# ansonb/FeTA_TMLR

Hardware: AMD Instinct MI355X
Metric: graphs/sec fwd+bwd, ZINC batch (N<=37,d=64,K=16) (higher is better)
Workload: dtype f32; 1 GPU; ZINC-shaped synthetic padded-graph batch, ChebConvDynamic block (attention + coefficient generator + spectral filter), fwd+bwd; graphs_per_gpu=128, global_batch=128, n_pad=37, d_model=64, heads=4, filter_order=4, k_eig=16, filter_mode=spectral, layers=3, norm=batch(per-rank stats), hip_graph=True, backward=single, two_phase=False, graph_collectives=False, ranks=1, parallelism=dp1

## Files before the change

### feta_tmlr_amd/_abi.py

```python
import ctypes as C
import os

import torch

_F = C.c_void_p
_I = C.c_void_p
_S = C.c_void_p

SIGNATURES = {
    'feta_version': ([], C.c_int),
    'feta_last_error': ([], C.c_char_p),
    'feta_attn_fwd': ([_F, _F, _F, C.c_int64, C.c_int64, _F, _I, _F, C.c_int64, C.c_int64,
                       _F, _F, C.c_float, C.c_int, C.c_int, C.c_int, C.c_int, _S], C.c_int),
    'feta_attn_bwd': ([_F, _F, _F, C.c_int64, C.c_int64, _F, _I, _F, _F, _F, C.c_int64, C.c_int64,
                       _F, _F, _F, _F, _F, C.c_float, C.c_int, C.c_int, C.c_int, C.c_int, _S],
                      C.c_int),
    'feta_coeff_fwd': ([_F, _I, _F, _F, _F, _F, C.c_int, C.c_int, C.c_int, C.c_int, _S], C.c_int),
    'feta_coeff_bwd_groups': ([C.c_int, C.c_int], C.c_int),
    'feta_coeff_bwd': ([_F, _I, _F, _F, _F, _F, _F, _F, _F, C.c_int, C.c_int, C.c_int, C.c_int, C.c_int, _S],
                       C.c_int),
    'feta_colsum': ([_F, _F, C.c_int, C.c_int, _S], C.c_int),
    'feta_cheb_filter_fwd': ([_F, C.c_int64, C.c_int64, _F, _F, _F, _I, _F, C.c_int64, C.c_int64,
                              C.c_int, C.c_int, C.c_int, C.c_int, C.c_int, C.c_int, _S], C.c_int),
    'feta_cheb_filter_bwd': ([_F, C.c_int64, C.c_int64, _F, _F, _I, _F, C.c_int64, C.c_int64,
                              _F, _F, _F, C.c_int, C.c_int, C.c_int, C.c_int, C.c_int, C.c_int, _S],
                             C.c_int),
    'feta_spec_filter_fwd': ([_F, C.c_int64, C.c_int64, _F, _F, _F, _F, _I, _F, C.c_int64, C.c_int64,
                              C.c_int, C.c_int, C.c_int, C.c_int, C.c_int, C.c_int, C.c_int, _S],
                             C.c_int),
    'feta_spec_filter_bwd': ([_F, C.c_int64, C.c_int64, _F, _F, _F, _I, _F, C.c_int64, C.c_int64,
                              _F, _F, _F, C.c_int, C.c_int, C.c_int, C.c_int, C.c_int, C.c_int,
                              C.c_int, _S], C.c_int),
    'feta_rowlin_blocks': ([C.c_int], C.c_int),
    'feta_rowlin_chunks': ([C.c_int], C.c_int),
    'feta_rowlin_fwd': ([_F, _F, _F, _F, _F, _F, _F, C.c_int, C.c_int, C.c_int, C.c_int, _S], C.c_int),
    'feta_rowlin_bwd': ([_F, _F, _F, _F, _F, _F, _F, _F, C.c_int, C.c_int, C.c_int, _S], C.c_int),
    'feta_bn_stats': ([_F, _F, C.c_int, C.c_int, _S], C.c_int),
    'feta_bn_stats_shift': ([_F, _F, _F, C.c_int, C.c_int, _S], C.c_int),
    'feta_bn_apply_fwd': ([_F, _F, _F, _F, _F, _F, _F, _F, _I, C.c_float, C.c_float, C.c_int, C.c_int, _S],
                          C.c_int),
    'feta_bn_bwd': ([_F, _F, _F, _F, _F, _F, _F, _F, C.c_int, C.c_int, _S], C.c_int),
    'feta_lhat_from_edges': ([_I, C.c_int64, _I, _I, _F, _F, C.c_int, C.c_int, C.c_int64, _S],
                             C.c_int),
    'feta_layernorm_blocks': ([C.c_int], C.c_int),
    'feta_layernorm_fwd': ([_F, _F, _F, C.c_float, _F, _F, C.c_int, C.c_int, _S], C.c_int),
    'feta_layernorm_bwd': ([_F, _F, _F, _F, _F, _F, C.c_int, _F, C.c_int, C.c_int, _S], C.c_int),
    'feta_layernorm_fwd_ex': ([_F, _F, _F, C.c_float, _F, _F, C.c_int, C.c_int, C.c_int, C.c_int, _S], C.c_int),
    'feta_layernorm_bwd_eps': ([_F, _F, _F, C.c_float, _F, _F, _F, C.c_int, _F, C.c_int, C.c_int, C.c_int, C.c_int, C.c_int, _S],
                               C.c_int),
    'feta_layernorm_bwd_ex': ([_F, _F, _F, _F, _F, _F, C.c_int, _F, C.c_int, C.c_int, C.c_int, C.c_int, C.c_int, _S],
                              C.c_int),
    'feta_eigh_sym_supported': ([C.c_int], C.c_int),
    'feta_eigh_sym_workspace_bytes': ([C.c_int, C.c_int], C.c_int64),
    'feta_eigh_sym': ([_F, _I, C.c_float, _F, _F, _I, _F, C.c_int, C.c_int, C.c_int, C.c_int, C.c_float, _S],
                      C.c_int),
    'feta_spectral_kernel': ([_F, _F, _I, C.c_int, C.c_float, C.c_int, C.c_float, C.c_int, _F,
                              C.c_int, C.c_int, C.c_int, _S], C.c_int),
}

SIGNATURES.update({
    'feta_attn_fwd_bf16': SIGNATURES['feta_attn_fwd'],
    'feta_attn_bwd_bf16': ([_F, _F, _F, C.c_int64, C.c_int64, _F, _I, _F, _F, C.c_int64, C.c_int64,
                            _F, _F, _F, _F, _F, C.c_float, C.c_int, C.c_int, C.c_int, C.c_int, _S], C.c_int),
    'feta_attn_fwd_drop': ([_F, _F, _F, C.c_int64, C.c_int64, _F, _I, _F, C.c_int64, C.c_int64, _F, _F, C.c_float,
                            C.c_float, C.c_uint64, C.c_uint64, C.c_int, C.c_int, C.c_int, C.c_int, C.c_int, _S], C.c_int),
    'feta_attn_bwd_drop': ([_F, _F, _F, C.c_int64, C.c_int64, _F, _I, _F, _F, C.c_int64, C.c_int64, _F, _F, _F, _F, _F,
                            C.c_float, C.c_float, C.c_uint64, C.c_uint64, C.c_int, C.c_int, C.c_int, C.c_int, C.c_int,
                            _S], C.c_int),
    'feta_attn_fwd_drop_dev': ([_F, _F, _F, C.c_int64, C.c_int64, _F, _I, _F, C.c_int64, C.c_int64, _F, _F, C.c_float,
                                C.c_float, _I, C.c_uint64, C.c_int, C.c_int, C.c_int, C.c_int, C.c_int, _S], C.c_int),
    'feta_attn_bwd_drop_dev': ([_F, _F, _F, C.c_int64, C.c_int64, _F, _I, _F, _F, C.c_int64, C.c_int64, _F, _F, _F, _F, _F,
                                C.c_float, C.c_float, _I, C.c_uint64, C.c_int, C.c_int, C.c_int, C.c_int, C.c_int,
                                _S], C.c_int),
    'feta_attn_fwd_stab': ([_F, _F, _F, C.c_int64, C.c_int64, _F, _I, _F, C.c_int64, C.c_int64, _F, _F, C.c_float,
                            C.c_int, C.c_int, C.c_int, C.c_int, C.c_int, C.c_int, _S], C.c_int),
    'feta_attn_bwd_stab': ([_F, _F, _F, C.c_int64, C.c_int64, _F, _I, _F, _F, C.c_int64, C.c_int64, _F, _F, _F, _F, _F,
                            C.c_float, C.c_int, C.c_int, C.c_int, C.c_int, C.c_int, C.c_int, _S], C.c_int),
    'feta_spec_filter_fwd_bf16': SIGNATURES['feta_spec_filter_fwd'],
    'feta_spec_filter_bwd_bf16': SIGNATURES['feta_spec_filter_bwd'],
})


class ColsumSeg(C.Structure):
    _fields_ = [('in_', _F), ('out', _F), ('R', C.c_int), ('C', C.c_int), ('ld', C.c_int),
                ('bcast_out', _F), ('bcast_rows', C.c_int)]


SIGNATURES['feta_colsum_multi'] = ([C.POINTER(ColsumSeg), C.c_int, _S], C.c_int)
SIGNATURES['feta_lin_supported'] = ([C.c_int, C.c_int, C.c_int], C.c_int)
SIGNATURES['feta_lin_fwd'] = ([_F, _F, _F, _F, C.c_int, C.c_int, C.c_int, _S], C.c_int)
SIGNATURES['feta_lin_bwd'] = ([_F, _F, _F, _F, _F, _F, C.c_int, C.c_int, C.c_int, C.POINTER(ColsumSeg), C.c_int, _S],
                              C.c_int)
SIGNATURES['feta_lin_fwd_ex'] = ([_F, _F, _F, _F, C.c_int, C.c_int, C.c_int, C.c_int, _S], C.c_int)
SIGNATURES['feta_lin_bwd_ex'] = ([_F, _F, _F, _F, _F, _F, C.c_int, C.c_int, C.c_int, C.POINTER(ColsumSeg), C.c_int, C.c_int,
                                  _S], C.c_int)


class RowLinEx(C.Structure):
    _fields_ = [
        ('x', _F), ('w', _F), ('bias', _F), ('rowscale', _F),
        ('M', C.c_int), ('KI', C.c_int), ('NO', C.c_int), ('relu', C.c_int),
        ('residual', _F), ('res_bn', _F), ('y', _F), ('stats', _F),
        ('x_bn', _F), ('x_stats', _F), ('Gx', C.c_int),
        ('x_gamma', _F), ('x_beta', _F), ('x_bn_out', _F), ('x_rmean', _F), ('x_rvar', _F), ('x_nbt', _I),
        ('momentum', C.c_float), ('eps', C.c_float),
        ('dy', _F), ('relu_y', _F), ('dx', _F), ('partial', _F), ('partial_ld', C.c_int),
        ('g_y', _F), ('g_bn', _F), ('g_sum', _F), ('Gs', C.c_int),
        ('g_fin', _F), ('g_fin_out', _F), ('dgamma', _F), ('dbeta', _F),
        ('add_plain', _F), ('add_dout', _F), ('add_y', _F), ('add_bn', _F), ('add_fin', _F),
        ('x2', _F), ('x_split', C.c_int), ('dx2', _F),
        ('sum_y', _F), ('sum_bn', _F), ('sum_out', _F), ('stats_shift', _F),
    ]


SIGNATURES.update({
    'feta_rowlin_fwd_ex': ([C.POINTER(RowLinEx), _S], C.c_int),
    'feta_rowlin_bwd_ex': ([C.POINTER(RowLinEx), _F, _S], C.c_int),
    'feta_bn_apply_fwd_prm': ([_F, _F, _F, _F, _F, _F, _F, _F, _I, C.c_float, C.c_float, C.c_int, C.c_int,
                               C.c_int, _S], C.c_int),
    'feta_bn_bwd_reduce': ([_F, _F, _F, _F, C.c_int, C.c_int, _S], C.c_int),
})



class SpecCat(C.Structure):
    _fields_ = [
        ('y2', _F), ('y2_sb', C.c_int64), ('y2_sn', C.c_int64), ('y2_bn', _F), ('y2_stats', _F), ('Gx', C.c_int),
        ('gamma', _F), ('beta', _F), ('bn_out', _F), ('rmean', _F), ('rvar', _F), ('nbt', _I),
        ('momentum', C.c_float), ('eps', C.c_float), ('M', C.c_int), ('w_cat', _F), ('b_cat', _F), ('out', _F),
    ]


class SpecCatGrad(C.Structure):
    _fields_ = [
        ('dout', _F), ('y2', _F), ('y2_sb', C.c_int64), ('y2_sn', C.c_int64), ('y2_bn', _F), ('filt', _F), ('w_cat', _F),
        ('dxn', _F), ('gs', _F), ('partial', _F), ('partial_ld', C.c_int64),
    ]


SIGNATURES.update({
    'feta_spec_cat_bwd_supported': ([C.c_int] * 6, C.c_int),
    'feta_spec_cat_bwd_rows': ([C.c_int], C.c_int),
    'feta_spec_filter_cat_bwd': ([_F, C.c_int64, C.c_int64, _F, _F, _F, _I, C.c_int64, C.c_int64, _F, _F, _F,
                                  C.c_int, C.c_int, C.c_int, C.c_int, C.c_int, C.c_int, C.c_int, C.POINTER(SpecCatGrad), _S],
                                 C.c_int),
    'feta_spec_cat_supported': ([C.c_int] * 6, C.c_int),
    'feta_spec_filter_cat_fwd': ([_F, C.c_int64, C.c_int64, _F, _F, _F, _F, _I, _F, C.c_int64, C.c_int64,
                                  C.c_int, C.c_int, C.c_int, C.c_int, C.c_int, C.c_int, C.c_int, C.POINTER(SpecCat), _S], C.c_int),
})


class AttnBlock(C.Structure):
    _fields_ = [
        ('x', _F), ('x_bn', _F), ('x_stats', _F), ('Gx', C.c_int),
        ('x_gamma', _F), ('x_beta', _F), ('x_bn_out', _F), ('x_rmean', _F), ('x_rvar', _F), ('x_nbt', _I),
        ('momentum', C.c_float), ('eps', C.c_float),
        ('w_in', _F), ('b_in', _F), ('w_out', _F), ('b_out', _F), ('pe', _F), ('n_real', _I),
        ('rowscale', _F), ('qkv', _F), ('out', _F), ('attn_stats', _F), ('attn', _F), ('y', _F),
        ('y_stats', _F), ('scale', C.c_float), ('B', C.c_int), ('N', C.c_int), ('M', C.c_int),
        ('row_sb', C.c_int64), ('row_sn', C.c_int64), ('tie_qk', C.c_int), ('dtype', C.c_int), ('y_shift', _F),
        ('out_f32', _F), ('x_ln_gamma', _F), ('x_ln_beta', _F), ('H', C.c_int),
    ]


SIGNATURES.update({
    'feta_attn_block_supported': ([C.c_int, C.c_int, C.c_int], C.c_int),
    'feta_attn_block_stat_rows': ([C.c_int, C.c_int], C.c_int),
    'feta_attn_out_supported': ([C.c_int, C.c_int, C.c_int], C.c_int),
    'feta_attn_out_stat_rows': ([C.c_int, C.c_int], C.c_int),
    'feta_attn_out_fwd': ([C.POINTER(AttnBlock), _S], C.c_int),
    'feta_attn_out_fwd_sums': ([C.POINTER(AttnBlock), C.POINTER(ColsumSeg), C.c_int, _S], C.c_int),
    'feta_attn_block_fwd': ([C.POINTER(AttnBlock), _S], C.c_int),
    'feta_attn_block_fwd_sums': ([C.POINTER(AttnBlock), C.POINTER(ColsumSeg), C.c_int, _S], C.c_int),
})



class CoeffFwdRole(C.Structure):
    _fields_ = [('attn', _F), ('n_real', _I), ('s', _F), ('gcn_bias', _F), ('cj', _F), ('pooled', _F),
                ('B', C.c_int), ('N', C.c_int), ('H', C.c_int), ('C', C.c_int)]


class CoeffBwdRole(C.Structure):
    _fields_ = [('cj', _F), ('n_real', _I), ('s', _F), ('gcn_bias', _F), ('dpooled', _F), ('partial', _F),
                ('B', C.c_int), ('N', C.c_int), ('H', C.c_int), ('C', C.c_int)]


class Ffn(C.Structure):
    _fields_ = [
        ('x', _F), ('x_bn', _F), ('x_stats', _F), ('Gx', C.c_int),
        ('x_gamma', _F), ('x_beta', _F), ('x_bn_out', _F), ('x_rmean', _F), ('x_rvar', _F), ('x_nbt', _I),
        ('momentum', C.c_float), ('eps', C.c_float),
        ('w1', _F), ('b1', _F), ('w2', _F), ('b2', _F), ('h', _F), ('y', _F), ('y_stats', _F),
        ('M', C.c_int), ('FF', C.c_int), ('dtype', C.c_int), ('y_shift', _F), ('y_f32', C.c_int),
        ('x_ln_gamma', _F), ('x_ln_beta', _F),
        ('y_ln_out', _F), ('y_ln_gamma', _F), ('y_ln_beta', _F), ('y_ln_eps', C.c_float), ('y_ln_f32', C.c_int),
    ]


SIGNATURES.update({
    'feta_ffn_supported': ([C.c_int, C.c_int], C.c_int),
    'feta_ffn_blocks': ([C.c_int], C.c_int),
    'feta_ffn_fwd': ([C.POINTER(Ffn), _S], C.c_int),
    'feta_ffn_fwd_coeff': ([C.POINTER(Ffn), C.POINTER(CoeffFwdRole), _S], C.c_int),
})

class AttnBlockGrad(C.Structure):
    _fields_ = [
        ('dy', _F), ('y1', _F), ('bn1', _F), ('g_sum', _F), ('Gs', C.c_int), ('fin_out', _F), ('dgamma', _F),
        ('dbeta', _F), ('rowscale', _F), ('w_out', _F), ('w_in', _F), ('qkv', _F), ('out', _F), ('dout2', _F),
        ('pe', _F), ('n_real', _I), ('attn_stats', _F), ('x0', _F), ('bn0', _F), ('dx', _F), ('dx_b', _F), ('sum_out', _F),
        ('partial', _F), ('partial_ld', C.c_int), ('scale', C.c_float), ('B', C.c_int), ('N', C.c_int), ('M', C.c_int),
        ('row_sb', C.c_int64), ('row_sn', C.c_int64), ('dtype', C.c_int), ('dout2_f32', C.c_int),
        ('ln1_gamma', _F), ('x0_ln_gamma', _F), ('x0_ln_beta', _F), ('ln_eps', C.c_float), ('H', C.c_int),
    ]


SIGNATURES.update({
    'feta_attn_block_bwd_supported': ([C.c_int, C.c_int, C.c_int], C.c_int),
    'feta_attn_block_bwd_blocks': ([C.c_int], C.c_int),
    'feta_attn_block_bwd': ([C.POINTER(AttnBlockGrad), _S], C.c_int),
    'feta_attn_block_bwd_sums': ([C.POINTER(AttnBlockGrad), C.POINTER(ColsumSeg), C.c_int, _S], C.c_int),
})


class FfnGrad(C.Structure):
    _fields_ = [
        ('dy', _F), ('dy_b', _F), ('g_y', _F), ('g_bn', _F), ('g_sum', _F), ('Gs', C.c_int), ('g_fin', _F), ('g_fin_out', _F),
        ('dgamma', _F), ('dbeta', _F), ('h', _F), ('w2', _F), ('w1', _F), ('x', _F), ('x_bn', _F), ('dx', _F),
        ('sum_out', _F), ('partial', _F), ('partial_ld', C.c_int), ('M', C.c_int), ('FF', C.c_int), ('dtype', C.c_int), ('g_f32', C.c_int),
        ('g_ln_gamma', _F), ('x_ln_gamma', _F), ('x_ln_beta', _F), ('ln_eps', C.c_float),
    ]


SIGNATURES.update({
    'feta_ffn_bwd_supported': ([C.c_int, C.c_int], C.c_int),
    'feta_ffn_bwd_blocks': ([C.c_int], C.c_int),
    'feta_ffn_bwd_chunks': ([C.c_int, C.c_int], C.c_int),
    'feta_ffn_bwd': ([C.POINTER(FfnGrad), _S], C.c_int),
    'feta_ffn_bwd_coeff': ([C.POINTER(FfnGrad), C.POINTER(CoeffBwdRole), _S], C.c_int),
})

class EncoderLayer(C.Structure):
    _fields_ = [
        ('w_in', _F), ('b_in', _F), ('w_out', _F), ('b_out', _F),
        ('n1_gamma', _F), ('n1_beta', _F), ('n1_mean', _F), ('n1_var', _F),
        ('w1', _F), ('b1', _F), ('w2', _F), ('b2', _F),
        ('n2_gamma', _F), ('n2_beta', _F), ('n2_mean', _F), ('n2_var', _F),
        ('n1_eps', C.c_float), ('n2_eps', C.c_float), ('tie_qk', C.c_int),
    ]


class EncoderInfer(C.Structure):
    _fields_ = [
        ('x', _F), ('row_sb', C.c_int64), ('row_sn', C.c_int64), ('pe', _F), ('n_real', _I), ('rowscale', _F),
        ('y', _F), ('out', _F), ('attn', _F), ('B', C.c_int), ('N', C.c_int), ('H', C.c_int), ('FF', C.c_int),
        ('L', C.c_int), ('norm', C.c_int), ('layers', C.c_void_p),
    ]


class EncoderInferEx(C.Structure):
    _fields_ = EncoderInfer._fields_ + [('dtype', C.c_int), ('in_dtype', C.c_int)]


class EncoderFwdSave(C.Structure):
    _fields_ = EncoderInferEx._fields_ + [
        ('qkv', _F), ('out_save', _F), ('attn_stats', _F), ('y1', _F), ('h', _F), ('y2', _F), ('y2_last_f32', _F),
        ('qkv_stride', C.c_int64), ('out_stride', C.c_int64), ('attn_stats_stride', C.c_int64), ('y1_stride', C.c_int64),
        ('h_stride', C.c_int64), ('y2_stride', C.c_int64),
    ]


SIGNATURES.update({
    'feta_encoder_fwd_save_supported': ([C.c_int, C.c_int, C.c_int, C.c_int, C.c_int, C.c_int, C.c_int], C.c_int),
    'feta_encoder_fwd_save': ([C.POINTER(EncoderFwdSave), _S], C.c_int),
    'feta_encoder_fwd_save_sums': ([C.POINTER(EncoderFwdSave), C.POINTER(ColsumSeg), C.c_int, _S], C.c_int),
    'feta_encoder_infer_supported': ([C.c_int, C.c_int, C.c_int, C.c_int, C.c_int], C.c_int),
    'feta_encoder_infer': ([C.POINTER(EncoderInfer), _S], C.c_int),
    'feta_encoder_infer_ex_supported': ([C.c_int, C.c_int, C.c_int, C.c_int, C.c_int, C.c_int], C.c_int),
    'feta_encoder_infer_ex': ([C.POINTER(EncoderInferEx), _S], C.c_int),
})

ABI_VERSION = 13


class FetaError(RuntimeError):
    pass


def _p(t):
    return None if t is None else C.c_void_p(t.data_ptr())


def _same_dtype(dtype, *tensors):
    for t in tensors:
        if t is not None and t.dtype != dtype:
            raise TypeError('expected %s operands, got %s' % (dtype, t.dtype))


def _stack_dtype(ptrs, names, f32_ok=()):
    dt = None
    for k in names:
        t = ptrs.get(k)
        if t is None or k in f32_ok and t.dtype == torch.float32:
            continue
        if dt is None:
            dt = t.dtype
        elif t.dtype != dt:
            raise TypeError('%s is %s, the other token tensors are %s' % (k, t.dtype, dt))
    if dt is None:
        dt = torch.float32
    if dt not in (torch.float32, torch.bfloat16):
        raise TypeError('token tensors must be float32 or bfloat16, got %s' % dt)
    for k, t in ptrs.items():
        if t is not None and k not in names and t.dtype == torch.bfloat16:
            raise TypeError('%s must not be bfloat16' % k)
    return 1 if dt == torch.bfloat16 else 0


def tok_strides(t):
    assert t.dim() == 4 and t.stride(3) == 1 and t.stride(2) == t.shape[3], \
        'token tensor must be a [B,N,H,dh] view with dense (H,dh)'
    return (t.stride(0) if t.shape[0] > 1 else 0), (t.stride(1) if t.shape[1] > 1 else 0)
# ... 44 lines not shown
                                                    1 if q.dtype == torch.bfloat16 else 0, b, n, h, dh, stream),
                        'feta_attn_fwd_drop')
            return
        if q.dtype == torch.bfloat16:
            _same_dtype(torch.bfloat16, k, v, pe, out, attn)
            self._check(self.lib.feta_attn_fwd_bf16(_p(q), _p(k), _p(v), sb, sn, _p(pe), _p(n_real),
                                                    _p(out), osb, osn, _p(attn), _p(stats), scale,
                                                    b, n, h, dh, stream), 'feta_attn_fwd_bf16')
            return
        self._check(self.lib.feta_attn_fwd(_p(q), _p(k), _p(v), sb, sn, _p(pe), _p(n_real),
                                           _p(out), osb, osn, _p(attn), _p(stats), scale,
                                           b, n, h, dh, stream), 'feta_attn_fwd')

    @staticmethod
    def attn_bwd_takes_dout2(n, dh, dtype=torch.float32, heads=None):
        if dtype != torch.float32:
            return False
        head_kernel = os.environ.get('FETA_ATTN_BWD_HEAD', '1') != '0'
        return (n <= 64 and dh <= 16) or (head_kernel and n <= 256 and dh == 16 and heads == 4)

    def attn_bwd(self, q, k, v, pe, n_real, out, dout, stats, delta, dq, dk, dv, scale, stream, dout2=None,
                 drop=None, clamp5=False):
        b, n, h, dh = q.shape
        sb, sn = tok_strides(q)
        for t in (k, v, dq, dk, dv):
            assert tok_strides(t) == (sb, sn)
        osb, osn = tok_strides(out)
        assert tok_strides(dout) == (osb, osn)
        if clamp5:
            assert dout2 is None and (drop is None or drop[0] == 0.0)
            _same_dtype(q.dtype, k, v, pe, out, dout, dq, dk, dv)
            self._check(self.lib.feta_attn_bwd_stab(_p(q), _p(k), _p(v), sb, sn, _p(pe), _p(n_real), _p(out), _p(dout),
                                                    osb, osn, _p(stats), _p(delta), _p(dq), _p(dk), _p(dv), scale, 1,
                                                    1 if q.dtype == torch.bfloat16 else 0, b, n, h, dh, stream),
                        'feta_attn_bwd_stab')
            return
        if drop is not None and drop[0] > 0.0 and torch.is_tensor(drop[1]):
            _same_dtype(q.dtype, k, v, pe, out, dout, dq, dk, dv)
            assert dout2 is None
            self._check(self.lib.feta_attn_bwd_drop_dev(_p(q), _p(k), _p(v), sb, sn, _p(pe), _p(n_real), _p(out), _p(dout),
                                                        osb, osn, _p(stats), _p(delta), _p(dq), _p(dk), _p(dv), scale,
                                                        float(drop[0]), _p(drop[1]), int(drop[2]),
                                                        1 if q.dtype == torch.bfloat16 else 0, b, n, h, dh, stream),
                        'feta_attn_bwd_drop_dev')
            return
        if drop is not None and drop[0] > 0.0:
            _same_dtype(q.dtype, k, v, pe, out, dout, dq, dk, dv)
            assert dout2 is None
            self._check(self.lib.feta_attn_bwd_drop(_p(q), _p(k), _p(v), sb, sn, _p(pe), _p(n_real), _p(out), _p(dout),
                                                    osb, osn, _p(stats), _p(delta), _p(dq), _p(dk), _p(dv), scale,
                                                    float(drop[0]), int(drop[1]), int(drop[2]),
                                                    1 if q.dtype == torch.bfloat16 else 0, b, n, h, dh, stream),
                        'feta_attn_bwd_drop')
            return
        if q.dtype == torch.bfloat16:
            _same_dtype(torch.bfloat16, k, v, pe, out, dout, dq, dk, dv)
            assert dout2 is None
            self._check(self.lib.feta_attn_bwd_bf16(_p(q), _p(k), _p(v), sb, sn, _p(pe), _p(n_real),
                                                    _p(out), _p(dout), osb, osn, _p(stats), _p(delta),
                                                    _p(dq), _p(dk), _p(dv), scale, b, n, h, dh, stream),
                        'feta_attn_bwd_bf16')
            return
        self._check(self.lib.feta_attn_bwd(_p(q), _p(k), _p(v), sb, sn, _p(pe), _p(n_real),
                                           _p(out), _p(dout), _p(dout2), osb, osn, _p(stats), _p(delta),
                                           _p(dq), _p(dk), _p(dv), scale, b, n, h, dh, stream),
                    'feta_attn_bwd')

    def coeff_fwd(self, attn, n_real, s, gcn_bias, cj, pooled, stream):
        b, h, n, _ = attn.shape
        c = s.shape[0]
        self._check(self.lib.feta_coeff_fwd(_p(attn), _p(n_real), _p(s), _p(gcn_bias), _p(cj),
                                            _p(pooled), b, n, h, c, stream), 'feta_coeff_fwd')

    def coeff_bwd_groups(self, b, h):
        return self.lib.feta_coeff_bwd_groups(b, h)

    def coeff_bwd(self, cj, n_real, s, gcn_bias, dpooled, partial, ds, dbias, b, n, h, stream, dw_dense=None):
        c = s.shape[0]
        self._check(self.lib.feta_coeff_bwd(_p(cj), _p(n_real), _p(s), _p(gcn_bias), _p(dpooled),
                                            _p(partial), _p(ds), _p(dbias), _p(dw_dense),
                                            0 if dw_dense is None else dw_dense.shape[0], b, n, h, c, stream),
                    'feta_coeff_bwd')

    @staticmethod
    def _colsum_segs(pairs):
        segs = (ColsumSeg * max(len(pairs), 1))()
        for sg, pr in zip(segs, pairs):
            x, out = pr[0], pr[1]
            assert x.stride(1) == 1
            sg.in_, sg.out, sg.R, sg.C, sg.ld = x.data_ptr(), out.data_ptr(), x.shape[0], x.shape[1], x.stride(0)
            if len(pr) > 2 and pr[2] is not None:
                sg.bcast_out, sg.bcast_rows = pr[2].data_ptr(), pr[2].shape[0]
        return segs

    def colsum_multi(self, pairs, stream):
        self._check(self.lib.feta_colsum_multi(self._colsum_segs(pairs), len(pairs), stream), 'feta_colsum_multi')

    def lin_supported(self, r, k, n):
        return bool(self.lib.feta_lin_supported(r, k, n))

    def lin_fwd(self, x, w, bias, y, stream, bf16=False):
        r, k = x.shape
        self._check(self.lib.feta_lin_fwd_ex(_p(x), _p(w), _p(bias), _p(y), r, k, w.shape[0], int(bool(bf16)), stream),
                    'feta_lin_fwd')

    def lin_bwd(self, x, w, dy, dx, dw, db, stream, pairs=(), bf16=False):
        r, k = x.shape
        self._check(self.lib.feta_lin_bwd_ex(_p(x), _p(w), _p(dy), _p(dx), _p(dw), _p(db), r, k, w.shape[0],
                                             self._colsum_segs(pairs), len(pairs), int(bool(bf16)), stream),
                    'feta_lin_bwd')

    def colsum(self, x, out, stream):
        r, c = x.shape
        self._check(self.lib.feta_colsum(_p(x), _p(out), r, c, stream), 'feta_colsum')

    def cheb_filter_fwd(self, x, lhat, coeff, bias, n_real, y, order, share, stream):
        b, n, h, dh = x.shape
        xsb, xsn = tok_strides(x)
        ysb, ysn = tok_strides(y)
        self._check(self.lib.feta_cheb_filter_fwd(_p(x), xsb, xsn, _p(lhat), _p(coeff), _p(bias),
                                                  _p(n_real), _p(y), ysb, ysn, b, n, h, dh, order,
                                                  int(share), stream), 'feta_cheb_filter_fwd')

    def cheb_filter_bwd(self, x, lhat, coeff, n_real, dy, dx, dcoeff, dbias_part, order, share,
                        stream):
        b, n, h, dh = x.shape
        xsb, xsn = tok_strides(x)
        assert tok_strides(dx) == (xsb, xsn)
        ysb, ysn = tok_strides(dy)
        self._check(self.lib.feta_cheb_filter_bwd(_p(x), xsb, xsn, _p(lhat), _p(coeff), _p(n_real),
                                                  _p(dy), ysb, ysn, _p(dx), _p(dcoeff),
                                                  _p(dbias_part), b, n, h, dh, order, int(share),
                                                  stream), 'feta_cheb_filter_bwd')

    def spec_filter_fwd(self, x, u, lam, coeff, bias, n_real, y, order, share, stream):
        b, n, h, dh = x.shape
        k = u.shape[2]
        xsb, xsn = tok_strides(x)
        ysb, ysn = tok_strides(y)
        fn, nm = self.lib.feta_spec_filter_fwd, 'feta_spec_filter_fwd'
        if x.dtype == torch.bfloat16:
            _same_dtype(torch.bfloat16, u, coeff, y)
            fn, nm = self.lib.feta_spec_filter_fwd_bf16, 'feta_spec_filter_fwd_bf16'
        self._check(fn(_p(x), xsb, xsn, _p(u), _p(lam), _p(coeff), _p(bias), _p(n_real), _p(y), ysb, ysn,
                       b, n, h, dh, order, k, int(share), stream), nm)

    def spec_cat_supported(self, n, h, dh, order, k, share):
        return bool(self.lib.feta_spec_cat_supported(n, h, dh, order, k, int(share)))

    def spec_filter_cat_fwd(self, x, u, lam, coeff, bias, n_real, y, order, share, stream, y2, w_cat, b_cat, out,
                            y2_bn=None, y2_stats=None, Gx=0, gamma=None, beta=None, bn_out=None, rmean=None, rvar=None,
                            nbt=None, momentum=0.1, eps=1e-5):
        b, n, h, dh = x.shape
        k = u.shape[2]
        xsb, xsn = tok_strides(x)
        ysb, ysn = tok_strides(y)
        assert tok_strides(out) == (ysb, ysn)
        c = SpecCat()
        c.y2_sb, c.y2_sn = tok_strides(y2)
        c.Gx, c.momentum, c.eps, c.M = Gx, momentum, eps, b * n
        for name, t in (('y2', y2), ('y2_bn', y2_bn), ('y2_stats', y2_stats), ('gamma', gamma), ('beta', beta),
                        ('bn_out', bn_out), ('rmean', rmean), ('rvar', rvar), ('nbt', nbt), ('w_cat', w_cat),
                        ('b_cat', b_cat), ('out', out)):
            if t is not None:
                setattr(c, name, t.data_ptr())
        self._check(self.lib.feta_spec_filter_cat_fwd(_p(x), xsb, xsn, _p(u), _p(lam), _p(coeff), _p(bias), _p(n_real), _p(y),
                                                      ysb, ysn, b, n, h, dh, order, k, int(share), C.byref(c), stream),
                    'feta_spec_filter_cat_fwd')

    def spec_cat_bwd_supported(self, n, h, dh, order, k, share):
        return bool(self.lib.feta_spec_cat_bwd_supported(n, h, dh, order, k, int(share)))

    def spec_cat_bwd_rows(self, b):
        return int(self.lib.feta_spec_cat_bwd_rows(b))

    def spec_filter_cat_bwd(self, x, u, lam, coeff, n_real, filt, dx, dcoeff, dbias_part, order, share, stream, dout, y2,
                            w_cat, dxn, partial, y2_bn=None, gs=None):
        b, n, h, dh = x.shape
        k = u.shape[2]
        xsb, xsn = tok_strides(x)
        assert tok_strides(dx) == (xsb, xsn)
        ysb, ysn = tok_strides(filt)
        c = SpecCatGrad()
        c.y2_sb, c.y2_sn = tok_strides(y2)
        assert tok_strides(dout) == (c.y2_sb, c.y2_sn) and tok_strides(dxn) == (c.y2_sb, c.y2_sn)
        assert partial.shape[0] == self.spec_cat_bwd_rows(b) and partial.stride(1) == 1
        assert gs is None or gs.shape[0] == partial.shape[0]
        c.partial_ld = partial.stride(0)
        for name, t in (('dout', dout), ('y2', y2), ('y2_bn', y2_bn), ('filt', filt), ('w_cat', w_cat), ('dxn', dxn),
                        ('gs', gs), ('partial', partial)):
            if t is not None:
                setattr(c, name, t.data_ptr())
        self._check(self.lib.feta_spec_filter_cat_bwd(_p(x), xsb, xsn, _p(u), _p(lam), _p(coeff), _p(n_real), ysb, ysn,
                                                      _p(dx), _p(dcoeff), _p(dbias_part), b, n, h, dh, order, k, int(share),
                                                      C.byref(c), stream), 'feta_spec_filter_cat_bwd')

    def spec_filter_bwd(self, x, u, lam, coeff, n_real, dy, dx, dcoeff, dbias_part, order, share,
                        stream):
        b, n, h, dh = x.shape
        k = u.shape[2]
        xsb, xsn = tok_strides(x)
        assert tok_strides(dx) == (xsb, xsn)
        ysb, ysn = tok_strides(dy)
        fn, nm = self.lib.feta_spec_filter_bwd, 'feta_spec_filter_bwd'
        if x.dtype == torch.bfloat16:
            _same_dtype(torch.bfloat16, u, coeff, dy, dx, dcoeff)
            fn, nm = self.lib.feta_spec_filter_bwd_bf16, 'feta_spec_filter_bwd_bf16'
        self._check(fn(_p(x), xsb, xsn, _p(u), _p(lam), _p(coeff), _p(n_real), _p(dy), ysb, ysn, _p(dx),
                       _p(dcoeff), _p(dbias_part), b, n, h, dh, order, k, int(share), stream), nm)

    ROWLIN_DIMS = (16, 32, 64, 128, 192, 256)

    def rowlin_blocks(self, m):
        return self.lib.feta_rowlin_blocks(m)

    def rowlin_chunks(self, m):
        return self.lib.feta_rowlin_chunks(m)

    def rowlin_fwd(self, x, w, bias, rowscale, residual, y, stats, relu, stream):
        m, ki = x.shape
        no = w.shape[0]
        self._check(self.lib.feta_rowlin_fwd(_p(x), _p(w), _p(bias), _p(rowscale), _p(residual), _p(y),
                                             _p(stats), int(relu), m, ki, no, stream), 'feta_rowlin_fwd')

    def rowlin_bwd(self, x, w, dy, rowscale, ysaved, dx, partial, dwdb, stream):
        m, ki = x.shape
        no = w.shape[0]
        self._check(self.lib.feta_rowlin_bwd(_p(x), _p(w), _p(dy), _p(rowscale), _p(ysaved), _p(dx),
                                             _p(partial), _p(dwdb), m, ki, no, stream), 'feta_rowlin_bwd')

    def bn_stats(self, y, stats, stream, shift=None):
        m, d = y.shape
        assert stats.shape[0] == self.rowlin_blocks(m) + 1, 'stats needs rowlin_blocks(M) + 1 rows (shift row)'
        self._check(self.lib.feta_bn_stats_shift(_p(y), _p(shift), _p(stats), m, d, stream), 'feta_bn_stats')

    def bn_apply_fwd(self, y, stats, gamma, beta, out, mean_rstd, running_mean, running_var, momentum,
                     eps, stream, nbt=None):
        m, d = y.shape
        self._check(self.lib.feta_bn_apply_fwd(_p(y), _p(stats), _p(gamma), _p(beta), _p(out),
                                               _p(mean_rstd), _p(running_mean), _p(running_var), _p(nbt),
                                               momentum, eps, m, d, stream), 'feta_bn_apply_fwd')

    def bn_bwd(self, y, dout, mean_rstd, gamma, partial, dy, dgamma, dbeta, stream):
        m, d = y.shape
        self._check(self.lib.feta_bn_bwd(_p(y), _p(dout), _p(mean_rstd), _p(gamma), _p(partial), _p(dy),
                                         _p(dgamma), _p(dbeta), m, d, stream), 'feta_bn_bwd')

    def rowlin_ex(self, m, ki, no, relu=False, momentum=0.1, eps=1e-5, Gx=0, Gs=0, partial_ld=0,
# ... 60 lines not shown

    def attn_block_bwd_supported(self, n, d_model, heads):
        return bool(self.lib.feta_attn_block_bwd_supported(n, d_model, heads))

    def attn_block_bwd_blocks(self, b):
        return int(self.lib.feta_attn_block_bwd_blocks(b))

    def attn_block_bwd(self, b, n, scale, stream, seq_first=True, Gs=0, partial_ld=0, partial_ptr=None, sums=(), ln_eps=1e-5,
                       heads=4, **ptrs):
        d = AttnBlockGrad()
        d.B, d.N, d.M, d.scale, d.Gs, d.partial_ld, d.ln_eps, d.H = b, n, b * n, scale, Gs, partial_ld, ln_eps, heads
        d.row_sb, d.row_sn = (1, b) if seq_first else (n, 1)
        if partial_ptr is not None:
            d.partial = partial_ptr
        d.dtype = _stack_dtype(ptrs, ('dy', 'y1', 'qkv', 'out', 'dout2', 'pe', 'x0', 'dx', 'dx_b'), f32_ok=('dout2',))
        d.dout2_f32 = int(ptrs.get('dout2') is not None and ptrs['dout2'].dtype == torch.float32)
        for k, t in ptrs.items():
            if t is not None:
                setattr(d, k, t.data_ptr())
        if sums:
            self._check(self.lib.feta_attn_block_bwd_sums(C.byref(d), self._colsum_segs(sums), len(sums), stream),
                        'feta_attn_block_bwd_sums')
        else:
            self._check(self.lib.feta_attn_block_bwd(C.byref(d), stream), 'feta_attn_block_bwd')

    def ffn_supported(self, d_model, ff):
        return bool(self.lib.feta_ffn_supported(d_model, ff))

    def ffn_blocks(self, m):
        return int(self.lib.feta_ffn_blocks(m))

    def ffn_fwd(self, m, ff, stream, momentum=0.1, eps=1e-5, Gx=0, coeff=None, y_ln_eps=1e-5, **ptrs):
        self.ffn_launch(self.ffn_desc(m, ff, momentum, eps, Gx, y_ln_eps=y_ln_eps, **ptrs), stream, coeff)

    def ffn_desc(self, m, ff, momentum=0.1, eps=1e-5, Gx=0, y_ln_eps=1e-5, **ptrs):
        d = Ffn()
        d.M, d.FF, d.momentum, d.eps, d.Gx, d.y_ln_eps = m, ff, momentum, eps, Gx, y_ln_eps
        d.dtype = _stack_dtype(ptrs, ('x', 'h', 'y', 'y_ln_out'), f32_ok=('y', 'y_ln_out'))
        d.y_f32 = int(ptrs['y'].dtype == torch.float32)
        if ptrs.get('y_ln_out') is not None:
            d.y_ln_f32 = int(ptrs['y_ln_out'].dtype == torch.float32)
        for k, t in ptrs.items():
            if t is not None:
                setattr(d, k, t.data_ptr())
        return d

    def ffn_launch(self, desc, stream, coeff=None):
        if coeff is None:
            self._check(self.lib.feta_ffn_fwd(C.byref(desc), stream), 'feta_ffn_fwd')
            return
        attn, n_real, s, gcn_bias, cj, pooled = coeff
        b, h, n, _ = attn.shape
        r = CoeffFwdRole()
        r.attn, r.n_real, r.s, r.gcn_bias, r.cj, r.pooled = (t.data_ptr() for t in (attn, n_real, s, gcn_bias, cj, pooled))
        r.B, r.N, r.H, r.C = b, n, h, s.shape[0]
        self._check(self.lib.feta_ffn_fwd_coeff(C.byref(desc), C.byref(r), stream), 'feta_ffn_fwd_coeff')

    def ffn_bwd_supported(self, d_model, ff):
        return bool(self.lib.feta_ffn_bwd_supported(d_model, ff))

    def ffn_bwd_blocks(self, m):
        return int(self.lib.feta_ffn_bwd_blocks(m))

    def ffn_bwd_chunks(self, m, ff):
        return int(self.lib.feta_ffn_bwd_chunks(m, ff))

    def ffn_bwd_desc(self, m, ff, Gs=0, partial_ld=0, partial_ptr=None, ln_eps=1e-5, **ptrs):
        d = FfnGrad()
        d.M, d.FF, d.Gs, d.partial_ld, d.ln_eps = m, ff, Gs, partial_ld, ln_eps
        if partial_ptr is not None:
            d.partial = partial_ptr
        d.dtype = _stack_dtype(ptrs, ('dy', 'dy_b', 'g_y', 'h', 'x', 'dx'), f32_ok=('dy', 'g_y'))
        d.g_f32 = int(ptrs['dy'].dtype == torch.float32)
        if ptrs.get('g_y') is not None and ptrs['g_y'].dtype != ptrs['dy'].dtype:
            raise TypeError('dy and g_y must share a dtype')
        for k, t in ptrs.items():
            if t is not None:
                setattr(d, k, t.data_ptr())
        return d

    def ffn_bwd_launch(self, desc, stream, coeff=None):
        if coeff is None:
            self._check(self.lib.feta_ffn_bwd(C.byref(desc), stream), 'feta_ffn_bwd')
            return
        cj, n_real, s, gcn_bias, dpooled, partial, b, n, h = coeff
        r = CoeffBwdRole()
        r.cj, r.n_real, r.s, r.gcn_bias, r.dpooled, r.partial = (t.data_ptr() for t in
                                                                (cj, n_real, s, gcn_bias, dpooled, partial))
        r.B, r.N, r.H, r.C = b, n, h, s.shape[0]
        self._check(self.lib.feta_ffn_bwd_coeff(C.byref(desc), C.byref(r), stream), 'feta_ffn_bwd_coeff')

    def ffn_bwd(self, m, ff, stream, coeff=None, **kw):
        self.ffn_bwd_launch(self.ffn_bwd_desc(m, ff, **kw), stream, coeff)

    def bn_apply_fwd_prm(self, y, stats, gamma, beta, out, bn_prm, running_mean, running_var, momentum,
                         eps, stream, nbt=None):
        m, d = y.shape
        self._check(self.lib.feta_bn_apply_fwd_prm(_p(y), _p(stats), _p(gamma), _p(beta), _p(out),
                                                   _p(bn_prm), _p(running_mean), _p(running_var), _p(nbt),
                                                   momentum, eps, m, d, stats.shape[0] - 1, stream),
                    'feta_bn_apply_fwd_prm')

    def bn_bwd_reduce(self, y, dout, bn_prm, partial, stream):
        m, d = y.shape
        self._check(self.lib.feta_bn_bwd_reduce(_p(y), _p(dout), _p(bn_prm), _p(partial), m, d, stream),
                    'feta_bn_bwd_reduce')

    def lhat_from_edges(self, edge_index, node_graph, node_off, deg, lhat, stream):
        b, n, _ = lhat.shape
        self._check(self.lib.feta_lhat_from_edges(_p(edge_index), edge_index.shape[1],
                                                  _p(node_graph), _p(node_off), _p(deg), _p(lhat),
                                                  b, n, node_graph.shape[0], stream),
                    'feta_lhat_from_edges')

    def layernorm_blocks(self, m):
        return self.lib.feta_layernorm_blocks(m)

    @staticmethod
    def _dt(t):
        if t.dtype == torch.float32:
            return 0
        if t.dtype == torch.bfloat16:
            return 1
        raise TypeError('float32 or bfloat16 rows, got %s' % t.dtype)

    def layernorm_fwd(self, y, gamma, beta, eps, out, stats, stream):
        m, d = y.shape
        self._check(self.lib.feta_layernorm_fwd_ex(_p(y), _p(gamma), _p(beta), eps, _p(out), _p(stats), m, d,
                                                   self._dt(y), self._dt(out), stream), 'feta_layernorm_fwd')

    def layernorm_bwd(self, dout, y, stats, gamma, dy, partial, dgdb, stream, partial_ld=0, partial_ptr=None, eps=1e-5):
        m, d = y.shape
        pp = _p(partial) if partial_ptr is None else C.c_void_p(partial_ptr)
        self._check(self.lib.feta_layernorm_bwd_eps(_p(dout), _p(y), _p(stats), eps, _p(gamma), _p(dy), pp, partial_ld,
                                                    _p(dgdb), m, d, self._dt(dout), self._dt(y), self._dt(dy), stream),
                    'feta_layernorm_bwd')

    def eigh_sym_supported(self, n):
        return bool(self.lib.feta_eigh_sym_supported(n))

    def eigh_sym_workspace_bytes(self, b, n):
        return int(self.lib.feta_eigh_sym_workspace_bytes(b, n))

    def eigh_sym(self, a, n_real, shift, u, lam, sweeps, max_sweeps, tol, stream, workspace=None):
        b, n, k = u.shape
        if workspace is None and self.eigh_sym_workspace_bytes(b, n) > 0:
            workspace = torch.empty(self.eigh_sym_workspace_bytes(b, n) // 4, dtype=torch.float32, device=a.device)
        self._check(self.lib.feta_eigh_sym(_p(a), _p(n_real), shift, _p(u), _p(lam), _p(sweeps), _p(workspace),
                                           b, n, k, max_sweeps, tol, stream), 'feta_eigh_sym')

    def spectral_kernel(self, u, lam, n_real, mode, beta, p, lam_offset, zero_diag, out, stream):
        b, n, k = u.shape
        self._check(self.lib.feta_spectral_kernel(_p(u), _p(lam), _p(n_real), mode, beta, p, lam_offset,
                                                  int(zero_diag), _p(out), b, n, k, stream),
                    'feta_spectral_kernel')

    def encoder_infer_supported(self, n, d_model, heads, ff, nl):
        return bool(self.lib.feta_encoder_infer_supported(n, d_model, heads, ff, nl))

    @staticmethod
    def _encoder_table(layers):
        table = (EncoderLayer * len(layers))()
        for e, lp in zip(table, layers):
            for k, v in lp.items():
                if torch.is_tensor(v):
                    _same_dtype(torch.float32, v)
# ... 85 lines not shown
```

### feta_tmlr_amd/csrc/coeff.hip

```cpp
#include <cmath>

#include "feta_abi_common.h"
#include <feta_device.h>
#include <cstdlib>

#include "feta_coeff.h"
#include "feta_colsum.h"

namespace feta {

__global__ __launch_bounds__(kCoeffThreads) void coeff_fwd_kernel(
    const float* __restrict__ attn, const int32_t* __restrict__ n_real, const float* __restrict__ s,
    const float* __restrict__ gbias, float* __restrict__ cj_out, float* __restrict__ pooled, int B,
    int N, int H, int C, int stage) {
  coeff_fwd_body(attn, n_real, s, gbias, cj_out, pooled, B, N, H, C, stage, (int)blockIdx.x, (int)blockIdx.y,
                 (int)gridDim.y);
}

__global__ __launch_bounds__(kCoeffWideThreads) void coeff_fwd_wide_kernel(
    const float* __restrict__ attn, const int32_t* __restrict__ n_real, const float* __restrict__ s,
    const float* __restrict__ gbias, float* __restrict__ cj_out, float* __restrict__ pooled, int B,
    int N, int H, int C) {
  coeff_fwd_body<kCoeffWideThreads>(attn, n_real, s, gbias, cj_out, pooled, B, N, H, C, 2, (int)blockIdx.x);
}

__global__ __launch_bounds__(kCoeffThreads) void coeff_bwd_kernel(
    const float* __restrict__ cj, const int32_t* __restrict__ n_real, const float* __restrict__ s,
    const float* __restrict__ gbias, const float* __restrict__ dpooled, float* __restrict__ partial,
    int B, int N, int H, int C, int G) {
  coeff_bwd_body(cj, n_real, s, gbias, dpooled, partial, B, N, H, C, G, (int)blockIdx.x, (int)blockIdx.y);
}

constexpr int kCsCols = 16, kCsSlices = 64;
__global__ __launch_bounds__(kCsCols * kCsSlices) void colsum_kernel(const float* __restrict__ in,
                                                                      float* __restrict__ out, int R,
                                                                      int C, int ld) {
  float* red = feta_lds;
  const int lc = threadIdx.x & (kCsCols - 1);
  const int slice = threadIdx.x / kCsCols;
  const int col = blockIdx.x * kCsCols + lc;
  float acc = 0.0f;
  if (col < C)
    for (int r = slice; r < R; r += kCsSlices) acc += in[(int64_t)r * ld + col];
  red[threadIdx.x] = acc;
  __syncthreads();
  for (int half = kCsSlices / 2; half >= 1; half >>= 1) {
    if (slice < half) red[threadIdx.x] += red[threadIdx.x + half * kCsCols];
    __syncthreads();
  }
  if (slice == 0 && col < C) out[col] = red[lc];
}

__global__ __launch_bounds__(64) void colsum_wide_kernel(const float* __restrict__ in, float* __restrict__ out,
                                                         int R, int C4, int ld) {
  const int c4 = blockIdx.x * 64 + threadIdx.x;
  if (c4 >= C4) return;
  const float* p = in + 4 * (int64_t)c4;
  float4 acc = make_float4(0.0f, 0.0f, 0.0f, 0.0f);
  int r = 0;
  for (; r + 8 <= R; r += 8) {
    float4 v[8];
#pragma unroll
    for (int i = 0; i < 8; ++i) v[i] = *reinterpret_cast<const float4*>(p + (int64_t)(r + i) * ld);
#pragma unroll
    for (int i = 0; i < 8; ++i) {
      acc.x += v[i].x; acc.y += v[i].y; acc.z += v[i].z; acc.w += v[i].w;
    }
  }
  for (; r < R; ++r) {
    const float4 v = *reinterpret_cast<const float4*>(p + (int64_t)r * ld);
    acc.x += v.x; acc.y += v.y; acc.z += v.z; acc.w += v.w;
  }
  *reinterpret_cast<float4*>(out + 4 * (int64_t)c4) = acc;
}

int launch_colsum_strided(const float* in, float* out, int R, int C, int ld, hipStream_t stream) {
  if (R <= 256 && C >= 4096 && (C & 3) == 0 && (ld & 3) == 0 && aligned16(in) && aligned16(out)) {
    const int c4 = C / 4;
    auto kern = colsum_wide_kernel;
    hipLaunchKernelGGL(kern, dim3((c4 + 63) / 64), dim3(64), 0, stream, in, out, R, c4, ld);
    return check_launch("feta_colsum");
  }
  const dim3 grid((C + kCsCols - 1) / kCsCols), block(kCsCols * kCsSlices);
  auto kern = colsum_kernel;
  hipLaunchKernelGGL(kern, grid, block, kCsCols * kCsSlices * sizeof(float), stream, in, out, R, C, ld);
  return check_launch("feta_colsum");
}
int launch_colsum(const float* in, float* out, int R, int C, hipStream_t stream) {
  return launch_colsum_strided(in, out, R, C, C, stream);
}

struct ColsumSegs {
  feta_colsum_seg seg[FETA_COLSUM_MAX_SEGS];
  int tile_end[FETA_COLSUM_MAX_SEGS];
  int nseg;
};

__global__ __launch_bounds__(kCsCols * kCsSlices) void colsum_multi_kernel(ColsumSegs a) {
  float* red = feta_lds;
  int si = 0;
  while (si + 1 < a.nseg && (int)blockIdx.x >= a.tile_end[si]) ++si;
  const feta_colsum_seg sg = a.seg[si];
  const int tile = (int)blockIdx.x - (si > 0 ? a.tile_end[si - 1] : 0);
  const int lc = threadIdx.x & (kCsCols - 1);
  const int slice = threadIdx.x / kCsCols;
  const int col = tile * kCsCols + lc;
  const int ld = sg.ld > 0 ? sg.ld : sg.C;
  float acc = 0.0f;
  if (col < sg.C)
    for (int r = slice; r < sg.R; r += kCsSlices) acc += sg.in[(int64_t)r * ld + col];
  red[threadIdx.x] = acc;
  __syncthreads();
  for (int half = kCsSlices / 2; half >= 1; half >>= 1) {
// ... 73 lines not shown
    a.tile_end[i] = tiles;
  }
  auto kern = colsum_multi_kernel;
  hipLaunchKernelGGL(kern, dim3(tiles), dim3(kCsCols * kCsSlices), kCsCols * kCsSlices * sizeof(float), stream, a);
  return check_launch("feta_colsum_multi");
}

}

using namespace feta;

extern "C" int feta_coeff_fwd(const float* attn, const int32_t* n_real, const float* s,
                              const float* gcn_bias, float* cj, float* pooled, int B, int N, int H,
                              int C, feta_stream_t stream) {
  FETA_REQUIRE(attn && n_real && s && gcn_bias && cj && pooled, "coeff_fwd: null pointer");
  FETA_REQUIRE(B > 0 && H > 0 && C > 0 && N > 0 && N <= kCoeffThreads,
               "coeff_fwd: need 0 < N <= %d (got %d)", kCoeffThreads, N);
  const int want = N > 64 ? 2 : 1;
  const int stage = sizeof(float) * (size_t)coeff_fwd_lds_floats_mode(N, want) <= 150 * 1024 ? want : 0;
  const size_t lds = sizeof(float) * (size_t)coeff_fwd_lds_floats_mode(N, stage);
  if (N > 64) {
    const size_t wide = sizeof(float) * (size_t)coeff_fwd_lds_floats_mode(N, 2, kCoeffWideThreads);
    const char* e = getenv("FETA_COEFF_WIDE");
    if (wide <= 160 * 1024 && !(e != nullptr && e[0] == '0')) {
      auto kern = coeff_fwd_wide_kernel;
      static LdsSeen wide_seen;
      allow_dynamic_lds(kern, wide, wide_seen);
      hipLaunchKernelGGL(kern, dim3(B * H), dim3(kCoeffWideThreads), wide, (hipStream_t)stream, attn, n_real, s, gcn_bias,
                         cj, pooled, B, N, H, C);
      return check_launch("feta_coeff_fwd");
    }
  }
  const int cs = (N > 64 && C >= 4 * kCoeffThreads) ? 4 : 1;
  const dim3 grid(B * H, cs), block(kCoeffThreads);
  auto kern = coeff_fwd_kernel;
  static LdsSeen lds_seen;
  allow_dynamic_lds(kern, lds, lds_seen);
  hipLaunchKernelGGL(kern, grid, block, lds, (hipStream_t)stream, attn, n_real, s, gcn_bias, cj,
                     pooled, B, N, H, C, stage);
  return check_launch("feta_coeff_fwd");
}

extern "C" int feta_coeff_bwd_groups(int B, int H) {
  const int t = B * H;
  if (t >= 2048) return 4 * kCoeffGroupsMax;
  return t < kCoeffGroupsMax ? t : kCoeffGroupsMax;
}

extern "C" int feta_colsum_multi(const feta_colsum_seg* segs, int nseg, feta_stream_t stream) {
  FETA_REQUIRE(segs != nullptr && nseg >= 1 && nseg <= FETA_COLSUM_MAX_SEGS, "colsum_multi: 1..%d segments",
               FETA_COLSUM_MAX_SEGS);
  for (int i = 0; i < nseg; ++i)
    FETA_REQUIRE(segs[i].in && segs[i].out && segs[i].R > 0 && segs[i].C > 0 && (segs[i].ld == 0 || segs[i].ld >= segs[i].C) &&
                 (segs[i].bcast_out == nullptr || segs[i].bcast_rows > 0), "colsum_multi: bad segment %d", i);
  return launch_colsum_multi(segs, nseg, (hipStream_t)stream);
}

extern "C" int feta_coeff_bwd(const float* cj, const int32_t* n_real, const float* s,
                              const float* gcn_bias, const float* dpooled, float* partial, float* ds,
                              float* dbias, float* dw_dense, int dw_rows, int B, int N, int H, int C,
                              feta_stream_t stream) {
  FETA_REQUIRE(cj && n_real && s && gcn_bias && dpooled && partial && (ds == nullptr || dbias != nullptr),
               "coeff_bwd: null pointer");
  FETA_REQUIRE(B > 0 && H > 0 && C > 0 && N > 0, "coeff_bwd: empty shape");
  const int G = feta_coeff_bwd_groups(B, H);
  const dim3 grid((C + kCoeffThreads - 1) / kCoeffThreads, G), block(kCoeffThreads);
  auto kern = coeff_bwd_kernel;
  hipLaunchKernelGGL(kern, grid, block, kCoeffPass * N * sizeof(float), (hipStream_t)stream, cj, n_real, s,
                     gcn_bias, dpooled, partial, B, N, H, C, G);
  int rc = check_launch("feta_coeff_bwd");
  if (rc != FETA_OK || ds == nullptr) return rc;
  if (dw_dense != nullptr) {
    FETA_REQUIRE(dw_rows > 0, "coeff_bwd: dw_dense needs dw_rows");
    feta_colsum_seg segs[2] = {{partial, ds, G, C, 2 * C, dw_dense, dw_rows}, {partial + C, dbias, G, C, 2 * C, nullptr, 0}};
    return launch_colsum_multi(segs, 2, (hipStream_t)stream);
  }
  if (dbias == ds + C)
    return launch_colsum(partial, ds, G, 2 * C, (hipStream_t)stream);
  rc = launch_colsum_strided(partial, ds, G, C, 2 * C, (hipStream_t)stream);
  if (rc != FETA_OK) return rc;
  return launch_colsum_strided(partial + C, dbias, G, C, 2 * C, (hipStream_t)stream);
}

extern "C" int feta_colsum(const float* in, float* out, int R, int C, feta_stream_t stream) {
  FETA_REQUIRE(in && out && R > 0 && C > 0, "colsum: bad arguments");
  return launch_colsum(in, out, R, C, (hipStream_t)stream);
}
```

### feta_tmlr_amd/csrc/feta_coeff.h

```cpp
#pragma once
#include <cmath>

#include "feta_abi_common.h"
#include <feta_device.h>

namespace feta {

constexpr int kCoeffThreads = 256;
constexpr int kCoeffWideThreads = 1024;
constexpr int kCoeffGroupsMax = 128;
constexpr int kCoeffLdsTileMax = 12 * 1024;

template <int TH = 256>
__device__ __forceinline__ void coeff_fwd_body(
    const float* __restrict__ attn, const int32_t* __restrict__ n_real, const float* __restrict__ s,
    const float* __restrict__ gbias, float* __restrict__ cj_out, float* __restrict__ pooled, int B,
    int N, int H, int C, int stage, int blk, int cs = 0, int CS = 1) {
  float* dis = feta_lds;
  float* cjs = feta_lds + N;
  float* ps = feta_lds + 2 * N;
  float* tile = ps + 4 * 64;
  const int h = blk / B, b = blk % B;
  const int n = n_real[b];
  const float* a = attn + ((int64_t)b * H + h) * N * N;
// ... 189 lines not shown
    for (int k = 0; k < 4; ++k) {
      const int c = c0 + k * TH;
      if (c < cend) pooled[(int64_t)blk * C + c] = acc[k] * inv_n;
    }
  }
}

constexpr int kCoeffPass = 4;
__device__ __forceinline__ void coeff_bwd_body(
    const float* __restrict__ cj, const int32_t* __restrict__ n_real, const float* __restrict__ s,
    const float* __restrict__ gbias, const float* __restrict__ dpooled, float* __restrict__ partial,
    int B, int N, int H, int C, int G, int bx, int grp) {
  float* cjs = feta_lds;
  const int c = bx * kCoeffThreads + threadIdx.x;
  const int cc = c < C ? c : C - 1;
  const int total = B * H;
  const float sc = s[cc], bc = gbias[cc];
  float as = 0.0f, ab = 0.0f;
  for (int blk0 = grp; blk0 < total; blk0 += G * kCoeffPass) {
    float dp[kCoeffPass];
    int nn[kCoeffPass];
#pragma unroll
    for (int u = 0; u < kCoeffPass; ++u) {
      const int blk = blk0 + u * G;
      const int bc_ = blk < total ? blk : total - 1;
      nn[u] = blk < total ? n_real[bc_ % B] : 0;
      dp[u] = dpooled[(int64_t)bc_ * C + cc];
    }
    __syncthreads();
    for (int i = threadIdx.x; i < kCoeffPass * N; i += kCoeffThreads) {
      const int u = i / N, k = i - u * N;
      const int blk = blk0 + u * G;
      cjs[i] = blk < total ? cj[(int64_t)blk * N + k] : 0.0f;
    }
    __syncthreads();
    int nmax = 0;
#pragma unroll
    for (int u = 0; u < kCoeffPass; ++u) nmax = max(nmax, nn[u]);
    if (N <= 64 && (int64_t)total * N <= 32768) {
      float dpn[kCoeffPass], as_[kCoeffPass], ab_[kCoeffPass];
#pragma unroll
      for (int u = 0; u < kCoeffPass; ++u) {
        dpn[u] = nn[u] > 0 ? dp[u] / (float)nn[u] : 0.0f;
        as_[u] = ab_[u] = 0.0f;
      }
      for (int i = 0; i < nmax; ++i) {
#pragma unroll
        for (int u = 0; u < kCoeffPass; ++u) {
          const float ci = cjs[u * N + i];
          const float z = fast_tanh(ci * sc + bc);
          const float t = i < nn[u] ? dpn[u] * (1.0f - z * z) : 0.0f;
          as_[u] += t * ci;
          ab_[u] += t;
        }
      }
#pragma unroll
      for (int u = 0; u < kCoeffPass; ++u) {
        as += as_[u];
        ab += ab_[u];
      }
    } else {
#pragma unroll
      for (int u = 0; u < kCoeffPass; ++u) {
        const int n = nn[u];
        if (n == 0) continue;
        const float dpn = dp[u] / (float)n;
        for (int i = 0; i < n; ++i) {
          const float ci = cjs[u * N + i];
          const float z = fast_tanh(ci * sc + bc);
          const float t = dpn * (1.0f - z * z);
          as += t * ci;
          ab += t;
        }
      }
    }
  }
  if (c < C) {
    partial[(int64_t)grp * 2 * C + c] = as;
    partial[(int64_t)grp * 2 * C + C + c] = ab;
  }
}


__host__ __device__ inline int coeff_fwd_stage(int N) {
  if (N <= 64) return 1;
  return N * ((N + 3) & ~3) <= kCoeffLdsTileMax ? 2 : 0;
}
__host__ __device__ inline int coeff_fwd_lds_floats_mode(int N, int stage, int threads = kCoeffThreads) {
  return 2 * N + (stage == 2 ? 4 * threads + N * ((N + 3) & ~3) : 4 * 64 + (stage == 1 ? N * N : 0));
}
__host__ __device__ inline int coeff_fwd_lds_floats(int N) { return coeff_fwd_lds_floats_mode(N, coeff_fwd_stage(N)); }

struct CoeffFwdRole {
  const float* attn; const int32_t* n_real; const float* s; const float* gbias; float* cj; float* pooled;
  int B, N, H, C;
};
struct CoeffBwdRole {
  const float* cj; const int32_t* n_real; const float* s; const float* gbias; const float* dpooled; float* partial;
  int B, N, H, C, G;
};

}
```

### feta_tmlr_amd/csrc/ffn_bwd.hip

```cpp
#include <cstdlib>

#include "feta_abi_common.h"
#include "feta_coeff.h"
#include "feta_ln.h"
#include "feta_lp.h"
#include "feta_rowops.h"

namespace feta {

typedef feta_ffn_grad FfnGradArgs;

constexpr int kFbD = 64;
constexpr int kFbRows = 32;
constexpr int kFbSlice = 32;

struct FfnBwdGeom {
  int XB;
  int RC;
  int per;
  int NS;
  int xcd;
  int wxcd;
  int cxw;
  int main_grid;
  int role, role_lead;
};

inline int ffn_bwd_xblocks(int M) {
  int cap = 512;
  if (const char* e = getenv("FETA_FFN_MAX_GRID")) cap = atoi(e) > 0 ? atoi(e) : cap;
  const int nblk = (M + kFbRows - 1) / kFbRows;
  return nblk < cap ? nblk : cap;
}

template <int NV>
__device__ __forceinline__ void g2_of(float (&v)[NV], const float (&yy)[NV], const float* gv, int o, bool gbn) {
  if (gbn) {
#pragma unroll
    for (int s = 0; s < NV; ++s) {
      const float xh = (yy[s] - gv[kFbD + o + s]) * gv[2 * kFbD + o + s];
      v[s] = gv[o + s] * (v[s] - gv[3 * kFbD + o + s] - xh * gv[4 * kFbD + o + s]);
    }
  }
}

template <class T> struct FbPad { static constexpr int W = 16; };
template <> struct FbPad<bf16_t> { static constexpr int W = 8; };

template <class T>
inline size_t ffn_bwd_lds_bytes(int FF, bool gbn) {
  const size_t x_lds = kFbRows * (kFbD + Lp<T>::PAD) + kFbRows * (FF + Lp<T>::PAD);
  const size_t w_lds = 2 * 64 * (kFbD + FbPad<T>::W) + 2 * 64 * (kFbSlice + FbPad<T>::W);
  return sizeof(T) * (x_lds > w_lds ? x_lds : w_lds) + sizeof(float) * (gbn ? 5 * kFbD + reduce_scratch_floats(kFbD) : 0);
}

template <class T, int FF>
__global__ __launch_bounds__(kRowThreads) void ffn_bwd_kernel(FfnGradArgs a, FfnBwdGeom ge, CoeffBwdRole cb) {
  typedef Lp<T> L;
  typedef typename L::Op Op;
  typedef typename L::Vec Vec;
  constexpr int D = kFbD, NJ2 = FF / 16, VEC = L::VEC, RV = D / VEC;
  int bid = (int)blockIdx.x;
  if (bid < ge.role_lead || bid >= ge.role_lead + ge.main_grid) {
    const int r = bid < ge.role_lead ? bid : bid - ge.main_grid;
    const int nbx = (cb.C + kCoeffThreads - 1) / kCoeffThreads;
    if (r < ge.role)
      coeff_bwd_body(cb.cj, cb.n_real, cb.s, cb.gbias, cb.dpooled, cb.partial, cb.B, cb.N, cb.H, cb.C, cb.G, r % nbx, r / nbx);
    return;
  }
  bid -= ge.role_lead;
  const int tid = threadIdx.x, lane = tid & 63, w = tid >> 6, lq = lane & 15, g = lane >> 4;
  const T* gdy = reinterpret_cast<const T*>(a.dy);
  const T* gdyb = reinterpret_cast<const T*>(a.dy_b);
  const T* ggy = reinterpret_cast<const T*>(a.g_y);
  const T* ghh = reinterpret_cast<const T*>(a.h);
  const T* gxx = reinterpret_cast<const T*>(a.x);
  T* gdx = reinterpret_cast<T*>(a.dx);
  int xblk, wbi;
  if (ge.xcd) {
    const int xcd = bid & 7, v = bid >> 3, items = 2 + ge.NS;
    const int item = v % items, rc = (v / items) * 8 + xcd;
    if (rc >= ge.RC) return;
    xblk = item < 2 ? 2 * rc + item : -1;
    wbi = item < 2 ? -1 : rc * ge.NS + (item - 2);
    if (item < 2 && xblk >= ge.XB) return;
  } else {
    xblk = bid < ge.XB ? bid : -1;
    wbi = bid - ge.XB;
    if (wbi >= 0 && ge.wxcd) {
      const int xcd = wbi & 7, v = wbi >> 3;
      const int si_ = v % ge.NS, rc_ = (v / ge.NS) * 8 + xcd;
      if (rc_ >= ge.RC) return;
      wbi = rc_ * ge.NS + si_;
    }
  }
  int x_lo = xblk, x_hi = (a.M + kFbRows - 1) / kFbRows, x_step = ge.XB;
  if (ge.cxw > 0) {
    const int xcd = bid & 7, v = bid >> 3, items = ge.cxw + ge.NS;
    const int item = v % items, rc = (v / items) * 8 + xcd;
    if (rc >= ge.RC) return;
    if (item < ge.cxw) {
      xblk = rc * ge.cxw + item;
      wbi = -1;
      x_lo = rc * (ge.per / 2) + item;
      x_hi = min((rc + 1) * (ge.per / 2), x_hi);
      x_step = ge.cxw;
    } else {
      xblk = -1;
      wbi = rc * ge.NS + (item - ge.cxw);
    }
  }
  float* gv = feta_lds;
  float* after = gv;
  const bool gbn = a.g_bn != nullptr;
  const bool gln = a.g_ln_gamma != nullptr, xln = a.x_ln_gamma != nullptr;
  const float ln_eps = a.ln_eps;
  float gl2[L::VEC], gl1[L::VEC], bl1[L::VEC];
  {
    const int c0v = L::VEC * (tid % (kFbD / L::VEC));
#pragma unroll
    for (int e = 0; e < L::VEC; ++e) {
      gl2[e] = gln ? a.g_ln_gamma[c0v + e] : 1.0f;
      gl1[e] = xln ? a.x_ln_gamma[c0v + e] : 1.0f;
      bl1[e] = xln ? a.x_ln_beta[c0v + e] : 0.0f;
    }
  }
  if (gbn) {
    float* scr = gv + 5 * D;
    after = scr;
    const int cpre = min(tid, D - 1);
    const float bn_scale = a.g_bn[cpre], bn_mean = a.g_bn[2 * D + cpre], bn_rstd = a.g_bn[3 * D + cpre];
    if (a.g_sum != nullptr) {
      reduce_partials_t<kRowThreads, 32>(a.g_sum, a.Gs, D, scr + 2 * D, scr);
      for (int c = tid; c < D; c += kRowThreads) {
        gv[3 * D + c] = scr[c] / (float)a.M;
        gv[4 * D + c] = scr[D + c] / (float)a.M;
        if (bid == 0) {
          if (a.dbeta != nullptr) a.dbeta[c] = scr[c];
          if (a.dgamma != nullptr) a.dgamma[c] = scr[D + c];
          if (a.g_fin_out != nullptr) {
            a.g_fin_out[c] = gv[3 * D + c];
            a.g_fin_out[D + c] = gv[4 * D + c];
          }
        }
      }
    } else {
      for (int c = tid; c < 2 * D; c += kRowThreads) gv[3 * D + c] = a.g_fin[c];
    }
    if (tid < D) {
      gv[tid] = bn_scale;
// ... 271 lines not shown
  float* p = a.partial + (int64_t)rc * (a.partial_ld > 0 ? (int64_t)a.partial_ld
                                                         : (int64_t)(2 * D * FF + D + FF + (gln ? 2 * D : 0)));
  float* pW2 = p;
  float* pb2 = p + D * FF;
  float* pW1 = pb2 + D;
  float* pb1 = pW1 + FF * D;
#pragma unroll
  for (int ct = 0; ct < 2; ++ct)
#pragma unroll
    for (int r = 0; r < 4; ++r) {
      pW2[(int64_t)(16 * w + 4 * g + r) * FF + c0 + 16 * ct + lq] = aW2[ct][r];
      pW1[(int64_t)(c0 + 16 * ct + 4 * g + r) * D + 16 * w + lq] = aW1[ct][r];
    }
  __syncthreads();
  float* red2 = after;
  float* red1 = after + kRowThreads * VEC;
  float* red3 = red1 + 4 * 2 * 16;
  float* red4 = red3 + kRowThreads * VEC;
  if (gln && si == 0) {
#pragma unroll
    for (int e = 0; e < VEC; ++e) {
      red3[tid * VEC + e] = dgam[e];
      red4[tid * VEC + e] = dbet[e];
    }
  }
#pragma unroll
  for (int e = 0; e < VEC; ++e) red2[tid * VEC + e] = cs2[e];
#pragma unroll
  for (int t = 0; t < 2; ++t)
#pragma unroll
    for (int r = 0; r < 4; ++r) {
      const float sv = row16_sum(cs1[t][r]);
      if (lq == 0) red1[(w * 2 + t) * 16 + 4 * g + r] = sv;
    }
  __syncthreads();
  if (si == 0 && tid < D) {
    const int c4 = tid / VEC, e = tid % VEC;
    float sv = 0.0f;
    for (int k = 0; k < kRowThreads / RV; ++k) sv += red2[(c4 + RV * k) * VEC + e];
    pb2[tid] = sv;
    if (gln) {
      float sg = 0.0f, sb = 0.0f;
      for (int k = 0; k < kRowThreads / RV; ++k) {
        sg += red3[(c4 + RV * k) * VEC + e];
        sb += red4[(c4 + RV * k) * VEC + e];
      }
      pb1[FF + tid] = sg;
      pb1[FF + D + tid] = sb;
    }
  }
  if (tid < kFbSlice) {
    const int t = tid >> 4, cc = tid & 15;
    pb1[c0 + tid] = (red1[(0 * 2 + t) * 16 + cc] + red1[(1 * 2 + t) * 16 + cc]) +
                    (red1[(2 * 2 + t) * 16 + cc] + red1[(3 * 2 + t) * 16 + cc]);
  }
}

extern int row_chunks(int M);

static int ffn_bwd_main_grid(int M, int RC, int NS) {
  const int XB = ffn_bwd_xblocks(M), nblk = (M + kFbRows - 1) / kFbRows, nrb16 = (M + 15) / 16;
  const int per = (nrb16 + RC - 1) / RC;
  const bool xcd = XB == nblk && per == 4;
  return xcd ? 8 * ((RC + 7) / 8) * (2 + NS) : XB + 8 * ((RC + 7) / 8) * NS;
}
static int ffn_bwd_chunks_for(int M, int ff) {
  const int rc = row_chunks(M), ns = ff / kFbSlice;
  if (const char* e = getenv("FETA_FFN_BWD_RC_HALF"))
    if (atoi(e) == 0) return rc;
  const int half = (rc + 1) / 2;
  if (rc >= 2 && ffn_bwd_main_grid(M, rc, ns) > 512 && ffn_bwd_main_grid(M, half, ns) <= 512) return half;
  return rc;
}

template <class T, int FF>
int launch_ffn_bwd(const FfnGradArgs& a, const CoeffBwdRole& cb, hipStream_t stream) {
  FfnBwdGeom ge{};
  ge.XB = ffn_bwd_xblocks(a.M);
  ge.RC = ffn_bwd_chunks_for(a.M, FF);
  const int nrb16 = (a.M + 15) / 16;
  ge.per = (nrb16 + ge.RC - 1) / ge.RC;
  ge.NS = FF / kFbSlice;
  size_t lds = ffn_bwd_lds_bytes<T>(FF, a.g_bn != nullptr);
  const int role = cb.cj != nullptr ? ((cb.C + kCoeffThreads - 1) / kCoeffThreads) * cb.G : 0;
  if (role > 0 && sizeof(float) * (size_t)(kCoeffPass * cb.N) > lds) lds = sizeof(float) * (size_t)(kCoeffPass * cb.N);
  auto kern = ffn_bwd_kernel<T, FF>;
  static LdsSeen seen;
  allow_dynamic_lds(kern, lds, seen);
  const int nblk = (a.M + kFbRows - 1) / kFbRows;
  ge.xcd = (ge.XB == nblk && ge.per == 4) ? 1 : 0;
  if (const char* e = getenv("FETA_FFN_BWD_XCD")) ge.xcd = ge.xcd && atoi(e) != 0;
  ge.wxcd = ge.xcd ? 0 : 1;
  if (const char* e = getenv("FETA_FFN_BWD_WXCD")) ge.wxcd = ge.wxcd && atoi(e) != 0;
  ge.cxw = 0;
  if (const char* e = getenv("FETA_FFN_BWD_CXW")) {
    if (atoi(e) != 0 && !ge.xcd && ge.wxcd && ge.per % 2 == 0 && ge.XB >= ge.RC && ge.XB % ge.RC == 0) ge.cxw = ge.XB / ge.RC;
  }
  if (ge.cxw > 0) ge.wxcd = 0;
  const int grid = ge.xcd ? 8 * ((ge.RC + 7) / 8) * (2 + ge.NS)
                 : ge.cxw > 0 ? 8 * ((ge.RC + 7) / 8) * (ge.cxw + ge.NS)
                              : ge.XB + (ge.wxcd ? 8 * ((ge.RC + 7) / 8) * ge.NS : ge.RC * ge.NS);
  ge.main_grid = grid;
  ge.role = role;
  ge.role_lead = 8 * ((role + 7) / 8);
  if (const char* e = getenv("FETA_COEFF_ROLE_FIRST")) if (atoi(e) == 0) ge.role_lead = 0;
  hipLaunchKernelGGL(kern, dim3(grid + (ge.role_lead > 0 ? ge.role_lead : role)), dim3(kRowThreads), lds, stream, a, ge, cb);
  return check_launch("feta_ffn_bwd");
}

}

using namespace feta;

extern "C" int feta_ffn_bwd_supported(int d_model, int ff) { return (d_model == kFbD && (ff == 64 || ff == 128)) ? 1 : 0; }

extern "C" int feta_ffn_bwd_blocks(int M) { return ffn_bwd_xblocks(M); }
extern "C" int feta_ffn_bwd_chunks(int M, int ff) { return (M < 1 || !feta_ffn_bwd_supported(kFbD, ff)) ? 0 : ffn_bwd_chunks_for(M, ff); }

extern "C" int feta_ffn_bwd(const feta_ffn_grad* d, feta_stream_t stream) { return feta_ffn_bwd_coeff(d, nullptr, stream); }

extern "C" int feta_ffn_bwd_coeff(const feta_ffn_grad* d, const feta_coeff_bwd_role* c, feta_stream_t stream) {
  FETA_REQUIRE(d != nullptr, "ffn_bwd: null descriptor");
  CoeffBwdRole cb{};
  if (c != nullptr) {
    FETA_REQUIRE(c->cj && c->n_real && c->s && c->gcn_bias && c->dpooled && c->partial, "ffn_bwd_coeff: null pointer");
    FETA_REQUIRE(c->B > 0 && c->H > 0 && c->C > 0 && c->N > 0, "ffn_bwd_coeff: empty shape");
    cb = CoeffBwdRole{c->cj, c->n_real, c->s, c->gcn_bias, c->dpooled, c->partial, c->B, c->N, c->H, c->C,
                      feta_coeff_bwd_groups(c->B, c->H)};
  }
  const FfnGradArgs& a = *d;
  FETA_REQUIRE(a.dy && a.h && a.w2 && a.w1 && a.x && a.dx && a.partial && a.M > 0, "ffn_bwd: null pointer / empty");
  FETA_REQUIRE(feta_ffn_bwd_supported(kFbD, a.FF), "ffn_bwd: dim_feedforward %d not in {64,128}", a.FF);
  FETA_REQUIRE(!a.g_y || a.g_ln_gamma || (a.g_bn && (a.g_sum || a.g_fin)), "ffn_bwd: g_y needs g_bn and g_sum | g_fin, or g_ln_gamma");
  FETA_REQUIRE(!a.g_ln_gamma || (a.g_y && !a.g_bn && !a.g_sum && !a.g_fin), "ffn_bwd: g_ln_gamma needs g_y and excludes g_bn / g_sum / g_fin");
  FETA_REQUIRE(!a.x_ln_gamma || (a.x_ln_beta && !a.x_bn), "ffn_bwd: x_ln_gamma needs x_ln_beta and excludes x_bn");
  FETA_REQUIRE(!a.g_bn || a.g_y, "ffn_bwd: g_bn needs g_y");
  FETA_REQUIRE(!a.g_sum || a.Gs > 0, "ffn_bwd: g_sum needs Gs");
  FETA_REQUIRE(!a.sum_out || a.x_bn, "ffn_bwd: sum_out needs x_bn (the BatchNorm that produced x)");
  FETA_REQUIRE(aligned16(a.dy_b) && aligned16(a.dy) && aligned16(a.h) && aligned16(a.x) && aligned16(a.dx) && aligned16(a.g_y) &&
               aligned16(a.x_bn) && aligned16(a.g_sum), "ffn_bwd: pointers must be 16-byte aligned");
  FETA_REQUIRE(a.dtype == FETA_F32 || a.dtype == FETA_BF16, "ffn_bwd: dtype %d", a.dtype);
  if (a.dtype == FETA_BF16) {
    if (a.FF == 64) return launch_ffn_bwd<bf16_t, 64>(a, cb, (hipStream_t)stream);
    return launch_ffn_bwd<bf16_t, 128>(a, cb, (hipStream_t)stream);
  }
  if (a.FF == 64) return launch_ffn_bwd<float, 64>(a, cb, (hipStream_t)stream);
  return launch_ffn_bwd<float, 128>(a, cb, (hipStream_t)stream);
}
```

### feta_tmlr_amd/csrc/filter.hip

```cpp
#include "feta_abi_common.h"
#include "feta_rowops.h"
#include "feta_tiles.h"

namespace feta {

struct FilterArgs {
  const float* x;
  const float* lhat;
  const float* u;
  const float* lam;
  const float* coeff;
  const float* bias;
  const int32_t* n_real;
  const float* dy;
  float* y;
  float* dx;
  float* dcoeff;
  float* dbias_part;
  int64_t xsb, xsn, ysb, ysn;
  int B, N, H, P, K;
  int share;
  int total;
};

constexpr int kFWaves = 4;


template <int DH>
__device__ __forceinline__ f32x4 load_acc(const float* p, int64_t sb, int64_t sn, int b, int h,
                                          int row0, int nvalid, int ct, int lq, int g) {
  f32x4 v;
  const int c = 16 * ct + lq;
#pragma unroll
  for (int r = 0; r < 4; ++r) {
    const int node = row0 + 4 * g + r;
    v[r] = (node < nvalid && c < DH) ? tok_row(p, sb, sn, b, node, h, DH)[c] : 0.0f;
  }
  return v;
}

template <int DH>
__device__ __forceinline__ float w_b(const float* w, int k, int j, int s, int ct, int lq, int g) {
  const int c = 16 * j + 4 * g + s, cp = 16 * ct + lq;
  return (c < DH && cp < DH) ? w[(k * DH + c) * DH + cp] : 0.0f;
}

template <int DH>
__device__ __forceinline__ float4 w_row4(const float* w, int k, int ct, int j, int lq, int g) {
  const int c = 16 * ct + lq, cp = 16 * j + 4 * g;
  if (c < DH && cp < DH) return *reinterpret_cast<const float4*>(w + (k * DH + c) * DH + cp);
  return make_float4(0.0f, 0.0f, 0.0f, 0.0f);
}

__device__ __forceinline__ float4 keep4(bool c, const float4& v) {
  return make_float4(c ? v.x : 0.0f, c ? v.y : 0.0f, c ? v.z : 0.0f, c ? v.w : 0.0f);
}

__device__ __forceinline__ float f4(const float4& v, int s) {
  return s == 0 ? v.x : (s == 1 ? v.y : (s == 2 ? v.z : v.w));
}

template <int DH>
__device__ __forceinline__ void xw_tile(const Feat<DH>& xf, const float* w, int k, int lq, int g,
                                        f32x4 (&z)[Feat<DH>::CT]) {
  constexpr int CT = Feat<DH>::CT, NJ = Feat<DH>::NJ;
#pragma unroll
  for (int ct = 0; ct < CT; ++ct) {
    z[ct] = zero4();
#pragma unroll
    for (int j = 0; j < NJ; ++j)
#pragma unroll
      for (int s = 0; s < 4; ++s) z[ct] = mfma16(xf.f[j][s], w_b<DH>(w, k, j, s, ct, lq, g), z[ct]);
  }
}

template <int DH>
__device__ __forceinline__ void dyw_tile(const Feat<DH>& dyf, const float* w, int k, int lq, int g,
                                         f32x4 (&gk)[Feat<DH>::CT]) {
  constexpr int CT = Feat<DH>::CT, NJ = Feat<DH>::NJ;
#pragma unroll
  for (int ct = 0; ct < CT; ++ct) {
    gk[ct] = zero4();
#pragma unroll
// ... 1133 lines not shown
    const float4 l4 = *reinterpret_cast<const float4*>(lams + 16 * et + 4 * g);
#pragma unroll
    for (int r = 0; r < 4; ++r) {
      float tk[kMaxOrder];
      cheb_poly(f4(l4, r), PP, tk);
#pragma unroll
      for (int k = 0; k < PP; ++k) dwa[k] = mfma16(xt[et][r] * tk[k], dyt[et][r], dwa[k]);
    }
  }
#pragma unroll
  for (int k = 0; k < PP; ++k)
#pragma unroll
    for (int r = 0; r < 4; ++r) dw[(k * DH + 4 * g + r) * DH + lq] = dwa[k][r];

  f32x4 dxt[ET_MAX];
#pragma unroll
  for (int et = 0; et < ET_MAX; ++et) {
    float tk[kMaxOrder];
    cheb_poly(lams[16 * et + lq], PP, tk);
    dxt[et] = zero4();
#pragma unroll
    for (int k = 0; k < PP; ++k) {
      dxt[et] = mfma16(dytT[et][0] * tk[k], wr[k].x, dxt[et]);
      dxt[et] = mfma16(dytT[et][1] * tk[k], wr[k].y, dxt[et]);
      dxt[et] = mfma16(dytT[et][2] * tk[k], wr[k].z, dxt[et]);
      dxt[et] = mfma16(dytT[et][3] * tk[k], wr[k].w, dxt[et]);
    }
  }

  f32x4 dx[NT_MAX];
#pragma unroll
  for (int nt = 0; nt < NT_MAX; ++nt) {
    dx[nt] = zero4();
    if (16 * nt < n) {
#pragma unroll
      for (int et = 0; et < ET_MAX; ++et) {
        const float4 ub = *reinterpret_cast<const float4*>(Us + (16 * nt + lq) * UP + 16 * et + 4 * g);
        dx[nt] = mfma16(ub.x, dxt[et][0], dx[nt]);
        dx[nt] = mfma16(ub.y, dxt[et][1], dx[nt]);
        dx[nt] = mfma16(ub.z, dxt[et][2], dx[nt]);
        dx[nt] = mfma16(ub.w, dxt[et][3], dx[nt]);
      }
    }
  }
  __syncthreads();
#pragma unroll
  for (int nt = 0; nt < NT_MAX; ++nt)
#pragma unroll
    for (int r = 0; r < 4; ++r) Xs[(16 * nt + 4 * g + r) * XP + DH * h + lq] = dx[nt][r];
  __syncthreads();
#pragma unroll
  for (int i = 0; i < NT_MAX; ++i) {
    const int idx = tid + 256 * i, node = idx >> 4, q = idx & 15;
    if (node < a.N)
      *reinterpret_cast<float4*>(tok_row(a.dx, a.xsb, a.xsn, b, node, 0, DH) + 4 * q) =
          *reinterpret_cast<const float4*>(Xs + node * XP + 4 * q);
  }
}

struct CatArgs {
  const float* y2;
  int64_t y2sb, y2sn;
  const float* y2_bn;
  const float* y2_stats;
  int Gx;
  const float* gamma; const float* beta;
  float* bn_out; float* rmean; float* rvar; int64_t* nbt;
  float momentum, eps;
  int M;
  const float* w_cat;
  const float* b_cat;
  float* out;
};

constexpr int kCatD = 64;

template <int NT_MAX, int ET_MAX>
__host__ __device__ inline int spec_cat_fwd_lds_floats(int pp) {
  constexpr int NR = 16 * NT_MAX, UP = 16 * ET_MAX + 4;
  return 2 * NR * kGraphXP + NR * UP + 16 * ET_MAX + 4 * pp * 16 * kGraphWP + 16 * ET_MAX * (kCatD + 4) + 2 * kCatD +
         reduce_scratch_floats(kCatD, 256);
}

template <int NT_MAX, int ET_MAX, int PP>
__global__ __launch_bounds__(256) void spec_cat_fwd_graph_kernel(FilterArgs a, CatArgs c) {
  constexpr int DH = 16, XP = kGraphXP, UP = 16 * ET_MAX + 4, WP = kGraphWP, NR = 16 * NT_MAX, D = kCatD, YP = D + 4;
  const int tid = threadIdx.x, lane = tid & 63, h = tid >> 6, lq = lane & 15, g = lane >> 4;
  const int b = blockIdx.x;
  const int n = a.n_real[b], nm1 = max(n - 1, 0), Nm1 = a.N - 1;
  float* Xs = feta_lds;
  float* Ys = Xs + NR * XP;
  float* Us = Ys + NR * XP;
  float* lams = Us + NR * UP;
  float* Wsb = lams + 16 * ET_MAX;
  float* Ws = Wsb + h * (PP * DH * WP);
  float* YT = Wsb + 4 * PP * DH * WP;
  float* xss = YT + 16 * ET_MAX * YP;
  float* scr = xss + 2 * D;
  const float* U = a.u + (int64_t)b * a.N * a.K;
  const float* w = a.coeff + ((int64_t)h * a.B + b) * PP * DH * DH;

  PartialBatchT<32> pb;
  partials_request_t<256, 32>(c.y2_stats != nullptr ? c.y2_stats : c.w_cat, c.y2_stats != nullptr ? c.Gx : 0, D, pb);
  float4 xv[NT_MAX], yv[NT_MAX];
#pragma unroll
  for (int i = 0; i < NT_MAX; ++i) {
    const int idx = tid + 256 * i, node = idx >> 4, q = idx & 15;
    const float4 v = *reinterpret_cast<const float4*>(tok_row(a.x, a.xsb, a.xsn, b, min(node, nm1), 0, DH) + 4 * q);
    xv[i] = keep4(node < n, v);
    yv[i] = *reinterpret_cast<const float4*>(c.y2 + (int64_t)b * c.y2sb + (int64_t)min(node, Nm1) * c.y2sn + 4 * q);
  }
  constexpr int UQ = 4 * ET_MAX, UI = (NR * UQ + 255) / 256;
  float4 uv[UI];
#pragma unroll
  for (int i = 0; i < UI; ++i) {
    const int idx = tid + 256 * i, node = idx / UQ, e = 4 * (idx % UQ);
    const float4 v = *reinterpret_cast<const float4*>(U + (int64_t)min(node, nm1) * a.K + min(e, a.K - 4));
    uv[i] = keep4(node < n && e < a.K, v);
  }
  {
    float4 wv[PP];
#pragma unroll
    for (int i = 0; i < PP; ++i) wv[i] = reinterpret_cast<const float4*>(w)[lane + 64 * i];
#pragma unroll
    for (int i = 0; i < PP; ++i) {
      const int idx = lane + 64 * i;
      *reinterpret_cast<float4*>(Ws + (idx >> 2) * WP + 4 * (idx & 3)) = wv[i];
    }
  }
  Feat<D> waf, wbf;
  load_row<D>(waf, c.w_cat + (int64_t)(DH * h + lq) * 2 * D, g);
  load_row<D>(wbf, c.w_cat + (int64_t)(DH * h + lq) * 2 * D + D, g);
  const float bcat = c.b_cat != nullptr ? c.b_cat[DH * h + lq] : 0.0f;
  const float lv = a.lam[(int64_t)b * a.K + min(tid, a.K - 1)];
  const float bv = (a.bias != nullptr) ? a.bias[lq] : 0.0f;
  float4 bs4 = make_float4(0.0f, 0.0f, 0.0f, 0.0f);
  if (a.bias != nullptr) bs4 = *reinterpret_cast<const float4*>(a.bias + 4 * g);
  float xg = 1.0f, xb = 0.0f, xk = 0.0f;
  if (c.y2_stats != nullptr && tid < D) {
    xg = c.gamma[tid];
    xb = c.beta[tid];
    xk = partials_shift(c.y2_stats, c.Gx, D, tid);
  }
  if (c.y2_stats != nullptr) {
    reduce_partials_finish_t<256, 32>(c.y2_stats, c.Gx, D, pb, scr + 2 * D, scr);
    if (tid < D) {
      float mean, var;
      bn_moments_k(xk, D, c.M, scr, tid, mean, var);
      const float rstd = rsqrtf(var + c.eps);
      const float scale = xg * rstd, shift = xb - mean * scale;
      xss[tid] = scale;
      xss[D + tid] = shift;
      if (blockIdx.x == 0) {
        c.bn_out[tid] = scale;
        c.bn_out[D + tid] = shift;
        c.bn_out[2 * D + tid] = mean;
        c.bn_out[3 * D + tid] = rstd;
        if (c.rmean != nullptr) {
          const float unbiased = c.M > 1 ? var * (float)c.M / (float)(c.M - 1) : var;
          c.rmean[tid] = (1.0f - c.momentum) * c.rmean[tid] + c.momentum * mean;
          c.rvar[tid] = (1.0f - c.momentum) * c.rvar[tid] + c.momentum * unbiased;
        }
        if (tid == 0 && c.nbt != nullptr) *c.nbt += 1;
      }
    }
  } else if (tid < 2 * D) {
    xss[tid] = c.y2_bn != nullptr ? c.y2_bn[tid] : (tid < D ? 1.0f : 0.0f);
  }
// ... 24 lines not shown
      for (int r = 0; r < 4; ++r) {
        const int nd = 16 * nt + 4 * g + r;
        const float xa = Xs[nd * XP + DH * h + lq];
#pragma unroll
        for (int et = 0; et < ET_MAX; ++et) xtT[et] = mfma16(xa, Us[nd * UP + 16 * et + lq], xtT[et]);
      }
    }
  }
  f32x4 yt[ET_MAX];
#pragma unroll
  for (int et = 0; et < ET_MAX; ++et) {
    float tk[kMaxOrder];
    cheb_poly(lams[16 * et + lq], PP, tk);
    yt[et] = zero4();
#pragma unroll
    for (int k = 0; k < PP; ++k)
#pragma unroll
      for (int r = 0; r < 4; ++r)
        yt[et] = mfma16(xtT[et][r] * tk[k], Ws[(k * DH + 4 * g + r) * WP + lq], yt[et]);
#pragma unroll
    for (int r = 0; r < 4; ++r) YT[(16 * et + 4 * g + r) * YP + DH * h + lq] = yt[et][r];
  }
  __syncthreads();
  f32x4 ytp[ET_MAX];
#pragma unroll
  for (int et = 0; et < ET_MAX; ++et) {
    Feat<D> yf;
    load_row<D>(yf, YT + (16 * et + lq) * YP, g);
    ytp[et] = dot_rows<D>(yf, wbf, zero4());
  }
  float cbo = 0.0f;
#pragma unroll
  for (int j = 0; j < 4; ++j)
    cbo += (wbf.f[j][0] * bs4.x + wbf.f[j][1] * bs4.y) + (wbf.f[j][2] * bs4.z + wbf.f[j][3] * bs4.w);
  cbo += shfl_xor(cbo, 16);
  cbo += shfl_xor(cbo, 32);
  f32x4 y[NT_MAX], o[NT_MAX];
#pragma unroll
  for (int nt = 0; nt < NT_MAX; ++nt) {
    y[nt] = zero4();
    o[nt] = zero4();
    if (16 * nt < a.N) {
      Feat<D> xf;
      load_row<D>(xf, Ys + (16 * nt + lq) * XP, g);
      o[nt] = dot_rows<D>(xf, waf, zero4());
    }
    if (16 * nt < n) {
#pragma unroll
      for (int et = 0; et < ET_MAX; ++et) {
        const float4 ub = *reinterpret_cast<const float4*>(Us + (16 * nt + lq) * UP + 16 * et + 4 * g);
        y[nt] = mfma16(ub.x, yt[et][0], y[nt]);
        y[nt] = mfma16(ub.y, yt[et][1], y[nt]);
        y[nt] = mfma16(ub.z, yt[et][2], y[nt]);
        y[nt] = mfma16(ub.w, yt[et][3], y[nt]);
        o[nt] = mfma16(ub.x, ytp[et][0], o[nt]);
        o[nt] = mfma16(ub.y, ytp[et][1], o[nt]);
        o[nt] = mfma16(ub.z, ytp[et][2], o[nt]);
        o[nt] = mfma16(ub.w, ytp[et][3], o[nt]);
      }
    }
  }
  __syncthreads();
#pragma unroll
  for (int nt = 0; nt < NT_MAX; ++nt)
#pragma unroll
    for (int r = 0; r < 4; ++r) {
      const int nd = 16 * nt + 4 * g + r;
      Xs[nd * XP + DH * h + lq] = nd < n ? y[nt][r] + bv : 0.0f;
      Ys[nd * XP + DH * h + lq] = o[nt][r] + bcat + (nd < n ? cbo : 0.0f);
    }
  __syncthreads();
#pragma unroll
  for (int i = 0; i < NT_MAX; ++i) {
    const int idx = tid + 256 * i, node = idx >> 4, q = idx & 15;
    if (node < a.N) {
      *reinterpret_cast<float4*>(tok_row(a.y, a.ysb, a.ysn, b, node, 0, DH) + 4 * q) =
          *reinterpret_cast<const float4*>(Xs + node * XP + 4 * q);
      *reinterpret_cast<float4*>(tok_row(c.out, a.ysb, a.ysn, b, node, 0, DH) + 4 * q) =
          *reinterpret_cast<const float4*>(Ys + node * XP + 4 * q);
    }
  }
}

template <int NT_MAX, int ET_MAX>
int launch_spec_cat_fwd(const FilterArgs& a, const CatArgs& c, hipStream_t stream) {
  const size_t lds = sizeof(float) * spec_cat_fwd_lds_floats<NT_MAX, ET_MAX>(4);
  auto kern = spec_cat_fwd_graph_kernel<NT_MAX, ET_MAX, 4>;
  static LdsSeen lds_seen;
  allow_dynamic_lds(kern, lds, lds_seen);
  hipLaunchKernelGGL(kern, dim3(a.B), dim3(256), lds, stream, a, c);
  return check_launch("feta_spec_filter_cat_fwd");
}

constexpr int kCatBwdMaxGrid = 512;
inline int spec_cat_bwd_rows(int B) { return B < kCatBwdMaxGrid ? B : kCatBwdMaxGrid; }

struct CatGradArgs {
  const float* dout;
  const float* y2;
  int64_t y2sb, y2sn;
  const float* y2_bn;
  const float* filt;
  const float* w_cat;
  float* dxn;
  float* gs;
  float* partial;
  int64_t partial_ld;
};

template <int NT_MAX, int ET_MAX>
__host__ __device__ inline int spec_cat_bwd_lds_floats() {
  constexpr int NR = 16 * NT_MAX, UP = 16 * ET_MAX + 4;
  return 2 * NR * kGraphXP + NR * UP + 16 * ET_MAX + 16 * ET_MAX * (kCatD + 4) + 2 * kCatD;
}

template <int NT_MAX, int ET_MAX, int PP>
__global__ __launch_bounds__(256) void spec_cat_bwd_graph_kernel(FilterArgs a, CatGradArgs c) {
  constexpr int DH = 16, XP = kGraphXP, UP = 16 * ET_MAX + 4, NR = 16 * NT_MAX, D = kCatD, DP = D + 4;
  const int h = threadIdx.x >> 6, lane0 = threadIdx.x & 63;
  const int Nm1 = a.N - 1;
  const int col = DH * h + (lane0 & 15);
  float* Xs = feta_lds;
  float* Ds = Xs + NR * XP;
  float* Us = Ds + NR * XP;
  float* lams = Us + NR * UP;
  float* DT = lams + 16 * ET_MAX;
  float* SR = DT + 16 * ET_MAX * DP;
  float wa[16], wb[16];
#pragma unroll
  for (int j = 0; j < 4; ++j)
#pragma unroll
    for (int s_ = 0; s_ < 4; ++s_) {
      const float* row = c.w_cat + (int64_t)(16 * j + 4 * (lane0 >> 4) + s_) * 2 * D;
      wa[4 * j + s_] = row[col];
      wb[4 * j + s_] = row[D + col];
    }
  float bsc = 1.0f, bsh = 0.0f, bmean = 0.0f, brstd = 0.0f;
  if (c.y2_bn != nullptr) {
    bsc = c.y2_bn[col];
    bsh = c.y2_bn[D + col];
    bmean = c.y2_bn[2 * D + col];
    brstd = c.y2_bn[3 * D + col];
  }
  f32x4 gaw[4], gbw[4];
#pragma unroll
  for (int t = 0; t < 4; ++t) {
    gaw[t] = zero4();
    gbw[t] = zero4();
  }
  float sall_w = 0.0f, g1 = 0.0f, g2 = 0.0f;
  for (int b = blockIdx.x; b < a.B; b += gridDim.x) {
  if (b != (int)blockIdx.x) __syncthreads();
  int lane_l = lane0;
  FETA_OPAQUE_LANE(lane_l);
  const int lane = lane_l, tid = (h << 6) | lane, lq = lane & 15, g = lane >> 4;
  const int item = b * a.H + h;
  const int n = a.n_real[b], nm1 = max(n - 1, 0);
  const float* U = a.u + (int64_t)b * a.N * a.K;
  const int64_t blk = (int64_t)h * a.B + b;
  const float* w = a.coeff + blk * PP * DH * DH;
  float* dw = a.dcoeff + blk * PP * DH * DH;
  const int64_t rb = (int64_t)b * c.y2sb;

  float4 xv[NT_MAX], dv[NT_MAX];
#pragma unroll
  for (int i = 0; i < NT_MAX; ++i) {
    const int idx = tid + 256 * i, node = idx >> 4, q = idx & 15;
    const float4 v1 = *reinterpret_cast<const float4*>(tok_row(a.x, a.xsb, a.xsn, b, min(node, nm1), 0, DH) + 4 * q);
    const float4 v2 = *reinterpret_cast<const float4*>(c.dout + rb + (int64_t)min(node, Nm1) * c.y2sn + 4 * q);
    xv[i] = keep4(node < n, v1);
    dv[i] = keep4(node < a.N, v2);
  }
  constexpr int UQ = 4 * ET_MAX, UI = (NR * UQ + 255) / 256;
// ... 396 lines not shown
                                    const float* lam, const float* coeff, const float* bias,
                                    const int32_t* n_real, float* y, int64_t y_sb, int64_t y_sn,
                                    int B, int N, int H, int dh, int P, int K,
                                    int heads_share_graph, feta_stream_t stream) {
  FilterArgs a{};
  a.x = x; a.u = u; a.lam = lam; a.coeff = coeff; a.bias = bias; a.n_real = n_real; a.y = y;
  a.xsb = x_sb; a.xsn = x_sn; a.ysb = y_sb; a.ysn = y_sn;
  a.B = B; a.N = N; a.H = H; a.P = P; a.K = K; a.share = heads_share_graph; a.total = B * H;
  FETA_REQUIRE(x && u && lam && coeff && n_real && y, "spec_filter_fwd: null pointer");
  FETA_REQUIRE(K >= 1 && K <= FETA_MAX_NODES, "spec_filter_fwd: K=%d out of range", K);
  int rc = check_filter(a, dh, x, y);
  if (rc != FETA_OK) return rc;
  int rcd = FETA_OK;
  if (try_spec_dense(a, dh, false, (hipStream_t)stream, &rcd)) return rcd;
  return dispatch<SpecFwd>(a, dh, (K + 15) / 16, (hipStream_t)stream);
}

extern "C" int feta_spec_filter_bwd(const float* x, int64_t x_sb, int64_t x_sn, const float* u,
                                    const float* lam, const float* coeff, const int32_t* n_real,
                                    const float* dy, int64_t y_sb, int64_t y_sn, float* dx,
                                    float* dcoeff, float* dbias_part, int B, int N, int H, int dh,
                                    int P, int K, int heads_share_graph, feta_stream_t stream) {
  FilterArgs a{};
  a.x = x; a.u = u; a.lam = lam; a.coeff = coeff; a.n_real = n_real; a.dy = dy;
  a.dx = dx; a.dcoeff = dcoeff; a.dbias_part = dbias_part;
  a.xsb = x_sb; a.xsn = x_sn; a.ysb = y_sb; a.ysn = y_sn;
  a.B = B; a.N = N; a.H = H; a.P = P; a.K = K; a.share = heads_share_graph; a.total = B * H;
  FETA_REQUIRE(x && u && lam && coeff && n_real && dy && dx && dcoeff && dbias_part,
               "spec_filter_bwd: null pointer");
  FETA_REQUIRE(K >= 1 && K <= FETA_MAX_NODES, "spec_filter_bwd: K=%d out of range", K);
  int rc = check_filter(a, dh, x, dy);
  if (rc != FETA_OK) return rc;
  FETA_REQUIRE(aligned16(dx) && aligned16(dcoeff), "spec_filter_bwd: outputs must be 16-byte aligned");
  int rcd = FETA_OK;
  if (try_spec_dense(a, dh, true, (hipStream_t)stream, &rcd)) return rcd;
  return dispatch<SpecBwd>(a, dh, (K + 15) / 16, (hipStream_t)stream);
}

extern "C" int feta_spec_cat_supported(int N, int H, int dh, int P, int K, int heads_share_graph) {
  const int nt = (N + 15) / 16, et = (K + 15) / 16;
  return (heads_share_graph && H == 4 && dh == 16 && P == 4 && nt >= 1 && nt <= 8 && et <= 2 && (K & 3) == 0 && K >= 4) ? 1 : 0;
}

extern "C" int feta_spec_cat_bwd_supported(int N, int H, int dh, int P, int K, int heads_share_graph) {
  const int nt = (N + 15) / 16, et = (K + 15) / 16;
  return (heads_share_graph && H == 4 && dh == 16 && P == 4 && nt >= 1 && nt <= 4 && et <= 2 && (K & 3) == 0 && K >= 4) ? 1 : 0;
}

extern "C" int feta_spec_cat_bwd_rows(int B) { return B < 1 ? 0 : spec_cat_bwd_rows(B); }

extern "C" int feta_spec_filter_cat_bwd(const float* x, int64_t x_sb, int64_t x_sn, const float* u, const float* lam,
                                        const float* coeff, const int32_t* n_real, int64_t y_sb, int64_t y_sn, float* dx,
                                        float* dcoeff, float* dbias_part, int B, int N, int H, int dh, int P, int K,
                                        int heads_share_graph, const feta_spec_cat_grad* cat, feta_stream_t stream) {
  FilterArgs a{};
  a.x = x; a.u = u; a.lam = lam; a.coeff = coeff; a.n_real = n_real; a.dx = dx; a.dcoeff = dcoeff; a.dbias_part = dbias_part;
  a.xsb = x_sb; a.xsn = x_sn; a.ysb = y_sb; a.ysn = y_sn;
  a.B = B; a.N = N; a.H = H; a.P = P; a.K = K; a.share = heads_share_graph; a.total = B * H;
  FETA_REQUIRE(x && u && lam && coeff && n_real && dx && dcoeff && dbias_part && cat, "spec_filter_cat_bwd: null pointer");
  FETA_REQUIRE(feta_spec_cat_bwd_supported(N, H, dh, P, K, heads_share_graph),
               "spec_filter_cat_bwd: needs 4 heads x 16, order 4, N <= 64, K <= 32 (multiple of 4), every head on the graph");
  int rc = check_filter(a, dh, x, dx);
  if (rc != FETA_OK) return rc;
  FETA_REQUIRE(cat->dout && cat->y2 && cat->filt && cat->w_cat && cat->dxn && cat->partial,
               "spec_filter_cat_bwd: dout, y2, filt, w_cat, dxn, partial");
  FETA_REQUIRE(cat->partial_ld >= 64 * 128 + 64, "spec_filter_cat_bwd: partial_ld %lld < 64 * 128 + 64", (long long)cat->partial_ld);
  FETA_REQUIRE(!cat->gs || cat->y2_bn, "spec_filter_cat_bwd: gs (BatchNorm-backward sums) needs the published block y2_bn");
  FETA_REQUIRE(aligned16(u) && aligned16(cat->dout) && aligned16(cat->dxn) && aligned16(cat->filt) && (cat->y2_sb % 4) == 0 &&
                   (cat->y2_sn % 4) == 0 && (y_sb % 4) == 0 && (y_sn % 4) == 0,
               "spec_filter_cat_bwd: 16-byte aligned tensors, strides multiples of 4 elements");
  CatGradArgs c{};
  c.dout = cat->dout; c.y2 = cat->y2; c.y2sb = cat->y2_sb; c.y2sn = cat->y2_sn; c.y2_bn = cat->y2_bn; c.filt = cat->filt;
  c.w_cat = cat->w_cat; c.dxn = cat->dxn; c.gs = cat->gs; c.partial = cat->partial; c.partial_ld = cat->partial_ld;
  const int nt = (N + 15) / 16, et = (K + 15) / 16;
  hipStream_t st = (hipStream_t)stream;
  if (nt <= 3) return et <= 1 ? launch_spec_cat_bwd<3, 1>(a, c, st) : launch_spec_cat_bwd<3, 2>(a, c, st);
  return et <= 1 ? launch_spec_cat_bwd<4, 1>(a, c, st) : launch_spec_cat_bwd<4, 2>(a, c, st);
}

extern "C" int feta_spec_filter_cat_fwd(const float* x, int64_t x_sb, int64_t x_sn, const float* u, const float* lam,
                                        const float* coeff, const float* bias, const int32_t* n_real, float* y,
                                        int64_t y_sb, int64_t y_sn, int B, int N, int H, int dh, int P, int K,
                                        int heads_share_graph, const feta_spec_cat* cat, feta_stream_t stream) {
  FilterArgs a{};
  a.x = x; a.u = u; a.lam = lam; a.coeff = coeff; a.bias = bias; a.n_real = n_real; a.y = y;
  a.xsb = x_sb; a.xsn = x_sn; a.ysb = y_sb; a.ysn = y_sn;
  a.B = B; a.N = N; a.H = H; a.P = P; a.K = K; a.share = heads_share_graph; a.total = B * H;
  FETA_REQUIRE(x && u && lam && coeff && n_real && y && cat, "spec_filter_cat_fwd: null pointer");
  FETA_REQUIRE(feta_spec_cat_supported(N, H, dh, P, K, heads_share_graph),
               "spec_filter_cat_fwd: needs 4 heads x 16, order 4, N <= 128, K <= 32 (multiple of 4), every head on the graph");
  int rc = check_filter(a, dh, x, y);
  if (rc != FETA_OK) return rc;
  FETA_REQUIRE(cat->y2 && cat->w_cat && cat->out, "spec_filter_cat_fwd: y2, w_cat, out");
  FETA_REQUIRE(!(cat->y2_bn && cat->y2_stats), "spec_filter_cat_fwd: y2_bn and y2_stats exclude each other");
  FETA_REQUIRE(!cat->y2_stats || (cat->gamma && cat->beta && cat->bn_out && cat->Gx > 0 && cat->M > 0),
               "spec_filter_cat_fwd: y2_stats needs gamma, beta, bn_out, Gx, M");
  FETA_REQUIRE(aligned16(u) && aligned16(cat->y2) && aligned16(cat->w_cat) && aligned16(cat->out) && aligned16(cat->y2_stats) &&
                   aligned16(bias) && (cat->y2_sb % 4) == 0 && (cat->y2_sn % 4) == 0,
               "spec_filter_cat_fwd: 16-byte aligned tensors, strides multiples of 4 elements");
  CatArgs c{};
  c.y2 = cat->y2; c.y2sb = cat->y2_sb; c.y2sn = cat->y2_sn; c.y2_bn = cat->y2_bn; c.y2_stats = cat->y2_stats; c.Gx = cat->Gx;
  c.gamma = cat->gamma; c.beta = cat->beta; c.bn_out = cat->bn_out; c.rmean = cat->rmean; c.rvar = cat->rvar;
  c.nbt = cat->nbt; c.momentum = cat->momentum; c.eps = cat->eps; c.M = cat->M;
  c.w_cat = cat->w_cat; c.b_cat = cat->b_cat; c.out = cat->out;
  const int nt = (N + 15) / 16, et = (K + 15) / 16;
  hipStream_t st = (hipStream_t)stream;
  if (nt <= 3) return et <= 1 ? launch_spec_cat_fwd<3, 1>(a, c, st) : launch_spec_cat_fwd<3, 2>(a, c, st);
  if (nt <= 4) return et <= 1 ? launch_spec_cat_fwd<4, 1>(a, c, st) : launch_spec_cat_fwd<4, 2>(a, c, st);
  return et <= 1 ? launch_spec_cat_fwd<8, 1>(a, c, st) : launch_spec_cat_fwd<8, 2>(a, c, st);
}
```

### feta_tmlr_amd/functional.py

```python
import torch

from . import _lib


def _token_view(t, batch_first, heads):
    d = t.shape[-1]
    v = t.view(t.shape[0], t.shape[1], heads, d // heads)
    return v if batch_first else v.permute(1, 0, 2, 3)


def _dense_like(t, batch_first):
    if batch_first:
        return t.contiguous()
    return t.permute(1, 0, 2, 3).contiguous().permute(1, 0, 2, 3)


def _new_token(b, n, h, dh, batch_first, ref):
    if batch_first:
        return torch.empty((b, n, h, dh), dtype=ref.dtype, device=ref.device)
    return torch.empty((n, b, h, dh), dtype=ref.dtype, device=ref.device).permute(1, 0, 2, 3)


class AttentionCoreFn(torch.autograd.Function):

    @staticmethod
    def forward(ctx, qkv, pe, n_real, num_heads, need_attn, tie_qk, batch_first, drop=None, clamp5=False):
        abi, stream = _lib.backend(qkv, pe, n_real)
        ctx.set_materialize_grads(False)
        qkv = qkv.contiguous()
        l0, l1, d3 = qkv.shape
        d = d3 // 3
        dh = d // num_heads
        b, n = (l0, l1) if batch_first else (l1, l0)
        v5 = qkv.view(l0, l1, 3, num_heads, dh)
        sel = (lambda i: v5[:, :, i]) if batch_first else (lambda i: v5[:, :, i].permute(1, 0, 2, 3))
        q, k, v = sel(0), (sel(0) if tie_qk else sel(1)), sel(2)
        out = _new_token(b, n, num_heads, dh, batch_first, qkv)
        attn = torch.empty((b, num_heads, n, n), dtype=qkv.dtype, device=qkv.device) if need_attn else None
        stats = torch.empty((b, num_heads, n, 2), dtype=torch.float32, device=qkv.device)
        pe_c = None if pe is None else pe.to(qkv.dtype).contiguous()
        scale = float(dh) ** -0.5
        abi.attn_fwd(q, k, v, pe_c, n_real, out, attn, stats, scale, stream, drop=drop, clamp5=clamp5)
        ctx.clamp5 = bool(clamp5)
        ctx.save_for_backward(qkv, pe_c, n_real, out, stats)
        ctx.cfg = (num_heads, tie_qk, batch_first, scale)
        ctx.drop = drop
        concat = (out if batch_first else out.permute(1, 0, 2, 3)).reshape(l0, l1, d)
        if attn is not None:
            ctx.mark_non_differentiable(attn)
        return concat, attn

    @staticmethod
    def backward(ctx, dconcat, _dattn):
        qkv, pe_c, n_real, out, stats = ctx.saved_tensors
        if dconcat is None:
            return (None,) * 9
        num_heads, tie_qk, batch_first, scale = ctx.cfg
        abi, stream = _lib.backend(qkv)
        l0, l1, d3 = qkv.shape
        d = d3 // 3
        dh = d // num_heads
        b, n = (l0, l1) if batch_first else (l1, l0)
        v5 = qkv.view(l0, l1, 3, num_heads, dh)
        dqkv = torch.empty_like(qkv)
        g5 = dqkv.view(l0, l1, 3, num_heads, dh)
        if batch_first:
            sel, gsel = (lambda i: v5[:, :, i]), (lambda i: g5[:, :, i])
        else:
            sel = lambda i: v5[:, :, i].permute(1, 0, 2, 3)
            gsel = lambda i: g5[:, :, i].permute(1, 0, 2, 3)
        q, k, v = sel(0), (sel(0) if tie_qk else sel(1)), sel(2)
        dout = _token_view(dconcat.to(qkv.dtype).contiguous(), batch_first, num_heads)
        delta = torch.empty((b, num_heads, n), dtype=torch.float32, device=qkv.device)
        abi.attn_bwd(q, k, v, pe_c, n_real, out, dout, stats, delta, gsel(0), gsel(1), gsel(2),
                     scale, stream, drop=ctx.drop, clamp5=ctx.clamp5)
        if tie_qk:
            dqkv[..., :d] += dqkv[..., d:2 * d]
            dqkv[..., d:2 * d] = 0
        return dqkv, None, None, None, None, None, None, None, None


class FilterCoefficientsFn(torch.autograd.Function):

    @staticmethod
    def forward(ctx, attn, n_real, gcn_weight, gcn_bias, pending=None):
        abi, stream = _lib.backend(attn, gcn_weight)
        ctx.pending = pending
        ctx.params = (gcn_weight, gcn_bias)
        if pending is not None and (ctx.needs_input_grad[2] or ctx.needs_input_grad[3]):
            pending.coeff_armed = True
        attn = attn.contiguous()
        b, h, n, _ = attn.shape
        c = gcn_weight.shape[1]
        dev = attn.device
        if pending is not None and pending.s is not None:
            s = pending.s
            left = pending.take_fwd()
            if left:
                abi.colsum_multi(left, stream)
            pending.s = None
        else:
            s = torch.empty(c, dtype=torch.float32, device=dev)
            abi.colsum(gcn_weight.contiguous(), s, stream)
        gb = gcn_bias.contiguous()
        if pending is not None and pending.coeff_fwd_out is not None:
            cj, pooled = pending.coeff_fwd_out
            pending.coeff_fwd_out = None
        else:
            cj = torch.empty((h * b, n), dtype=torch.float32, device=dev)
            pooled = torch.empty((h * b, c), dtype=torch.float32, device=dev)
            abi.coeff_fwd(attn, n_real, s, gb, cj, pooled, stream)
        if pending is not None:
            pending.coeff_fwd_req = None
        ctx.save_for_backward(cj, n_real, s, gb)
        ctx.dims = (b, n, h, gcn_weight.shape[0])
        return pooled

    @staticmethod
    def backward(ctx, dpooled):
        cj, n_real, s, gb = ctx.saved_tensors
        b, n, h, rows = ctx.dims
        abi, stream = _lib.backend(cj)
        c = s.shape[0]
        groups = abi.coeff_bwd_groups(b, h)
        partial = torch.empty((groups, 2, c), dtype=torch.float32, device=cj.device)
        dsdb = torch.empty((2, c), dtype=torch.float32, device=cj.device)
        ds, db = dsdb[0], dsdb[1]
        dw = torch.empty((rows, c), dtype=torch.float32, device=cj.device)
        pend = ctx.pending
        if (pend is not None and pend.stack_armed and not pend.stack_done and PendingSums.untouched(*ctx.params)):
            pend.coeff_bwd_req = (cj, n_real, s, gb, dpooled.contiguous(), partial, b, n, h)
            p2 = partial.view(groups, 2 * c)
            pend.add(p2[:, :c], ds, dw, owners=[(ctx.params[0], dw)])
            pend.add(p2[:, c:], db, owners=[(ctx.params[1], db)])
            return None, None, dw, db, None
        waiting = pend.take() if pend is not None else []
        if waiting:
            abi.coeff_bwd(cj, n_real, s, gb, dpooled.contiguous(), partial, None, None, b, n, h, stream)
            p2 = partial.view(groups, 2 * c)
            abi.colsum_multi([(p2[:, :c], ds, dw), (p2[:, c:], db)] + waiting, stream)
        else:
            abi.coeff_bwd(cj, n_real, s, gb, dpooled.contiguous(), partial, ds, db, b, n, h, stream, dw_dense=dw)
        return None, None, dw, db, None


class DenseLinearFn(torch.autograd.Function):

    @staticmethod
    def forward(ctx, x, w, bias):
        ctx.save_for_backward(x, w)
        with _lib.tuned_gemm():
            return torch.addmm(bias, x, w.t())

    @staticmethod
    def backward(ctx, dy):
        x, w = ctx.saved_tensors
        abi, stream = _lib.backend(dy)
        dy = dy.contiguous()
        db = torch.empty(dy.shape[1], dtype=dy.dtype, device=dy.device)
        abi.colsum(dy, db, stream)
        with _lib.tuned_gemm():
            return dy.mm(w), dy.t().mm(x), db


def dense_linear(x, w, bias):
    return DenseLinearFn.apply(x, w, bias)


class _FilterFn(torch.autograd.Function):

    @staticmethod
    def forward(ctx, x, coeff, bias, n_real, g0, g1, mode, order, share, batch_first):
        abi, stream = _lib.backend(x, coeff)
        b, n, h, dh = x.shape
        xs = _dense_like(x, batch_first)
        coeff = coeff.contiguous()
        y = _new_token(b, n, h, dh, batch_first, x)
        if mode == 'cheb':
            abi.cheb_filter_fwd(xs, g0, coeff, bias, n_real, y, order, share, stream)
        else:
            abi.spec_filter_fwd(xs, g0, g1, coeff, bias, n_real, y, order, share, stream)
        ctx.save_for_backward(xs, coeff, n_real, g0, g1)
        ctx.cfg = (mode, order, share, batch_first, bias is not None)
        return y

    @staticmethod
    def backward(ctx, dy):
        xs, coeff, n_real, g0, g1 = ctx.saved_tensors
        mode, order, share, batch_first, has_bias = ctx.cfg
        abi, stream = _lib.backend(xs)
        b, n, h, dh = xs.shape
        dys = _dense_like(dy.to(xs.dtype), batch_first)
        dx = _new_token(b, n, h, dh, batch_first, xs)
        dcoeff = torch.empty_like(coeff)
        dbp = torch.empty((b * h, dh), dtype=torch.float32, device=xs.device)
        if mode == 'cheb':
            abi.cheb_filter_bwd(xs, g0, coeff, n_real, dys, dx, dcoeff, dbp, order, share, stream)
        else:
            abi.spec_filter_bwd(xs, g0, g1, coeff, n_real, dys, dx, dcoeff, dbp, order, share, stream)
        dbias = None
        if has_bias:
            dbias = torch.empty(dh, dtype=torch.float32, device=xs.device)
            abi.colsum(dbp, dbias, stream)
        return dx, dcoeff, dbias, None, None, None, None, None, None, None


import os as _os
LIN_OWN_GEMM_MAX_MACS = int(_os.environ.get('FETA_LIN_OWN_MAX_MACS', str(1 << 27)))
LIN_LIB_BF16_MIN_ROWS = int(_os.environ.get('FETA_LIN_LIB_BF16_MIN_ROWS', '2048'))


COEFF_ROLE_MAX_BLOCKS = int(_os.environ.get('FETA_COEFF_ROLE_MAX', 2048))


class PendingSums:

    def __init__(self):
        self.armed = False
        self.coeff_armed = False
        self.stack_armed = False
        self.stack_done = False
        self.items = []
        self.owners = []
        self._callback_queued = False
        self.fwd_sums = []
        self.s = None
        self.coeff_fwd_req = None
        self.coeff_fwd_out = None
        self.coeff_bwd_req = None

    @staticmethod
    def untouched(*params):
        if torch.is_grad_enabled() or torch.is_anomaly_enabled():
            return False
        for p in params:
            if p is None:
                continue
            if p.grad is not None or p._backward_hooks or getattr(p, '_post_accumulate_grad_hooks', None):
                return False
        return True

    def add(self, partial, out, bcast=None, owners=()):
        self.items.append((partial, out.detach(), None if bcast is None else bcast.detach()))
        for p, g in owners:
            if p is not None and g is not None:
                self.owners.append((p, g.detach()))
        if not self._callback_queued:
            torch.autograd.Variable._execution_engine.queue_callback(self._finish_pass)
            self._callback_queued = True

    def take(self):
        items, self.items = self.items, []
        return items

    def take_fwd(self):
        sums, self.fwd_sums = self.fwd_sums, []
        return sums

    def coeff_fwd_role(self, attn, n_real):
        if self.coeff_fwd_req is None or self.s is None or self.fwd_sums or attn is None:
            return None
        if attn.shape[-1] > 64:
            return None
        if attn.shape[0] * attn.shape[1] > COEFF_ROLE_MAX_BLOCKS:
            return None
        gcn_bias, self.coeff_fwd_req = self.coeff_fwd_req, None
        b, h, n, _ = attn.shape
        cj = torch.empty((h * b, n), dtype=torch.float32, device=attn.device)
        pooled = torch.empty((h * b, self.s.shape[0]), dtype=torch.float32, device=attn.device)
        self.coeff_fwd_out = (cj, pooled)
        return (attn, n_real, self.s, gcn_bias.detach().contiguous(), cj, pooled)

    def take_coeff_bwd(self):
        req, self.coeff_bwd_req = self.coeff_bwd_req, None
        return req

    def _finish_pass(self):
        self._callback_queued = False
        req = self.take_coeff_bwd()
        items = self.take()
        if items:
            abi, stream = _lib.backend(items[0][0])
            if req is not None:
                cj, n_real, s, gb, dpooled, partial, b, n, h = req
                abi.coeff_bwd(cj, n_real, s, gb, dpooled, partial, None, None, b, n, h, stream)
            abi.colsum_multi(items, stream)
        owners, self.owners = self.owners, []
        for p, g in owners:
            if p.grad is not None and p.grad.data_ptr() != g.data_ptr():
                with torch.no_grad():
                    p.grad.copy_(g.view_as(p.grad))


USE_CAT_FOLD = _os.environ.get('FETA_CAT_FOLD', '1') != '0'


class CatFold:

    def __init__(self, y2, w, bias, tail=None):
        self.y2, self.w, self.bias, self.tail = y2.detach(), w, bias, tail
        self.out = None
        self.y = None
        self.bwd_ok = False
        self.bwd = None

    def defer_backward(self, dy, y2, x2, w, prm, pending, owners_of, has_bias):
        if not (self.bwd_ok and USE_CAT_FOLD_BWD and pending is not None and self.bwd is None and self.y is not None):
            return None
        m, k1 = y2.shape
        ki, no = k1 + x2.shape[1], w.shape[0]
        nb = _lib.backend(y2)[0].spec_cat_bwd_rows(self.y.shape[0])
        dx1, dx2 = torch.empty_like(y2), torch.empty_like(x2)
        partial = torch.empty((nb, no * ki + no), dtype=torch.float32, device=y2.device)
        dwdb = torch.empty(no * ki + no, dtype=torch.float32, device=y2.device)
        gs = torch.empty((nb, 2, k1), dtype=torch.float32, device=y2.device) if prm is not None else None
        self.bwd = dict(dout=dy, dxn=dx1, partial=partial, gs=gs, prm=prm)
        pending.add(partial, dwdb, owners=[(owners_of[0], dwdb[:no * ki].view(no, ki)),
                                           (owners_of[1], dwdb[no * ki:] if has_bias else None)])
        return dx1, dx2, dwdb[:no * ki].view(no, ki), (dwdb[no * ki:] if has_bias else None), gs


USE_CAT_FOLD_BWD = _os.environ.get('FETA_CAT_FOLD_BWD', '1') != '0'


class FilterFromPooledFn(torch.autograd.Function):

    @staticmethod
    def forward(ctx, x, pooled, lin_w, lin_b, bias, n_real, g0, g1, mode, order, share, batch_first, pending,
                gemm_bf16=False, cat=None):
        abi, stream = _lib.backend(x, pooled)
        ctx.gemm_bf16 = bool(gemm_bf16)
        b, n, h, dh = x.shape
        xs = _dense_like(x, batch_first)
        pooled, lin_w = pooled.contiguous(), lin_w.contiguous()
        r_, k_, n_ = pooled.shape[0], pooled.shape[1], lin_w.shape[0]
        ctx.lib_bf16 = bool(ctx.gemm_bf16 and r_ >= LIN_LIB_BF16_MIN_ROWS and pooled.is_cuda)
        ctx.own_gemm = (not ctx.lib_bf16 and abi.lin_supported(r_, k_, n_)
                        and (r_ * k_ * n_ <= LIN_OWN_GEMM_MAX_MACS or ctx.gemm_bf16))
        ctx.lp = None
        if ctx.own_gemm:
            coeff = torch.empty((pooled.shape[0], lin_w.shape[0]), dtype=torch.float32, device=pooled.device)
            abi.lin_fwd(pooled, lin_w, lin_b, coeff, stream, bf16=ctx.gemm_bf16)
        elif ctx.lib_bf16:
            p16, w16 = pooled.to(torch.bfloat16), lin_w.to(torch.bfloat16)
            coeff = torch.mm(p16, w16.t(), out_dtype=torch.float32)
            if lin_b is not None:
                coeff += lin_b
            ctx.lp = (p16, w16)
        else:
            with _lib.tuned_gemm():
                coeff = torch.addmm(lin_b, pooled, lin_w.t())
        ctx.pending = pending
        ctx.defer = pending is not None and pending.coeff_armed and ctx.needs_input_grad[1] and not ctx.own_gemm
        ctx.params = (lin_b, bias)
        if pending is not None and any(ctx.needs_input_grad):
            pending.armed = True
        cw = coeff if x.dtype == torch.float32 else coeff.to(x.dtype)
        y = _new_token(b, n, h, dh, batch_first, x)
        fold = (cat is not None and USE_CAT_FOLD and mode == 'spec' and x.dtype == torch.float32 and not batch_first
                and cat.w.shape == (h * dh, 2 * h * dh) and abi.spec_cat_supported(n, h, dh, order, g0.shape[2], share))
        if fold:
            out = _new_token(b, n, h, dh, batch_first, x)
            y2v = cat.y2.detach().view(n, b, h, dh).permute(1, 0, 2, 3)
            kw = {}
            if cat.tail is not None:
                t, nm = cat.tail, cat.tail.norm
                kw = dict(y2_stats=t.st2, Gx=t.G2, gamma=t.gamma, beta=t.beta, bn_out=t.prm2, rmean=nm.running_mean,
                          rvar=nm.running_var, nbt=nm.num_batches_tracked, momentum=float(nm.momentum), eps=float(nm.eps))
            abi.spec_filter_cat_fwd(xs, g0, g1, cw, bias, n_real, y, order, share, stream, y2=y2v, w_cat=cat.w.detach().contiguous(),
                                    b_cat=None if cat.bias is None else cat.bias.detach(), out=out, **kw)
            cat.out = out.permute(1, 0, 2, 3).reshape(n * b, h * dh)
            cat.y = y.detach()
            cat.bwd_ok = bool(abi.spec_cat_bwd_supported(n, h, dh, order, g0.shape[2], share))
        elif mode == 'cheb':
            abi.cheb_filter_fwd(xs, g0, cw, bias, n_real, y, order, share, stream)
        else:
            abi.spec_filter_fwd(xs, g0, g1, cw, bias, n_real, y, order, share, stream)
        ctx.save_for_backward(xs, cw, pooled, lin_w, n_real, g0, g1)
        ctx.cfg = (mode, order, share, batch_first, bias is not None)
        ctx.cat = cat if fold else None
        ctx.set_materialize_grads(False)
        return y, coeff

    @staticmethod
    def backward(ctx, dy, dcoeff_ext):
        xs, coeff, pooled, lin_w, n_real, g0, g1 = ctx.saved_tensors
        mode, order, share, batch_first, has_bias = ctx.cfg
        abi, stream = _lib.backend(xs)
        b, n, h, dh = xs.shape
        waiting = ctx.pending.take() if ctx.pending is not None else []
        sums = []
        if dy is None:
            dx, dbias = None, None
            dcoeff = dcoeff_ext.contiguous()
            db_lin = torch.empty(dcoeff.shape[1], dtype=torch.float32, device=xs.device)
        else:
            st = None
            if ctx.cat is not None and ctx.cat.bwd is not None:
                st, ctx.cat.bwd = ctx.cat.bwd, None
            dx = _new_token(b, n, h, dh, batch_first, xs)
            dcoeff = torch.empty_like(coeff)
            dbp = torch.empty((b * h, dh), dtype=torch.float32, device=xs.device)
            if st is not None:
                cat = ctx.cat
                tv = lambda t: t.view(n, b, h, dh).permute(1, 0, 2, 3)
                abi.spec_filter_cat_bwd(xs, g0, g1, coeff, n_real, cat.y, dx, dcoeff, dbp, order, share, stream,
                                        dout=tv(st['dout']), y2=tv(cat.y2.detach()), w_cat=cat.w.detach().contiguous(),
                                        dxn=tv(st['dxn']), partial=st['partial'], y2_bn=st['prm'], gs=st['gs'])
            else:
                dys = _dense_like(dy.to(xs.dtype), batch_first)
            if st is not None:
                pass
            elif mode == 'cheb':
                abi.cheb_filter_bwd(xs, g0, coeff, n_real, dys, dx, dcoeff, dbp, order, share, stream)
            else:
                abi.spec_filter_bwd(xs, g0, g1, coeff, n_real, dys, dx, dcoeff, dbp, order, share, stream)
            if dcoeff.dtype != torch.float32:
                dcoeff = dcoeff.float()
            if dcoeff_ext is not None:
                dcoeff += dcoeff_ext
            both = torch.empty(dh + dcoeff.shape[1], dtype=torch.float32, device=xs.device)
            dbias, db_lin = both[:dh], both[dh:]
            sums.append((dbp, dbias))
        sums += waiting
        if ctx.own_gemm:
            dpooled = torch.empty_like(pooled) if ctx.needs_input_grad[1] else None
            dw_lin = torch.empty_like(lin_w)
            abi.lin_bwd(pooled, lin_w, dcoeff, dpooled, dw_lin, db_lin, stream, pairs=sums, bf16=ctx.gemm_bf16)
        else:
            sums.append((dcoeff, db_lin))
            if ctx.defer and PendingSums.untouched(*ctx.params):
                for pr in sums:
                    ctx.pending.add(*pr)
                ctx.pending.owners += [(p_, g_.detach()) for p_, g_ in ((ctx.params[0], db_lin), (ctx.params[1], dbias))
                                       if p_ is not None and g_ is not None]
            else:
                abi.colsum_multi(sums, stream)
            if ctx.lib_bf16:
                p16, w16 = ctx.lp
                d16 = dcoeff.to(torch.bfloat16)
                dpooled = torch.mm(d16, w16, out_dtype=torch.float32)
                dw_lin = torch.mm(d16.t(), p16, out_dtype=torch.float32)
            else:
                with _lib.tuned_gemm():
                    dpooled, dw_lin = dcoeff.mm(lin_w), dcoeff.t().mm(pooled)
        if not has_bias:
            dbias = None
        return (dx, dpooled, dw_lin, db_lin, dbias) + (None,) * 10


def filter_from_pooled(x, pooled, lin_w, lin_b, bias, n_real, graph, mode, order, heads_share_graph=False,
                       batch_first=False, pending=None, gemm_bf16=False, cat=None):
    g0 = graph[0].contiguous()
    g1 = graph[1].contiguous() if len(graph) > 1 else None
    if x.dtype != torch.float32:
        if mode != 'spec':
            raise NotImplementedError("the bf16 storage path runs the eigenbasis filter (filter_mode='spectral')")
        g0 = g0.to(x.dtype)
    return FilterFromPooledFn.apply(x, pooled, lin_w, lin_b, bias, n_real, g0, g1, mode, order,
                                    bool(heads_share_graph), batch_first, pending, bool(gemm_bf16), cat)
# ... 381 lines not shown
```

### feta_tmlr_amd/fused_stack.py

```python
import os
import weakref

import torch

from . import _lib


def _views(t, l0, l1, heads, dh):
    v5 = t.view(l0, l1, 3, heads, dh)
    return [v5[:, :, i].permute(1, 0, 2, 3) for i in range(3)]


PER_LAYER = 12
USE_ATTN_BLOCK = os.environ.get('FETA_ATTN_BLOCK', '1') != '0'
USE_FFN_FUSED = os.environ.get('FETA_FFN_FUSED', '1') != '0'
USE_ATTN_OUT = os.environ.get('FETA_ATTN_OUT', '1') != '0'
USE_LN_EPILOGUE = os.environ.get('FETA_LN_EPILOGUE', '1') != '0'
USE_FFN_BWD = os.environ.get('FETA_FFN_BWD', '1') != '0'
USE_ATTN_BLOCK_BWD = os.environ.get('FETA_ATTN_BLOCK_BWD', '1') != '0'
USE_ATTN_BLOCK_SPLIT = os.environ.get('FETA_ATTN_BLOCK_SPLIT', '1') != '0'
USE_ATTN_BLOCK_BWD_LOOP = os.environ.get('FETA_BLOCK_BWD_LOOP', '1') != '0'


def _fused_attn_bwd(abi, b, n, d, heads, tie, dt):
# ... 787 lines not shown
        ctx.mark_non_differentiable(attn)
    concat_last = (out32 if lowp else saved[-1]['out']).view(n, b, d)
    return final.view(n, b, d), concat_last, attn


def _ln_on_load_backward(ctx, d_final, d_concat_last):
    saved, params = ctx.saved_state, ctx.params
    n, b, d, heads, dh, tie, scale, nl = ctx.meta
    pe_c, degree_rows, n_real = ctx.aux
    abi, stream = _lib.backend(saved[0]['qkv'])
    m = n * b
    dev = saved[0]['qkv'].device
    dt = saved[0]['qkv'].dtype
    new = lambda *s: torch.empty(s, dtype=torch.float32, device=dev)
    newt = lambda *s: torch.empty(s, dtype=dt, device=dev)
    grads = [None] * len(params)
    ff0 = params[6].shape[0]
    part_f, part_a, tf, ta, wslot = _partial_buffers(abi, new, m, b, n, d, heads, ff0, nl, True, ln_cols=True, ffn_fused=True)
    coeff_req = _coeff_bwd_request(ctx, abi, stream, d, params[(nl - 1) * PER_LAYER + 6].shape[0])
    total = tf + ta
    dwdb_all = new(total)
    slots, ln_slots = {}, {}
    if d_final is None:
        d_final = torch.zeros(n, b, d, dtype=torch.float32, device=dev)
    if d_final.dtype != torch.float32:
        d_final = d_final.float()
    dcur, dcur_b = d_final.contiguous().view(m, d), None
    GB = abi.attn_block_bwd_blocks(b)
    for li in range(nl - 1, -1, -1):
        s = saved[li]
        (w_in, b_in, w_o, b_o, g1, be1, w1, bb1, w2, bb2, g2, be2) = params[li * PER_LAYER:(li + 1) * PER_LAYER]
        ff = w1.shape[0]
        base = li * PER_LAYER
        eps1, eps2 = ctx.eps[li]
        pp, off = wslot('f', d, ff)
        slots[base + 8] = (off, d, ff)
        _, off1 = wslot('f', ff, d)
        slots[base + 6] = (off1, ff, d)
        ln_slots[base + 10] = wslot.raw('f', 2 * d)
        dx1 = newt(m, d)
        abi.ffn_bwd(m, ff, stream, coeff=(coeff_req if li == nl - 1 else None), partial_ptr=pp, partial_ld=tf,
                    dy=dcur, dy_b=dcur_b, g_y=s['y2'], g_ln_gamma=g2, ln_eps=eps2, h=s['h'], w2=w2, w1=w1, x=s['y1'],
                    x_ln_gamma=g1, x_ln_beta=be1, dx=dx1)
        ppo, offo = wslot('a', d, d)
        slots[base + 2] = (offo, d, d)
        _, offi = wslot('a', 3 * d, d)
        slots[base + 0] = (offi, 3 * d, d)
        ln_slots[base + 4] = wslot.raw('a', 2 * d)
        d2 = d_concat_last if (li == nl - 1 and d_concat_last is not None) else None
        split = USE_ATTN_BLOCK_SPLIT and li > 0 and GB == b
        dx0 = newt(m, d)
        dx0b = newt(m, d) if split else None
        ln0 = {}
        if li > 0:
            ln0 = dict(x0_ln_gamma=params[(li - 1) * PER_LAYER + 10], x0_ln_beta=params[(li - 1) * PER_LAYER + 11])
        abi.attn_block_bwd(b, n, scale, stream, heads=heads, partial_ptr=ppo, partial_ld=ta, dy=dx1, y1=s['y1'], ln1_gamma=g1,
                           ln_eps=eps1, dx_b=dx0b, rowscale=degree_rows, w_out=w_o, w_in=w_in, qkv=s['qkv'], out=s['out'],
                           dout2=None if d2 is None else d2.contiguous().view(m, d), pe=pe_c, n_real=n_real,
                           attn_stats=s['ast'], x0=s['x0'], dx=dx0, **ln0)
        dcur, dcur_b = dx0, dx0b
    assert dcur_b is None
    assert wslot.cur == {'f': tf, 'a': ta}
    abi.colsum_multi([(part_f, dwdb_all[:tf]), (part_a, dwdb_all[tf:total])] + _take_pending(ctx), stream)
    if ctx.owner is not None:
        STACK_FLAT_GRAD[ctx.owner] = dwdb_all
    for idx, (off, no, ki) in slots.items():
        grads[idx] = dwdb_all[off:off + no * ki].view(no, ki)
        if params[idx + 1] is not None:
            grads[idx + 1] = dwdb_all[off + no * ki:off + no * ki + no]
    for idx, off in ln_slots.items():
        grads[idx], grads[idx + 1] = dwdb_all[off:off + d], dwdb_all[off + d:off + 2 * d]
    return (dcur.view(n, b, d), None, None, None, None, None, None, None) + tuple(grads)


def _coeff_fwd_role(pending, li, nl, attn, n_real):
    if pending is None or li != nl - 1:
        return None
    return pending.coeff_fwd_role(attn, n_real)


def _coeff_bwd_request(ctx, abi, stream, d, ff_last):
    from . import functional as F
    req = ctx.pending.take_coeff_bwd() if ctx.pending is not None else None
    if req is not None and (not (USE_FFN_BWD and abi.ffn_bwd_supported(d, ff_last))
                            or req[6] * req[8] > F.COEFF_ROLE_MAX_BLOCKS):
        cj, n_real, s, gb, dpooled, partial, b, n, h = req
        abi.coeff_bwd(cj, n_real, s, gb, dpooled, partial, None, None, b, n, h, stream)
        req = None
    return req


def _take_pending(ctx):
    pend = ctx.pending
    if pend is None:
        return []
    pend.stack_done = True
    return pend.take()


def fused_encoder_stack(src, pe, degree_rows, n_real, layers, need_attn=True, tail=None, pending=None, one_launch=None):
    params = []
    for l in layers:
        params += layer_params(l)
    bn = layers[0].batch_norm
    fn = FusedEncoderStackFn if bn else FusedLayerNormStackFn
    stack = StackLayers(layers)
    stack.one_launch = one_launch
    return fn.apply(src, pe, degree_rows, n_real, stack, need_attn, tail if bn else None, pending, *params)


def infer_supported(layers, n, d):
    if not len(layers):
        return False
    l0 = layers[0]
    bn, heads, ff, dt = l0.batch_norm, l0.self_attn.num_heads, l0.linear1.out_features, l0.storage_dtype
    if dt not in (torch.float32, torch.bfloat16):
        return False
    for l in layers:
        a = l.self_attn
        if l.batch_norm != bn or a.num_heads != heads or l.linear1.out_features != ff:
            return False
        if l.training and (l.dropout1.p > 0.0 or l.dropout.p > 0.0 or l.dropout2.p > 0.0 or a.dropout > 0.0):
            return False
        if getattr(a, 'stab', 'rowmax') != 'rowmax' or l.storage_dtype != dt:
            return False
        for nm in (l.norm1, l.norm2):
            if bn:
                if (not isinstance(nm, torch.nn.BatchNorm1d) or nm.training or nm.running_mean is None
                        or nm.running_var is None or nm.weight is None):
                    return False
            elif (not isinstance(nm, torch.nn.LayerNorm) or not nm.elementwise_affine or nm.bias is None
                  or tuple(nm.normalized_shape) != (d,)):
                return False
    abi = _lib._TEST_ABI if _lib._TEST_ABI is not None else _lib.abi()
    if dt == torch.float32:
        return abi.encoder_infer_supported(n, d, heads, ff, len(layers))
    return abi.encoder_infer_ex_supported(n, d, heads, ff, len(layers), dt)


def encoder_stack_infer(src, pe, degree_rows, n_real, layers, need_attn=True):
    n, b, d = src.shape
    abi, stream = _lib.backend(src)
    l0 = layers[0]
    heads, ff, bn = l0.self_attn.num_heads, l0.linear1.out_features, l0.batch_norm
    x = src.detach().contiguous()
    y = torch.empty(n, b, d, dtype=torch.float32, device=x.device)
    concat = torch.empty_like(y)
    attn = torch.empty(b, heads, n, n, dtype=torch.float32, device=x.device) if need_attn else None
    t = lambda p: None if p is None else p.detach().contiguous()
    table = []
    for l in layers:
        a = l.self_attn
        table.append(dict(
            w_in=t(a.in_proj_weight), b_in=t(a.in_proj_bias), w_out=t(a.out_proj.weight), b_out=t(a.out_proj.bias),
            n1_gamma=t(l.norm1.weight), n1_beta=t(l.norm1.bias),
            n1_mean=t(l.norm1.running_mean) if bn else None, n1_var=t(l.norm1.running_var) if bn else None,
            w1=t(l.linear1.weight), b1=t(l.linear1.bias), w2=t(l.linear2.weight), b2=t(l.linear2.bias),
            n2_gamma=t(l.norm2.weight), n2_beta=t(l.norm2.bias),
            n2_mean=t(l.norm2.running_mean) if bn else None, n2_var=t(l.norm2.running_var) if bn else None,
            n1_eps=l.norm1.eps, n2_eps=l.norm2.eps, tie_qk=int(a.tie_qk)))
    ptrs = dict(x=x, pe=t(pe), n_real=n_real.contiguous(), rowscale=t(degree_rows), y=y, out=concat, attn=attn)
    if l0.storage_dtype == torch.float32:
        abi.encoder_infer(b, n, heads, ff, table, not bn, stream, **ptrs)
    else:
        if ptrs['pe'] is not None and ptrs['pe'].dtype != x.dtype:
            ptrs['pe'] = ptrs['pe'].to(x.dtype)
        abi.encoder_infer_ex(b, n, heads, ff, table, not bn, stream, dtype=l0.storage_dtype, **ptrs)
    return y, concat, attn
# ... 1 lines not shown
```

### include/feta_hip.h

```cpp
#ifndef FETA_HIP_H_
#define FETA_HIP_H_

#include <stdint.h>

#ifdef __cplusplus
extern "C" {
#endif

#define FETA_ABI_VERSION 13

#define FETA_OK 0
#define FETA_E_ARG (-1)
#define FETA_E_LAUNCH (-2)

typedef void* feta_stream_t;

#define FETA_F32 0
#define FETA_BF16 1

int feta_version(void);
const char* feta_last_error(void);

#define FETA_MAX_NODES 256
#define FETA_MAX_HEAD_DIM 64

int feta_attn_fwd(const float* q, const float* k, const float* v,
                  int64_t qkv_sb, int64_t qkv_sn,
                  const float* pe, const int32_t* n_real,
                  float* out, int64_t o_sb, int64_t o_sn,
                  float* attn, float* stats, float scale,
                  int B, int N, int H, int dh, feta_stream_t stream);

int feta_attn_bwd(const float* q, const float* k, const float* v,
                  int64_t qkv_sb, int64_t qkv_sn,
                  const float* pe, const int32_t* n_real,
                  const float* out, const float* dout, const float* dout2, int64_t o_sb, int64_t o_sn,
                  const float* stats, float* delta,
                  float* dq, float* dk, float* dv, float scale,
                  int B, int N, int H, int dh, feta_stream_t stream);

int feta_coeff_fwd(const float* attn, const int32_t* n_real,
                   const float* s, const float* gcn_bias,
                   float* cj, float* pooled,
                   int B, int N, int H, int C, feta_stream_t stream);

int feta_coeff_bwd_groups(int B, int H);
int feta_coeff_bwd(const float* cj, const int32_t* n_real,
                   const float* s, const float* gcn_bias, const float* dpooled,
                   float* partial, float* ds, float* dbias, float* dw_dense, int dw_rows,
                   int B, int N, int H, int C, feta_stream_t stream);

int feta_colsum(const float* in, float* out, int R, int C, feta_stream_t stream);

#define FETA_COLSUM_MAX_SEGS 12
typedef struct feta_colsum_seg {
  const float* in;
  float* out;
  int R, C, ld;
  float* bcast_out;
  int bcast_rows;
} feta_colsum_seg;
int feta_colsum_multi(const feta_colsum_seg* segs, int nseg, feta_stream_t stream);

int feta_lin_supported(int R, int K, int N);
int feta_lin_fwd(const float* x, const float* w, const float* bias, float* y, int R, int K, int N,
                 feta_stream_t stream);
int feta_lin_bwd(const float* x, const float* w, const float* dy, float* dx, float* dw, float* db, int R, int K,
                 int N, const feta_colsum_seg* segs, int nseg, feta_stream_t stream);
int feta_lin_fwd_ex(const float* x, const float* w, const float* bias, float* y, int R, int K, int N, int compute,
                    feta_stream_t stream);
int feta_lin_bwd_ex(const float* x, const float* w, const float* dy, float* dx, float* dw, float* db, int R, int K,
                    int N, const feta_colsum_seg* segs, int nseg, int compute, feta_stream_t stream);

int feta_cheb_filter_fwd(const float* x, int64_t x_sb, int64_t x_sn,
                         const float* lhat, const float* coeff, const float* bias,
                         const int32_t* n_real,
                         float* y, int64_t y_sb, int64_t y_sn,
                         int B, int N, int H, int dh, int P, int heads_share_graph,
                         feta_stream_t stream);

int feta_cheb_filter_bwd(const float* x, int64_t x_sb, int64_t x_sn,
                         const float* lhat, const float* coeff, const int32_t* n_real,
                         const float* dy, int64_t y_sb, int64_t y_sn,
                         float* dx, float* dcoeff, float* dbias_part,
                         int B, int N, int H, int dh, int P, int heads_share_graph,
                         feta_stream_t stream);

int feta_spec_filter_fwd(const float* x, int64_t x_sb, int64_t x_sn,
                         const float* u, const float* lam,
                         const float* coeff, const float* bias, const int32_t* n_real,
                         float* y, int64_t y_sb, int64_t y_sn,
                         int B, int N, int H, int dh, int P, int K, int heads_share_graph,
                         feta_stream_t stream);

int feta_spec_filter_bwd(const float* x, int64_t x_sb, int64_t x_sn,
                         const float* u, const float* lam,
                         const float* coeff, const int32_t* n_real,
                         const float* dy, int64_t y_sb, int64_t y_sn,
                         float* dx, float* dcoeff, float* dbias_part,
                         int B, int N, int H, int dh, int P, int K, int heads_share_graph,
                         feta_stream_t stream);

typedef struct feta_spec_cat {
  const float* y2;
  int64_t y2_sb, y2_sn;
  const float* y2_bn;
  const float* y2_stats;
  int Gx;
  const float* gamma;
  const float* beta;
  float* bn_out;
  float* rmean;
  float* rvar;
  int64_t* nbt;
  float momentum, eps;
  int M;
  const float* w_cat;
  const float* b_cat;
  float* out;
} feta_spec_cat;
int feta_spec_cat_supported(int N, int H, int dh, int P, int K, int heads_share_graph);
int feta_spec_filter_cat_fwd(const float* x, int64_t x_sb, int64_t x_sn, const float* u, const float* lam,
                             const float* coeff, const float* bias, const int32_t* n_real, float* y,
                             int64_t y_sb, int64_t y_sn, int B, int N, int H, int dh, int P, int K,
                             int heads_share_graph, const feta_spec_cat* cat, feta_stream_t stream);

typedef struct feta_spec_cat_grad {
  const float* dout;
  const float* y2;
  int64_t y2_sb, y2_sn;
  const float* y2_bn;
  const float* filt;
  const float* w_cat;
  float* dxn;
  float* gs;
  float* partial;
  int64_t partial_ld;
} feta_spec_cat_grad;
int feta_spec_cat_bwd_supported(int N, int H, int dh, int P, int K, int heads_share_graph);
int feta_spec_cat_bwd_rows(int B);
int feta_spec_filter_cat_bwd(const float* x, int64_t x_sb, int64_t x_sn, const float* u, const float* lam,
                             const float* coeff, const int32_t* n_real, int64_t y_sb, int64_t y_sn, float* dx,
                             float* dcoeff, float* dbias_part, int B, int N, int H, int dh, int P, int K,
                             int heads_share_graph, const feta_spec_cat_grad* cat, feta_stream_t stream);

int feta_attn_fwd_bf16(const void* q, const void* k, const void* v, int64_t qkv_sb, int64_t qkv_sn,
                       const void* pe, const int32_t* n_real, void* out, int64_t o_sb, int64_t o_sn,
                       void* attn, float* stats, float scale, int B, int N, int H, int dh,
                       feta_stream_t stream);
int feta_attn_bwd_bf16(const void* q, const void* k, const void* v, int64_t qkv_sb, int64_t qkv_sn,
                       const void* pe, const int32_t* n_real, const void* out, const void* dout,
                       int64_t o_sb, int64_t o_sn, const float* stats, float* delta,
                       void* dq, void* dk, void* dv, float scale, int B, int N, int H, int dh,
                       feta_stream_t stream);
int feta_spec_filter_fwd_bf16(const void* x, int64_t x_sb, int64_t x_sn, const void* u, const float* lam,
                              const void* coeff, const float* bias, const int32_t* n_real,
                              void* y, int64_t y_sb, int64_t y_sn,
                              int B, int N, int H, int dh, int P, int K, int heads_share_graph,
                              feta_stream_t stream);
int feta_spec_filter_bwd_bf16(const void* x, int64_t x_sb, int64_t x_sn, const void* u, const float* lam,
                              const void* coeff, const int32_t* n_real,
                              const void* dy, int64_t y_sb, int64_t y_sn,
                              void* dx, void* dcoeff, float* dbias_part,
                              int B, int N, int H, int dh, int P, int K, int heads_share_graph,
                              feta_stream_t stream);

#define FETA_DTYPE_F32 0
#define FETA_DTYPE_BF16 1
int feta_attn_fwd_drop(const void* q, const void* k, const void* v, int64_t qkv_sb, int64_t qkv_sn,
                       const void* pe, const int32_t* n_real, void* out, int64_t o_sb, int64_t o_sn,
                       void* attn, float* stats, float scale, float p_drop, uint64_t seed, uint64_t offset,
                       int dtype, int B, int N, int H, int dh, feta_stream_t stream);
int feta_attn_bwd_drop(const void* q, const void* k, const void* v, int64_t qkv_sb, int64_t qkv_sn,
                       const void* pe, const int32_t* n_real, const void* out, const void* dout,
                       int64_t o_sb, int64_t o_sn, const float* stats, float* delta,
                       void* dq, void* dk, void* dv, float scale, float p_drop, uint64_t seed, uint64_t offset,
                       int dtype, int B, int N, int H, int dh, feta_stream_t stream);
int feta_attn_fwd_drop_dev(const void* q, const void* k, const void* v, int64_t qkv_sb, int64_t qkv_sn,
                           const void* pe, const int32_t* n_real, void* out, int64_t o_sb, int64_t o_sn,
                           void* attn, float* stats, float scale, float p_drop, const uint64_t* state,
                           uint64_t offset_add, int dtype, int B, int N, int H, int dh, feta_stream_t stream);
int feta_attn_bwd_drop_dev(const void* q, const void* k, const void* v, int64_t qkv_sb, int64_t qkv_sn,
                           const void* pe, const int32_t* n_real, const void* out, const void* dout,
                           int64_t o_sb, int64_t o_sn, const float* stats, float* delta,
                           void* dq, void* dk, void* dv, float scale, float p_drop, const uint64_t* state,
                           uint64_t offset_add, int dtype, int B, int N, int H, int dh, feta_stream_t stream);

#define FETA_STAB_ROWMAX 0
#define FETA_STAB_CLAMP5 1
int feta_attn_fwd_stab(const void* q, const void* k, const void* v, int64_t qkv_sb, int64_t qkv_sn,
                       const void* pe, const int32_t* n_real, void* out, int64_t o_sb, int64_t o_sn,
                       void* attn, float* stats, float scale, int stab, int dtype, int B, int N, int H, int dh,
                       feta_stream_t stream);
int feta_attn_bwd_stab(const void* q, const void* k, const void* v, int64_t qkv_sb, int64_t qkv_sn,
                       const void* pe, const int32_t* n_real, const void* out, const void* dout,
                       int64_t o_sb, int64_t o_sn, const float* stats, float* delta,
                       void* dq, void* dk, void* dv, float scale, int stab, int dtype, int B, int N, int H, int dh,
                       feta_stream_t stream);

int feta_rowlin_blocks(int M);
int feta_rowlin_chunks(int M);
int feta_rowlin_fwd(const float* x, const float* w, const float* bias, const float* rowscale,
                    const float* residual, float* y, float* stats, int relu,
                    int M, int KI, int NO, feta_stream_t stream);
int feta_rowlin_bwd(const float* x, const float* w, const float* dy, const float* rowscale,
                    const float* ysaved, float* dx, float* partial, float* dwdb,
                    int M, int KI, int NO, feta_stream_t stream);

// ... 151 lines not shown
int feta_attn_block_bwd_blocks(int B);
int feta_attn_block_bwd(const feta_attn_block_grad* d, feta_stream_t stream);
int feta_attn_block_bwd_sums(const feta_attn_block_grad* d, const feta_colsum_seg* segs, int nseg, feta_stream_t stream);

typedef struct feta_ffn {
  const float* x;
  const float* x_bn;
  const float* x_stats;
  int Gx;
  const float* x_gamma;
  const float* x_beta;
  float* x_bn_out;
  float* x_rmean;
  float* x_rvar;
  int64_t* x_nbt;
  float momentum, eps;
  const float* w1;
  const float* b1;
  const float* w2;
  const float* b2;
  float* h;
  float* y;
  float* y_stats;
  int M, FF;
  int dtype;
  const float* y_shift;
  int y_f32;
  const float* x_ln_gamma;
  const float* x_ln_beta;
  float* y_ln_out;
  const float* y_ln_gamma;
  const float* y_ln_beta;
  float y_ln_eps;
  int y_ln_f32;
} feta_ffn;

int feta_ffn_supported(int d_model, int ff);
int feta_ffn_blocks(int M);
int feta_ffn_fwd(const feta_ffn* d, feta_stream_t stream);
typedef struct feta_coeff_fwd_role {
  const float* attn; const int32_t* n_real; const float* s; const float* gcn_bias; float* cj; float* pooled;
  int B, N, H, C;
} feta_coeff_fwd_role;
int feta_ffn_fwd_coeff(const feta_ffn* d, const feta_coeff_fwd_role* c, feta_stream_t stream);

typedef struct feta_ffn_grad {
  const float* dy;
  const float* dy_b;
  const float* g_y;
  const float* g_bn;
  const float* g_sum;
  int Gs;
  const float* g_fin;
  float* g_fin_out;
  float* dgamma;
  float* dbeta;
  const float* h;
  const float* w2;
  const float* w1;
  const float* x;
  const float* x_bn;
  float* dx;
  float* sum_out;
  float* partial;
  int partial_ld;
  int M, FF;
  int dtype;
  int g_f32;
  const float* g_ln_gamma;
  const float* x_ln_gamma;
  const float* x_ln_beta;
  float ln_eps;
} feta_ffn_grad;

int feta_ffn_bwd_supported(int d_model, int ff);
int feta_ffn_bwd_blocks(int M);
int feta_ffn_bwd_chunks(int M, int ff);
int feta_ffn_bwd(const feta_ffn_grad* d, feta_stream_t stream);
typedef struct feta_coeff_bwd_role {
  const float* cj; const int32_t* n_real; const float* s; const float* gcn_bias; const float* dpooled; float* partial;
  int B, N, H, C;
} feta_coeff_bwd_role;
int feta_ffn_bwd_coeff(const feta_ffn_grad* d, const feta_coeff_bwd_role* c, feta_stream_t stream);

#define FETA_ENCODER_MAX_LAYERS 16
#define FETA_NORM_BATCH 0
#define FETA_NORM_LAYER 1
typedef struct feta_encoder_layer {
  const float* w_in;
  const float* b_in;
  const float* w_out;
  const float* b_out;
  const float* n1_gamma;
  const float* n1_beta;
  const float* n1_mean;
  const float* n1_var;
  const float* w1;
  const float* b1;
  const float* w2;
  const float* b2;
  const float* n2_gamma;
  const float* n2_beta;
  const float* n2_mean;
  const float* n2_var;
  float n1_eps, n2_eps;
  int tie_qk;
} feta_encoder_layer;

struct feta_encoder_infer {
  const float* x;
  int64_t row_sb, row_sn;
  const float* pe;
  const int32_t* n_real;
  const float* rowscale;
  float* y;
  float* out;
  float* attn;
  int B, N, H, FF, L;
  int norm;
  const feta_encoder_layer* layers;
};

int feta_encoder_infer_supported(int N, int d_model, int heads, int ff, int L);
int feta_encoder_infer(const struct feta_encoder_infer* d, feta_stream_t stream);

struct feta_encoder_infer_ex {
  const void* x;
  int64_t row_sb, row_sn;
  const void* pe;
  const int32_t* n_real;
  const float* rowscale;
  float* y;
  float* out;
  float* attn;
  int B, N, H, FF, L;
  int norm;
  const feta_encoder_layer* layers;
  int dtype;
  int in_dtype;
};

int feta_encoder_infer_ex_supported(int N, int d_model, int heads, int ff, int L, int dtype);
int feta_encoder_infer_ex(const struct feta_encoder_infer_ex* d, feta_stream_t stream);

struct feta_encoder_fwd_save {
  const void* x;
  int64_t row_sb, row_sn;
  const void* pe;
  const int32_t* n_real;
  const float* rowscale;
  float* y;
  float* out;
  float* attn;
  int B, N, H, FF, L;
  int norm;
  const feta_encoder_layer* layers;
  int dtype;
  int in_dtype;
  void* qkv;
  void* out_save;
  float* attn_stats;
  void* y1;
  void* h;
  void* y2;
  float* y2_last_f32;
  int64_t qkv_stride, out_stride, attn_stats_stride, y1_stride, h_stride, y2_stride;
// ... 44 lines not shown
```

Measured before the change: 496,600 graphs/s.

## Precompute coefficient-generator tanh-derivative sums in forward, reuse in backward

The backward of the coefficient generator's pooled tanh is factored. Per-(graph,head) sums of (1-tanh^2)*cj and (1-tanh^2) are computed once in forward, folded into the spectral-filter cat kernel as an extra block role. Backward then only needs a cheap dot product of dpooled with these saved sums, not re-evaluating tanh over all nodes. This trades extra forward work and two extra B*H x C buffers for a lighter backward, with the saved-path role kept out of the FFN backward's lead blocks by default.

```diff
diff --git a/feta_tmlr_amd/_abi.py b/feta_tmlr_amd/_abi.py
--- a/feta_tmlr_amd/_abi.py
+++ b/feta_tmlr_amd/_abi.py
@@ -17,6 +17,9 @@
                       C.c_int),
     'feta_coeff_fwd': ([_F, _I, _F, _F, _F, _F, C.c_int, C.c_int, C.c_int, C.c_int, _S], C.c_int),
     'feta_coeff_bwd_groups': ([C.c_int, C.c_int], C.c_int),
+    'feta_coeff_dsum': ([_F, _I, _F, _F, _F, _F, C.c_int, C.c_int, C.c_int, C.c_int, _S], C.c_int),
+    'feta_coeff_bwd_saved_groups': ([C.c_int, C.c_int], C.c_int),
+    'feta_coeff_bwd_saved': ([_F, _F, _F, _F, _F, _F, _F, C.c_int, C.c_int, C.c_int, C.c_int, _S], C.c_int),
     'feta_coeff_bwd': ([_F, _I, _F, _F, _F, _F, _F, _F, _F, C.c_int, C.c_int, C.c_int, C.c_int, C.c_int, _S],
                        C.c_int),
     'feta_colsum': ([_F, _F, C.c_int, C.c_int, _S], C.c_int),
@@ -138,7 +141,16 @@
     ]
 
 
+class CoeffDsumRole(C.Structure):
+    _fields_ = [('cj', _F), ('n_real', _I), ('s', _F), ('gcn_bias', _F), ('A', _F), ('Bm', _F),
+                ('B', C.c_int), ('N', C.c_int), ('H', C.c_int), ('C', C.c_int)]
+
+
 SIGNATURES.update({
+    'feta_spec_cat_fwd_coeff_fits': ([C.c_int] * 4, C.c_int),
+    'feta_spec_filter_cat_fwd_coeff': ([_F, C.c_int64, C.c_int64, _F, _F, _F, _F, _I, _F, C.c_int64, C.c_int64,
+                                        C.c_int, C.c_int, C.c_int, C.c_int, C.c_int, C.c_int, C.c_int, C.POINTER(SpecCat),
+                                        C.POINTER(CoeffDsumRole), _S], C.c_int),
     'feta_spec_cat_bwd_supported': ([C.c_int] * 6, C.c_int),
     'feta_spec_cat_bwd_rows': ([C.c_int], C.c_int),
     'feta_spec_filter_cat_bwd': ([_F, C.c_int64, C.c_int64, _F, _F, _F, _I, C.c_int64, C.c_int64, _F, _F, _F,
@@ -186,6 +198,20 @@
                 ('B', C.c_int), ('N', C.c_int), ('H', C.c_int), ('C', C.c_int)]
 
 
+class CoeffSavedReq:
+    __slots__ = ('dpooled', 'A', 'Bm', 'partial', 'b', 'h')
+
+    def __init__(self, dpooled, A, Bm, partial, b, h):
+        self.dpooled, self.A, self.Bm, self.partial, self.b, self.h = dpooled, A, Bm, partial, b, h
+
+    def run(self, abi, stream):
+        abi.coeff_bwd_saved(self.dpooled, self.A, self.Bm, self.partial, None, None, self.b, self.h, stream)
+
+
+class CoeffBwdSavedRole(C.Structure):
+    _fields_ = [('dpooled', _F), ('A', _F), ('Bm', _F), ('partial', _F), ('B', C.c_int), ('H', C.c_int), ('C', C.c_int)]
+
+
 class Ffn(C.Structure):
     _fields_ = [
         ('x', _F), ('x_bn', _F), ('x_stats', _F), ('Gx', C.c_int),
@@ -239,6 +265,7 @@
     'feta_ffn_bwd_chunks': ([C.c_int, C.c_int], C.c_int),
     'feta_ffn_bwd': ([C.POINTER(FfnGrad), _S], C.c_int),
     'feta_ffn_bwd_coeff': ([C.POINTER(FfnGrad), C.POINTER(CoeffBwdRole), _S], C.c_int),
+    'feta_ffn_bwd_coeff_saved': ([C.POINTER(FfnGrad), C.POINTER(CoeffBwdSavedRole), _S], C.c_int),
 })
 
 class EncoderLayer(C.Structure):
@@ -449,6 +476,18 @@
                                             0 if dw_dense is None else dw_dense.shape[0], b, n, h, c, stream),
                     'feta_coeff_bwd')
 
+    def coeff_dsum(self, cj, n_real, s, gcn_bias, A, Bm, b, n, h, stream):
+        self._check(self.lib.feta_coeff_dsum(_p(cj), _p(n_real), _p(s), _p(gcn_bias), _p(A), _p(Bm), b, n, h, s.shape[0],
+                                             stream), 'feta_coeff_dsum')
+
+    def coeff_bwd_saved_groups(self, b, h):
+        return self.lib.feta_coeff_bwd_saved_groups(b, h)
+
+    def coeff_bwd_saved(self, dpooled, A, Bm, partial, ds, dbias, b, h, stream, dw_dense=None):
+        self._check(self.lib.feta_coeff_bwd_saved(_p(dpooled), _p(A), _p(Bm), _p(partial), _p(ds), _p(dbias), _p(dw_dense),
+                                                  0 if dw_dense is None else dw_dense.shape[0], b, h, dpooled.shape[1], stream),
+                    'feta_coeff_bwd_saved')
+
     @staticmethod
     def _colsum_segs(pairs):
         segs = (ColsumSeg * max(len(pairs), 1))()
@@ -515,9 +554,12 @@
     def spec_cat_supported(self, n, h, dh, order, k, share):
         return bool(self.lib.feta_spec_cat_supported(n, h, dh, order, k, int(share)))
 
+    def spec_cat_fwd_coeff_fits(self, b, n, k, blocks):
+        return bool(self.lib.feta_spec_cat_fwd_coeff_fits(b, n, k, blocks))
+
     def spec_filter_cat_fwd(self, x, u, lam, coeff, bias, n_real, y, order, share, stream, y2, w_cat, b_cat, out,
                             y2_bn=None, y2_stats=None, Gx=0, gamma=None, beta=None, bn_out=None, rmean=None, rvar=None,
-                            nbt=None, momentum=0.1, eps=1e-5):
+                            nbt=None, momentum=0.1, eps=1e-5, dsum=None):
         b, n, h, dh = x.shape
         k = u.shape[2]
         xsb, xsn = tok_strides(x)
@@ -531,6 +573,15 @@
                         ('b_cat', b_cat), ('out', out)):
             if t is not None:
                 setattr(c, name, t.data_ptr())
+        if dsum is not None:
+            r = CoeffDsumRole()
+            r.cj, r.n_real, r.s, r.gcn_bias, r.A, r.Bm = (None if t is None else t.data_ptr() for t in dsum[:6])
+            r.B, r.N, r.H, r.C = dsum[6], dsum[7], dsum[8], dsum[2].shape[0]
+            self._check(self.lib.feta_spec_filter_cat_fwd_coeff(_p(x), xsb, xsn, _p(u), _p(lam), _p(coeff), _p(bias),
+                                                                _p(n_real), _p(y), ysb, ysn, b, n, h, dh, order, k, int(share),
+                                                                C.byref(c), C.byref(r), stream),
+                        'feta_spec_filter_cat_fwd_coeff')
+            return
         self._check(self.lib.feta_spec_filter_cat_fwd(_p(x), xsb, xsn, _p(u), _p(lam), _p(coeff), _p(bias), _p(n_real), _p(y),
                                                       ysb, ysn, b, n, h, dh, order, k, int(share), C.byref(c), stream),
                     'feta_spec_filter_cat_fwd')
@@ -757,6 +808,12 @@
     def ffn_bwd_launch(self, desc, stream, coeff=None):
         if coeff is None:
             self._check(self.lib.feta_ffn_bwd(C.byref(desc), stream), 'feta_ffn_bwd')
+            return
+        if isinstance(coeff, CoeffSavedReq):
+            r = CoeffBwdSavedRole()
+            r.dpooled, r.A, r.Bm, r.partial = (t.data_ptr() for t in (coeff.dpooled, coeff.A, coeff.Bm, coeff.partial))
+            r.B, r.H, r.C = coeff.b, coeff.h, coeff.A.shape[1]
+            self._check(self.lib.feta_ffn_bwd_coeff_saved(C.byref(desc), C.byref(r), stream), 'feta_ffn_bwd_coeff_saved')
             return
         cj, n_real, s, gcn_bias, dpooled, partial, b, n, h = coeff
         r = CoeffBwdRole()
diff --git a/feta_tmlr_amd/csrc/coeff.hip b/feta_tmlr_amd/csrc/coeff.hip
--- a/feta_tmlr_amd/csrc/coeff.hip
+++ b/feta_tmlr_amd/csrc/coeff.hip
@@ -29,6 +29,18 @@
     const float* __restrict__ gbias, const float* __restrict__ dpooled, float* __restrict__ partial,
     int B, int N, int H, int C, int G) {
   coeff_bwd_body(cj, n_real, s, gbias, dpooled, partial, B, N, H, C, G, (int)blockIdx.x, (int)blockIdx.y);
+}
+
+__global__ __launch_bounds__(kCoeffThreads) void coeff_dsum_kernel(
+    const float* __restrict__ cj, const int32_t* __restrict__ n_real, const float* __restrict__ s,
+    const float* __restrict__ gbias, float* __restrict__ A, float* __restrict__ Bm, int B, int N, int C) {
+  coeff_dsum_body(cj, n_real, s, gbias, A, Bm, B, N, C, (int)blockIdx.x);
+}
+
+__global__ __launch_bounds__(kCoeffThreads) void coeff_bwd_saved_kernel(
+    const float* __restrict__ dpooled, const float* __restrict__ A, const float* __restrict__ Bm,
+    float* __restrict__ partial, int total, int C, int G) {
+  coeff_bwd_saved_body(dpooled, A, Bm, partial, total, C, G, (int)blockIdx.x, (int)blockIdx.y);
 }
 
 constexpr int kCsCols = 16, kCsSlices = 64;
@@ -268,6 +280,40 @@
   return launch_colsum_strided(partial + C, dbias, G, C, 2 * C, (hipStream_t)stream);
 }
 
+extern "C" int feta_coeff_dsum(const float* cj, const int32_t* n_real, const float* s, const float* gcn_bias, float* A,
+                               float* Bm, int B, int N, int H, int C, feta_stream_t stream) {
+  FETA_REQUIRE(cj && n_real && s && gcn_bias && A && Bm, "coeff_dsum: null pointer");
+  FETA_REQUIRE(B > 0 && H > 0 && C > 0 && N > 0, "coeff_dsum: empty shape");
+  auto kern = coeff_dsum_kernel;
+  hipLaunchKernelGGL(kern, dim3(B * H), dim3(kCoeffThreads), N * sizeof(float), (hipStream_t)stream, cj, n_real, s,
+                     gcn_bias, A, Bm, B, N, C);
+  return check_launch("feta_coeff_dsum");
+}
+
+extern "C" int feta_coeff_bwd_saved_groups(int B, int H) { return (B < 1 || H < 1) ? 0 : coeff_bwd_saved_groups(B * H); }
+
+extern "C" int feta_coeff_bwd_saved(const float* dpooled, const float* A, const float* Bm, float* partial, float* ds,
+                                    float* dbias, float* dw_dense, int dw_rows, int B, int H, int C,
+                                    feta_stream_t stream) {
+  FETA_REQUIRE(dpooled && A && Bm && partial && (ds == nullptr || dbias != nullptr), "coeff_bwd_saved: null pointer");
+  FETA_REQUIRE(B > 0 && H > 0 && C > 0, "coeff_bwd_saved: empty shape");
+  const int G = coeff_bwd_saved_groups(B * H);
+  const dim3 grid((C + kCoeffThreads - 1) / kCoeffThreads, G), block(kCoeffThreads);
+  auto kern = coeff_bwd_saved_kernel;
+  hipLaunchKernelGGL(kern, grid, block, 0, (hipStream_t)stream, dpooled, A, Bm, partial, B * H, C, G);
+  int rc = check_launch("feta_coeff_bwd_saved");
+  if (rc != FETA_OK || ds == nullptr) return rc;
+  if (dw_dense != nullptr) {
+    FETA_REQUIRE(dw_rows > 0, "coeff_bwd_saved: dw_dense needs dw_rows");
+    feta_colsum_seg segs[2] = {{partial, ds, G, C, 2 * C, dw_dense, dw_rows}, {partial + C, dbias, G, C, 2 * C, nullptr, 0}};
+    return launch_colsum_multi(segs, 2, (hipStream_t)stream);
+  }
+  if (dbias == ds + C) return launch_colsum(partial, ds, G, 2 * C, (hipStream_t)stream);
+  rc = launch_colsum_strided(partial, ds, G, C, 2 * C, (hipStream_t)stream);
+  if (rc != FETA_OK) return rc;
+  return launch_colsum_strided(partial + C, dbias, G, C, 2 * C, (hipStream_t)stream);
+}
+
 extern "C" int feta_colsum(const float* in, float* out, int R, int C, feta_stream_t stream) {
   FETA_REQUIRE(in && out && R > 0 && C > 0, "colsum: bad arguments");
   return launch_colsum(in, out, R, C, (hipStream_t)stream);
diff --git a/feta_tmlr_amd/csrc/feta_coeff.h b/feta_tmlr_amd/csrc/feta_coeff.h
--- a/feta_tmlr_amd/csrc/feta_coeff.h
+++ b/feta_tmlr_amd/csrc/feta_coeff.h
@@ -295,6 +295,80 @@
 }
 
 
+__device__ __forceinline__ void coeff_dsum_body(
+    const float* __restrict__ cj, const int32_t* __restrict__ n_real, const float* __restrict__ s,
+    const float* __restrict__ gbias, float* __restrict__ A, float* __restrict__ Bm, int B, int N, int C, int blk) {
+  float* cjs = feta_lds;
+  const int n = min(n_real[blk % B], N);
+  __syncthreads();
+  for (int i = threadIdx.x; i < N; i += kCoeffThreads) cjs[i] = cj[(int64_t)blk * N + i];
+  __syncthreads();
+  const float inv_n = n > 0 ? 1.0f / (float)n : 0.0f;
+  for (int c0 = threadIdx.x; c0 < C; c0 += 4 * kCoeffThreads) {
+    float sc[4], bc[4], as[4], ab[4];
+#pragma unroll
+    for (int k = 0; k < 4; ++k) {
+      const int c = min(c0 + k * kCoeffThreads, C - 1);
+      sc[k] = s[c];
+      bc[k] = gbias[c];
+      as[k] = ab[k] = 0.0f;
+    }
+#pragma unroll 2
+    for (int i = 0; i < n; ++i) {
+      const float ci = cjs[i];
+#pragma unroll
+      for (int k = 0; k < 4; ++k) {
+        const float z = fast_tanh(ci * sc[k] + bc[k]);
+        const float t = 1.0f - z * z;
+        as[k] += t * ci;
+        ab[k] += t;
+      }
+    }
+#pragma unroll
+    for (int k = 0; k < 4; ++k) {
+      const int c = c0 + k * kCoeffThreads;
+      if (c < C) {
+        A[(int64_t)blk * C + c] = as[k] * inv_n;
+        Bm[(int64_t)blk * C + c] = ab[k] * inv_n;
+      }
+    }
+  }
+}
+
+__host__ __device__ inline int coeff_bwd_saved_groups(int total) {
+  const int g = total / 64 > 8 ? total / 64 : 8;
+  return total < g ? total : g;
+}
+
+constexpr int kCoeffSavedPass = 8;
+__device__ __forceinline__ void coeff_bwd_saved_body(
+    const float* __restrict__ dpooled, const float* __restrict__ A, const float* __restrict__ Bm,
+    float* __restrict__ partial, int total, int C, int G, int bx, int grp) {
+  const int c = bx * kCoeffThreads + threadIdx.x;
+  const int cc = c < C ? c : C - 1;
+  float as = 0.0f, ab = 0.0f;
+  for (int blk0 = grp; blk0 < total; blk0 += G * kCoeffSavedPass) {
+    float dp[kCoeffSavedPass], av[kCoeffSavedPass], bv[kCoeffSavedPass];
+#pragma unroll
+    for (int u = 0; u < kCoeffSavedPass; ++u) {
+      const int blk = blk0 + u * G;
+      const int64_t o = (int64_t)(blk < total ? blk : total - 1) * C + cc;
+      dp[u] = blk < total ? dpooled[o] : 0.0f;
+      av[u] = blk < total ? A[o] : 0.0f;
+      bv[u] = blk < total ? Bm[o] : 0.0f;
+    }
+#pragma unroll
+    for (int u = 0; u < kCoeffSavedPass; ++u) {
+      as += dp[u] * av[u];
+      ab += dp[u] * bv[u];
+    }
+  }
+  if (c < C) {
+    partial[(int64_t)grp * 2 * C + c] = as;
+    partial[(int64_t)grp * 2 * C + C + c] = ab;
+  }
+}
+
 __host__ __device__ inline int coeff_fwd_stage(int N) {
   if (N <= 64) return 1;
   return N * ((N + 3) & ~3) <= kCoeffLdsTileMax ? 2 : 0;
@@ -311,6 +385,11 @@
 struct CoeffBwdRole {
   const float* cj; const int32_t* n_real; const float* s; const float* gbias; const float* dpooled; float* partial;
   int B, N, H, C, G;
+  const float* A; const float* Bm;
 };
-
-}
+struct CoeffDsumRole {
+  const float* cj; const int32_t* n_real; const float* s; const float* gbias; float* A; float* Bm;
+  int B, N, H, C;
+};
+
+}
diff --git a/feta_tmlr_amd/csrc/ffn_bwd.hip b/feta_tmlr_amd/csrc/ffn_bwd.hip
--- a/feta_tmlr_amd/csrc/ffn_bwd.hip
+++ b/feta_tmlr_amd/csrc/ffn_bwd.hip
@@ -64,8 +64,12 @@
   if (bid < ge.role_lead || bid >= ge.role_lead + ge.main_grid) {
     const int r = bid < ge.role_lead ? bid : bid - ge.main_grid;
     const int nbx = (cb.C + kCoeffThreads - 1) / kCoeffThreads;
-    if (r < ge.role)
-      coeff_bwd_body(cb.cj, cb.n_real, cb.s, cb.gbias, cb.dpooled, cb.partial, cb.B, cb.N, cb.H, cb.C, cb.G, r % nbx, r / nbx);
+    if (r < ge.role) {
+      if (cb.A != nullptr)
+        coeff_bwd_saved_body(cb.dpooled, cb.A, cb.Bm, cb.partial, cb.B * cb.H, cb.C, cb.G, r % nbx, r / nbx);
+      else
+        coeff_bwd_body(cb.cj, cb.n_real, cb.s, cb.gbias, cb.dpooled, cb.partial, cb.B, cb.N, cb.H, cb.C, cb.G, r % nbx, r / nbx);
+    }
     return;
   }
   bid -= ge.role_lead;
@@ -503,8 +507,9 @@
   ge.per = (nrb16 + ge.RC - 1) / ge.RC;
   ge.NS = FF / kFbSlice;
   size_t lds = ffn_bwd_lds_bytes<T>(FF, a.g_bn != nullptr);
-  const int role = cb.cj != nullptr ? ((cb.C + kCoeffThreads - 1) / kCoeffThreads) * cb.G : 0;
-  if (role > 0 && sizeof(float) * (size_t)(kCoeffPass * cb.N) > lds) lds = sizeof(float) * (size_t)(kCoeffPass * cb.N);
+  const bool saved = cb.A != nullptr;
+  const int role = (cb.cj != nullptr || saved) ? ((cb.C + kCoeffThreads - 1) / kCoeffThreads) * cb.G : 0;
+  if (role > 0 && !saved && sizeof(float) * (size_t)(kCoeffPass * cb.N) > lds) lds = sizeof(float) * (size_t)(kCoeffPass * cb.N);
   auto kern = ffn_bwd_kernel<T, FF>;
   static LdsSeen seen;
   allow_dynamic_lds(kern, lds, seen);
@@ -525,6 +530,10 @@
   ge.role = role;
   ge.role_lead = 8 * ((role + 7) / 8);
   if (const char* e = getenv("FETA_COEFF_ROLE_FIRST")) if (atoi(e) == 0) ge.role_lead = 0;
+  if (saved) {
+    const char* e = getenv("FETA_COEFF_SAVED_LEAD");
+    if (e == nullptr || atoi(e) == 0) ge.role_lead = 0;
+  }
   hipLaunchKernelGGL(kern, dim3(grid + (ge.role_lead > 0 ? ge.role_lead : role)), dim3(kRowThreads), lds, stream, a, ge, cb);
   return check_launch("feta_ffn_bwd");
 }
@@ -537,6 +546,8 @@
 
 extern "C" int feta_ffn_bwd_blocks(int M) { return ffn_bwd_xblocks(M); }
 extern "C" int feta_ffn_bwd_chunks(int M, int ff) { return (M < 1 || !feta_ffn_bwd_supported(kFbD, ff)) ? 0 : ffn_bwd_chunks_for(M, ff); }
+
+static int ffn_bwd_checked(const feta_ffn_grad* d, const CoeffBwdRole& cb, feta_stream_t stream);
 
 extern "C" int feta_ffn_bwd(const feta_ffn_grad* d, feta_stream_t stream) { return feta_ffn_bwd_coeff(d, nullptr, stream); }
 
@@ -547,8 +558,22 @@
     FETA_REQUIRE(c->cj && c->n_real && c->s && c->gcn_bias && c->dpooled && c->partial, "ffn_bwd_coeff: null pointer");
     FETA_REQUIRE(c->B > 0 && c->H > 0 && c->C > 0 && c->N > 0, "ffn_bwd_coeff: empty shape");
     cb = CoeffBwdRole{c->cj, c->n_real, c->s, c->gcn_bias, c->dpooled, c->partial, c->B, c->N, c->H, c->C,
-                      feta_coeff_bwd_groups(c->B, c->H)};
-  }
+                      feta_coeff_bwd_groups(c->B, c->H), nullptr, nullptr};
+  }
+  return ffn_bwd_checked(d, cb, stream);
+}
+
+extern "C" int feta_ffn_bwd_coeff_saved(const feta_ffn_grad* d, const feta_coeff_bwd_saved_role* c, feta_stream_t stream) {
+  FETA_REQUIRE(d != nullptr && c != nullptr, "ffn_bwd_coeff_saved: null descriptor");
+  FETA_REQUIRE(c->dpooled && c->A && c->Bm && c->partial, "ffn_bwd_coeff_saved: null pointer");
+  FETA_REQUIRE(c->B > 0 && c->H > 0 && c->C > 0, "ffn_bwd_coeff_saved: empty shape");
+  CoeffBwdRole cb{};
+  cb.dpooled = c->dpooled; cb.partial = c->partial; cb.A = c->A; cb.Bm = c->Bm;
+  cb.B = c->B; cb.H = c->H; cb.C = c->C; cb.G = coeff_bwd_saved_groups(c->B * c->H);
+  return ffn_bwd_checked(d, cb, stream);
+}
+
+static int ffn_bwd_checked(const feta_ffn_grad* d, const CoeffBwdRole& cb, feta_stream_t stream) {
   const FfnGradArgs& a = *d;
   FETA_REQUIRE(a.dy && a.h && a.w2 && a.w1 && a.x && a.dx && a.partial && a.M > 0, "ffn_bwd: null pointer / empty");
   FETA_REQUIRE(feta_ffn_bwd_supported(kFbD, a.FF), "ffn_bwd: dim_feedforward %d not in {64,128}", a.FF);
diff --git a/feta_tmlr_amd/csrc/filter.hip b/feta_tmlr_amd/csrc/filter.hip
--- a/feta_tmlr_amd/csrc/filter.hip
+++ b/feta_tmlr_amd/csrc/filter.hip
@@ -1,4 +1,7 @@
+#include <cstdlib>
+
 #include "feta_abi_common.h"
+#include "feta_coeff.h"
 #include "feta_rowops.h"
 #include "feta_tiles.h"
 
@@ -1298,8 +1301,19 @@
          reduce_scratch_floats(kCatD, 256);
 }
 
-template <int NT_MAX, int ET_MAX, int PP>
-__global__ __launch_bounds__(256) void spec_cat_fwd_graph_kernel(FilterArgs a, CatArgs c) {
+template <bool ROLE> struct CoeffDsumHost {};
+template <> struct CoeffDsumHost<true> { CoeffDsumRole r; int grid; };
+
+template <int NT_MAX, int ET_MAX, int PP, bool ROLE = false>
+__global__ __launch_bounds__(256) void spec_cat_fwd_graph_kernel(FilterArgs a, CatArgs c, CoeffDsumHost<ROLE> cr) {
+  if constexpr (ROLE) {
+    if ((int)blockIdx.x >= a.B) {
+      const int total = cr.r.B * cr.r.H;
+      for (int blk = (int)blockIdx.x - a.B; blk < total; blk += cr.grid)
+        coeff_dsum_body(cr.r.cj, cr.r.n_real, cr.r.s, cr.r.gbias, cr.r.A, cr.r.Bm, cr.r.B, cr.r.N, cr.r.C, blk);
+      return;
+    }
+  }
   constexpr int DH = 16, XP = kGraphXP, UP = 16 * ET_MAX + 4, WP = kGraphWP, NR = 16 * NT_MAX, D = kCatD, YP = D + 4;
   const int tid = threadIdx.x, lane = tid & 63, h = tid >> 6, lq = lane & 15, g = lane >> 4;
   const int b = blockIdx.x;
@@ -1490,13 +1504,53 @@
   }
 }
 
+constexpr int kCatRoleWalkMax = 2;
 template <int NT_MAX, int ET_MAX>
-int launch_spec_cat_fwd(const FilterArgs& a, const CatArgs& c, hipStream_t stream) {
-  const size_t lds = sizeof(float) * spec_cat_fwd_lds_floats<NT_MAX, ET_MAX>(4);
-  auto kern = spec_cat_fwd_graph_kernel<NT_MAX, ET_MAX, 4>;
+int spec_cat_fwd_slots() {
+  static int slots = 0;
+  if (slots == 0) {
+    const size_t lds = sizeof(float) * spec_cat_fwd_lds_floats<NT_MAX, ET_MAX>(4);
+    auto kern = spec_cat_fwd_graph_kernel<NT_MAX, ET_MAX, 4, true>;
+    static LdsSeen lds_seen;
+    allow_dynamic_lds(kern, lds, lds_seen);
+    int dev = 0, cus = 0, per = 0;
+    if (hipGetDevice(&dev) != hipSuccess || hipDeviceGetAttribute(&cus, hipDeviceAttributeMultiprocessorCount, dev) != hipSuccess ||
+        hipOccupancyMaxActiveBlocksPerMultiprocessor(&per, kern, 256, lds) != hipSuccess || cus < 1 || per < 1) {
+      (void)hipGetLastError();
+      return 0;
+    }
+    slots = cus * per;
+  }
+  return slots;
+}
+inline int spec_cat_fwd_role_grid(int slots, int B, int total) {
+  if (const char* e = getenv("FETA_COEFF_DSUM_WGS")) if (atoi(e) > 0) return atoi(e) < total ? atoi(e) : total;
+  if (slots < 1) return 0;
+  const int free_slots = slots - B % slots;
+  const int grid = total < free_slots ? total : free_slots;
+  return (total + grid - 1) / grid <= kCatRoleWalkMax ? grid : 0;
+}
+
+template <int NT_MAX, int ET_MAX>
+int launch_spec_cat_fwd(const FilterArgs& a, const CatArgs& c, const CoeffDsumRole* cr, hipStream_t stream) {
+  size_t lds = sizeof(float) * spec_cat_fwd_lds_floats<NT_MAX, ET_MAX>(4);
+  if constexpr (NT_MAX <= 4) {
+    if (cr != nullptr) {
+      if (sizeof(float) * (size_t)cr->N > lds) lds = sizeof(float) * (size_t)cr->N;
+      const int role = spec_cat_fwd_role_grid(spec_cat_fwd_slots<NT_MAX, ET_MAX>(), a.B, cr->B * cr->H);
+      FETA_REQUIRE(role > 0, "spec_filter_cat_fwd_coeff: %d blocks do not fit the slots %d graphs leave free (feta_spec_cat_fwd_coeff_fits)",
+                   cr->B * cr->H, a.B);
+      auto kern = spec_cat_fwd_graph_kernel<NT_MAX, ET_MAX, 4, true>;
+      static LdsSeen lds_seen;
+      allow_dynamic_lds(kern, lds, lds_seen);
+      hipLaunchKernelGGL(kern, dim3(a.B + role), dim3(256), lds, stream, a, c, CoeffDsumHost<true>{*cr, role});
+      return check_launch("feta_spec_filter_cat_fwd_coeff");
+    }
+  }
+  auto kern = spec_cat_fwd_graph_kernel<NT_MAX, ET_MAX, 4, false>;
   static LdsSeen lds_seen;
   allow_dynamic_lds(kern, lds, lds_seen);
-  hipLaunchKernelGGL(kern, dim3(a.B), dim3(256), lds, stream, a, c);
+  hipLaunchKernelGGL(kern, dim3(a.B), dim3(256), lds, stream, a, c, CoeffDsumHost<false>{});
   return check_launch("feta_spec_filter_cat_fwd");
 }
 
@@ -2059,6 +2113,33 @@
                                         const float* coeff, const float* bias, const int32_t* n_real, float* y,
                                         int64_t y_sb, int64_t y_sn, int B, int N, int H, int dh, int P, int K,
                                         int heads_share_graph, const feta_spec_cat* cat, feta_stream_t stream) {
+  return feta_spec_filter_cat_fwd_coeff(x, x_sb, x_sn, u, lam, coeff, bias, n_real, y, y_sb, y_sn, B, N, H, dh, P, K,
+                                        heads_share_graph, cat, nullptr, stream);
+}
+
+extern "C" int feta_spec_cat_fwd_coeff_fits(int B, int N, int K, int blocks) {
+  const int nt = (N + 15) / 16, et = (K + 15) / 16;
+  if (B < 1 || blocks < 1 || nt < 1 || nt > 4 || et < 1 || et > 2) return 0;
+  const int slots = nt <= 3 ? (et <= 1 ? spec_cat_fwd_slots<3, 1>() : spec_cat_fwd_slots<3, 2>())
+                            : (et <= 1 ? spec_cat_fwd_slots<4, 1>() : spec_cat_fwd_slots<4, 2>());
+  return spec_cat_fwd_role_grid(slots, B, blocks) > 0 ? 1 : 0;
+}
+
+extern "C" int feta_spec_filter_cat_fwd_coeff(const float* x, int64_t x_sb, int64_t x_sn, const float* u, const float* lam,
+                                              const float* coeff, const float* bias, const int32_t* n_real, float* y,
+                                              int64_t y_sb, int64_t y_sn, int B, int N, int H, int dh, int P, int K,
+                                              int heads_share_graph, const feta_spec_cat* cat,
+                                              const feta_coeff_dsum_role* role, feta_stream_t stream) {
+  CoeffDsumRole crv{};
+  const CoeffDsumRole* cr = nullptr;
+  if (role != nullptr) {
+    FETA_REQUIRE(role->cj && role->n_real && role->s && role->gcn_bias && role->A && role->Bm,
+                 "spec_filter_cat_fwd_coeff: null pointer");
+    FETA_REQUIRE(role->B > 0 && role->H > 0 && role->C > 0 && role->N > 0 && role->N <= 64,
+                 "spec_filter_cat_fwd_coeff: need 0 < N <= 64 (got %d)", role->N);
+    crv = CoeffDsumRole{role->cj, role->n_real, role->s, role->gcn_bias, role->A, role->Bm, role->B, role->N, role->H, role->C};
+    cr = &crv;
+  }
   FilterArgs a{};
   a.x = x; a.u = u; a.lam = lam; a.coeff = coeff; a.bias = bias; a.n_real = n_real; a.y = y;
   a.xsb = x_sb; a.xsn = x_sn; a.ysb = y_sb; a.ysn = y_sn;
@@ -2082,7 +2163,8 @@
   c.w_cat = cat->w_cat; c.b_cat = cat->b_cat; c.out = cat->out;
   const int nt = (N + 15) / 16, et = (K + 15) / 16;
   hipStream_t st = (hipStream_t)stream;
-  if (nt <= 3) return et <= 1 ? launch_spec_cat_fwd<3, 1>(a, c, st) : launch_spec_cat_fwd<3, 2>(a, c, st);
-  if (nt <= 4) return et <= 1 ? launch_spec_cat_fwd<4, 1>(a, c, st) : launch_spec_cat_fwd<4, 2>(a, c, st);
-  return et <= 1 ? launch_spec_cat_fwd<8, 1>(a, c, st) : launch_spec_cat_fwd<8, 2>(a, c, st);
-}
+  if (nt <= 3) return et <= 1 ? launch_spec_cat_fwd<3, 1>(a, c, cr, st) : launch_spec_cat_fwd<3, 2>(a, c, cr, st);
+  if (nt <= 4) return et <= 1 ? launch_spec_cat_fwd<4, 1>(a, c, cr, st) : launch_spec_cat_fwd<4, 2>(a, c, cr, st);
+  FETA_REQUIRE(cr == nullptr, "spec_filter_cat_fwd_coeff: the role needs N <= 64 in the filter launch too");
+  return et <= 1 ? launch_spec_cat_fwd<8, 1>(a, c, nullptr, st) : launch_spec_cat_fwd<8, 2>(a, c, nullptr, st);
+}
diff --git a/feta_tmlr_amd/functional.py b/feta_tmlr_amd/functional.py
--- a/feta_tmlr_amd/functional.py
+++ b/feta_tmlr_amd/functional.py
@@ -1,6 +1,7 @@
 import torch
 
 from . import _lib
+from ._abi import CoeffSavedReq
 
 
 def _token_view(t, batch_first, heads):
@@ -112,6 +113,9 @@
             abi.coeff_fwd(attn, n_real, s, gb, cj, pooled, stream)
         if pending is not None:
             pending.coeff_fwd_req = None
+            pending.coeff_dsum_req = pending.coeff_dsum_out = None
+            if USE_COEFF_DSUM and pending.coeff_armed and n <= 64 and h * b <= COEFF_ROLE_MAX_BLOCKS:
+                pending.coeff_dsum_req = (cj.detach(), n_real, s.detach(), gb.detach(), b, n, h)
         ctx.save_for_backward(cj, n_real, s, gb)
         ctx.dims = (b, n, h, gcn_weight.shape[0])
         return pooled
@@ -122,12 +126,37 @@
         b, n, h, rows = ctx.dims
         abi, stream = _lib.backend(cj)
         c = s.shape[0]
-        groups = abi.coeff_bwd_groups(b, h)
-        partial = torch.empty((groups, 2, c), dtype=torch.float32, device=cj.device)
         dsdb = torch.empty((2, c), dtype=torch.float32, device=cj.device)
         ds, db = dsdb[0], dsdb[1]
         dw = torch.empty((rows, c), dtype=torch.float32, device=cj.device)
         pend = ctx.pending
+        saved = None
+        if pend is not None:
+            saved, pend.coeff_dsum_out = pend.coeff_dsum_out, None
+            pend.coeff_dsum_req = None
+        if saved is not None and torch.is_grad_enabled():
+            saved = None
+        if saved is not None:
+            A, Bm = saved
+            sg = abi.coeff_bwd_saved_groups(b, h)
+            partial = torch.empty((sg, 2, c), dtype=torch.float32, device=cj.device)
+            dpc = dpooled.contiguous()
+            if (pend.stack_armed and not pend.stack_done and PendingSums.untouched(*ctx.params)):
+                pend.coeff_bwd_req = CoeffSavedReq(dpc, A, Bm, partial, b, h)
+                p2 = partial.view(sg, 2 * c)
+                pend.add(p2[:, :c], ds, dw, owners=[(ctx.params[0], dw)])
+                pend.add(p2[:, c:], db, owners=[(ctx.params[1], db)])
+                return None, None, dw, db, None
+            waiting = pend.take()
+            if waiting:
+                abi.coeff_bwd_saved(dpc, A, Bm, partial, None, None, b, h, stream)
+                p2 = partial.view(sg, 2 * c)
+                abi.colsum_multi([(p2[:, :c], ds, dw), (p2[:, c:], db)] + waiting, stream)
+            else:
+                abi.coeff_bwd_saved(dpc, A, Bm, partial, ds, db, b, h, stream, dw_dense=dw)
+            return None, None, dw, db, None
+        groups = abi.coeff_bwd_groups(b, h)
+        partial = torch.empty((groups, 2, c), dtype=torch.float32, device=cj.device)
         if (pend is not None and pend.stack_armed and not pend.stack_done and PendingSums.untouched(*ctx.params)):
             pend.coeff_bwd_req = (cj, n_real, s, gb, dpooled.contiguous(), partial, b, n, h)
             p2 = partial.view(groups, 2 * c)
@@ -211,6 +240,7 @@
 
 
 COEFF_ROLE_MAX_BLOCKS = int(_os.environ.get('FETA_COEFF_ROLE_MAX', 2048))
+USE_COEFF_DSUM = _os.environ.get('FETA_COEFF_DSUM', '1') != '0'
 
 
 class PendingSums:
@@ -228,6 +258,20 @@
         self.coeff_fwd_req = None
         self.coeff_fwd_out = None
         self.coeff_bwd_req = None
+        self.coeff_dsum_req = None
+        self.coeff_dsum_out = None
+
+    def coeff_dsum_role(self, abi, graphs, k_eig):
+        req, self.coeff_dsum_req = self.coeff_dsum_req, None
+        if req is None:
+            return None
+        cj, n_real, s, gb, b, n, h = req
+        if not abi.spec_cat_fwd_coeff_fits(graphs, n, k_eig, h * b):
+            return None
+        A = torch.empty((h * b, s.shape[0]), dtype=torch.float32, device=cj.device)
+        Bm = torch.empty_like(A)
+        self.coeff_dsum_out = (A, Bm)
+        return (cj, n_real, s, gb, A, Bm, b, n, h)
 
     @staticmethod
     def untouched(*params):
@@ -281,7 +325,9 @@
         items = self.take()
         if items:
             abi, stream = _lib.backend(items[0][0])
-            if req is not None:
+            if isinstance(req, CoeffSavedReq):
+                req.run(abi, stream)
+            elif req is not None:
                 cj, n_real, s, gb, dpooled, partial, b, n, h = req
                 abi.coeff_bwd(cj, n_real, s, gb, dpooled, partial, None, None, b, n, h, stream)
             abi.colsum_multi(items, stream)
@@ -367,8 +413,10 @@
                 t, nm = cat.tail, cat.tail.norm
                 kw = dict(y2_stats=t.st2, Gx=t.G2, gamma=t.gamma, beta=t.beta, bn_out=t.prm2, rmean=nm.running_mean,
                           rvar=nm.running_var, nbt=nm.num_batches_tracked, momentum=float(nm.momentum), eps=float(nm.eps))
+            dsum = (pending.coeff_dsum_role(abi, b, g0.shape[2]) if (pending is not None and ctx.needs_input_grad[1])
+                    else None)
             abi.spec_filter_cat_fwd(xs, g0, g1, cw, bias, n_real, y, order, share, stream, y2=y2v, w_cat=cat.w.detach().contiguous(),
-                                    b_cat=None if cat.bias is None else cat.bias.detach(), out=out, **kw)
+                                    b_cat=None if cat.bias is None else cat.bias.detach(), out=out, dsum=dsum, **kw)
             cat.out = out.permute(1, 0, 2, 3).reshape(n * b, h * dh)
             cat.y = y.detach()
             cat.bwd_ok = bool(abi.spec_cat_bwd_supported(n, h, dh, order, g0.shape[2], share))
@@ -376,6 +424,8 @@
             abi.cheb_filter_fwd(xs, g0, cw, bias, n_real, y, order, share, stream)
         else:
             abi.spec_filter_fwd(xs, g0, g1, cw, bias, n_real, y, order, share, stream)
+        if pending is not None:
+            pending.coeff_dsum_req = None
         ctx.save_for_backward(xs, cw, pooled, lin_w, n_real, g0, g1)
         ctx.cfg = (mode, order, share, batch_first, bias is not None)
         ctx.cat = cat if fold else None
diff --git a/feta_tmlr_amd/fused_stack.py b/feta_tmlr_amd/fused_stack.py
--- a/feta_tmlr_amd/fused_stack.py
+++ b/feta_tmlr_amd/fused_stack.py
@@ -893,8 +893,15 @@
 def _coeff_bwd_request(ctx, abi, stream, d, ff_last):
     from . import functional as F
     req = ctx.pending.take_coeff_bwd() if ctx.pending is not None else None
-    if req is not None and (not (USE_FFN_BWD and abi.ffn_bwd_supported(d, ff_last))
-                            or req[6] * req[8] > F.COEFF_ROLE_MAX_BLOCKS):
+    if req is None:
+        return None
+    hosted = USE_FFN_BWD and abi.ffn_bwd_supported(d, ff_last)
+    if isinstance(req, F.CoeffSavedReq):
+        if not hosted:
+            req.run(abi, stream)
+            req = None
+        return req
+    if not hosted or req[6] * req[8] > F.COEFF_ROLE_MAX_BLOCKS:
         cj, n_real, s, gb, dpooled, partial, b, n, h = req
         abi.coeff_bwd(cj, n_real, s, gb, dpooled, partial, None, None, b, n, h, stream)
         req = None
diff --git a/include/feta_hip.h b/include/feta_hip.h
--- a/include/feta_hip.h
+++ b/include/feta_hip.h
@@ -49,6 +49,13 @@
                    const float* s, const float* gcn_bias, const float* dpooled,
                    float* partial, float* ds, float* dbias, float* dw_dense, int dw_rows,
                    int B, int N, int H, int C, feta_stream_t stream);
+
+int feta_coeff_dsum(const float* cj, const int32_t* n_real, const float* s, const float* gcn_bias,
+                    float* A, float* Bm, int B, int N, int H, int C, feta_stream_t stream);
+int feta_coeff_bwd_saved_groups(int B, int H);
+int feta_coeff_bwd_saved(const float* dpooled, const float* A, const float* Bm,
+                         float* partial, float* ds, float* dbias, float* dw_dense, int dw_rows,
+                         int B, int H, int C, feta_stream_t stream);
 
 int feta_colsum(const float* in, float* out, int R, int C, feta_stream_t stream);
 
@@ -124,6 +131,17 @@
                              const float* coeff, const float* bias, const int32_t* n_real, float* y,
                              int64_t y_sb, int64_t y_sn, int B, int N, int H, int dh, int P, int K,
                              int heads_share_graph, const feta_spec_cat* cat, feta_stream_t stream);
+
+int feta_spec_cat_fwd_coeff_fits(int B, int N, int K, int blocks);
+typedef struct feta_coeff_dsum_role {
+  const float* cj; const int32_t* n_real; const float* s; const float* gcn_bias; float* A; float* Bm;
+  int B, N, H, C;
+} feta_coeff_dsum_role;
+int feta_spec_filter_cat_fwd_coeff(const float* x, int64_t x_sb, int64_t x_sn, const float* u, const float* lam,
+                                   const float* coeff, const float* bias, const int32_t* n_real, float* y,
+                                   int64_t y_sb, int64_t y_sn, int B, int N, int H, int dh, int P, int K,
+                                   int heads_share_graph, const feta_spec_cat* cat, const feta_coeff_dsum_role* role,
+                                   feta_stream_t stream);
 
 typedef struct feta_spec_cat_grad {
   const float* dout;
@@ -441,6 +459,11 @@
   int B, N, H, C;
 } feta_coeff_bwd_role;
 int feta_ffn_bwd_coeff(const feta_ffn_grad* d, const feta_coeff_bwd_role* c, feta_stream_t stream);
+typedef struct feta_coeff_bwd_saved_role {
+  const float* dpooled; const float* A; const float* Bm; float* partial;
+  int B, H, C;
+} feta_coeff_bwd_saved_role;
+int feta_ffn_bwd_coeff_saved(const feta_ffn_grad* d, const feta_coeff_bwd_saved_role* c, feta_stream_t stream);
 
 #define FETA_ENCODER_MAX_LAYERS 16
 #define FETA_NORM_BATCH 0
```

New measurement: 506,400 graphs/s, median of 6. 2.0% higher.
